# alxn3/nbody-llm

Hardware: AMD Instinct MI355X
Metric: pairwise_interactions_per_sec (higher is better)
Workload: dtype f32

## Files before the change

include/nbody_hip.h:

```cpp
#ifndef NBODY_HIP_H
#define NBODY_HIP_H

#include <stddef.h>
#include <stdint.h>

#ifdef __cplusplus
extern "C" {
#endif

#define NBODY_ABI_VERSION 4

typedef struct NbodyHandle NbodyHandle;

enum {
    NBODY_OK = 0,
    NBODY_ERR_INVALID = -1,
    NBODY_ERR_HIP = -2,
    NBODY_ERR_CAPACITY = -3,
    NBODY_ERR_TREE_DEPTH = -4,
    NBODY_ERR_COMM = -5,
    NBODY_ERR_NO_DEVICE = -6
};

#define NBODY_MAX_TREE_DEPTH 192

enum { NBODY_BRUTE_FORCE = 0,
       NBODY_BARNES_HUT = 1 };

enum { NBODY_MATH_STRICT = 0,
       NBODY_MATH_FAST = 1 };

enum { NBODY_TREE_HOST = 0,
       NBODY_TREE_DEVICE = 1,
       NBODY_TREE_AUTO = 2 };

enum {
    NBODY_LEAF_REFERENCE = 0,
    NBODY_LEAF_DIRECT = 1
};

enum { NBODY_F32 = 0,
       NBODY_F64 = 1 };

enum { NBODY_SHARD_INDEX = 0,
       NBODY_SHARD_SPATIAL = 1 };

typedef struct NbodyConfig {
    uint32_t struct_size;
    int32_t method;
    int32_t math_mode;
    int32_t leaf_mode;
    int32_t device;
    int32_t rank;
    int32_t world_size;
    int32_t host_threads;
    uint64_t capacity;
    int32_t tree_build;
    int32_t dtype;
    int32_t shard_mode;
    int32_t reserved;
} NbodyConfig;

typedef struct NbodyStats {
    uint64_t steps;
    uint64_t interactions;
    uint64_t node_visits;
    uint64_t tree_nodes;
    uint64_t force_launches;
    uint64_t force_kernel_interactions;
    double force_kernel_ms;
    double tree_build_ms;
    double tree_copy_ms;
    double exchange_ms;
} NbodyStats;

int nbody_create(const NbodyConfig* cfg, NbodyHandle** out);
void nbody_destroy(NbodyHandle* h);
int nbody_clone(const NbodyHandle* h, NbodyHandle** out);
int nbody_get_config(const NbodyHandle* h, NbodyConfig* out);

int nbody_upload(NbodyHandle* h, const void* aos, size_t n, size_t stride_bytes);
int nbody_download(NbodyHandle* h, void* aos, size_t cap, size_t stride_bytes, size_t* n_out);
int nbody_count(NbodyHandle* h, size_t* n_out);
int nbody_count_global(NbodyHandle* h, size_t* n_out);
int nbody_add_point(NbodyHandle* h, const void* particle);
int nbody_remove_point(NbodyHandle* h, size_t index);

int nbody_set_settings(NbodyHandle* h, float g, float g_soft, float dt, float theta2);
int nbody_get_settings(const NbodyHandle* h, float* g, float* g_soft, float* dt, float* theta2);
int nbody_set_bounds(NbodyHandle* h, const float center[3], float width);
int nbody_set_settings_f64(NbodyHandle* h, double g, double g_soft, double dt, double theta2);
int nbody_get_settings_f64(const NbodyHandle* h, double* g, double* g_soft, double* dt, double* theta2);
int nbody_set_bounds_f64(NbodyHandle* h, const double center[3], double width);

int nbody_init(NbodyHandle* h);
int nbody_step_by(NbodyHandle* h, float dt);
int nbody_step_by_f64(NbodyHandle* h, double dt);
int nbody_steps(NbodyHandle* h, int k);
int nbody_update_forces(NbodyHandle* h);
int nbody_elapsed(const NbodyHandle* h, float* out);
int nbody_elapsed_f64(const NbodyHandle* h, double* out);
int nbody_sync(NbodyHandle* h);

int nbody_set_profiling(NbodyHandle* h, int on);
int nbody_stats(NbodyHandle* h, NbodyStats* out);
int nbody_reset_stats(NbodyHandle* h);
int nbody_energy(NbodyHandle* h, double* kinetic, double* potential);
enum { NBODY_POTENTIAL_PAIRS = 0,
       NBODY_POTENTIAL_TREE  = 1 };
int nbody_potentials(NbodyHandle* h, int mode, double* phi, size_t cap, size_t* n_out, uint64_t counts[2]);
int nbody_energy_world(NbodyHandle* h, int mode, double* kinetic, double* potential);
int nbody_tree_export(NbodyHandle* h, float* com_mass, float* width, int32_t* skip, size_t cap, size_t* n_nodes);
int nbody_tree_export_f64(NbodyHandle* h, double* com_mass, double* width, int32_t* skip, size_t cap, size_t* n_nodes);
int nbody_tree_export_cells(NbodyHandle* h, float* min_max6, int32_t* depth, size_t cap, size_t* n_nodes);
const char* nbody_last_error(const NbodyHandle* h);

int nbody_set_tuning(NbodyHandle* h, const char* name, int value);
int nbody_get_tuning(const NbodyHandle* h, const char* name, int* value);
int nbody_is_tuning_build(void);

#define NBODY_COMM_ID_BYTES 128
int nbody_comm_unique_id(void* id_bytes);
int nbody_comm_local_id(void* id_bytes);
int nbody_comm_init(NbodyHandle* h, const void* id_bytes);
int nbody_comm_transport(const NbodyHandle* h, char* out, size_t cap);
int nbody_local_range(const NbodyHandle* h, size_t* first, size_t* count);
int nbody_download_ids(NbodyHandle* h, int32_t* ids, size_t cap, size_t* n_out);
typedef struct NbodyLetStats {
    uint64_t steps;
    uint64_t bodies_migrated;
    uint64_t nodes_local;
    uint64_t nodes_global;
    uint64_t nodes_sent;
    uint64_t nodes_received;
    uint64_t bytes_sent;
    uint64_t bytes_allgather_equivalent;
    double phase_ms[5];
    uint64_t host_syncs;
    uint64_t migrant_respills;
    uint64_t node_array_peak_bytes;
    uint64_t node_array_bytes;
} NbodyLetStats;
int nbody_let_stats(NbodyHandle* h, NbodyLetStats* out);

int nbody_ic_plummer(void* aos, size_t n, size_t stride_bytes, uint64_t seed);
int nbody_ic_disc(void* aos, size_t n_disc, size_t stride_bytes, uint64_t seed);
int nbody_ic_plummer_f64(void* aos, size_t n, size_t stride_bytes, uint64_t seed);
int nbody_ic_disc_f64(void* aos, size_t n_disc, size_t stride_bytes, uint64_t seed);

int nbody_debug_step_begin(NbodyHandle* h, float dt);
int nbody_debug_import_segment(NbodyHandle* h, NbodyHandle* peer);
int nbody_debug_step_forces(NbodyHandle* h, float dt);
int nbody_debug_import_partials(NbodyHandle* h, NbodyHandle* peer);
int nbody_debug_step_end(NbodyHandle* h, float dt);
int nbody_debug_let_phase(NbodyHandle* h, int phase, float dt);
int nbody_debug_let_exchange(NbodyHandle* h, NbodyHandle* peer, int which);
int nbody_debug_let_set_balance(NbodyHandle* h, int by_work);
int nbody_debug_let_bounds(NbodyHandle* h, unsigned long long* out);
int nbody_debug_let_set_prune(NbodyHandle* h, int prune);

int nbody_host_cross_plan(int rank, int world, int seg_cap, int n_own, int* ipt, int* n_sets, int* n_parts, int* parts,
                          int* n_recv, int* recv_from);

int nbody_host_exchange_layout(const int* matrix, int world, int rank, long long clamp, int packed_send, size_t send_stride,
                               size_t* out_at, size_t* n_out, size_t* in_at, size_t* n_in, size_t* total_in);

int nbody_host_launch_plan(size_t n_bodies, float theta2, int fast_math, int out[3]);

int nbody_host_build_tree(const float* pos4, size_t n, const float center[3], float width, int threads,
                          float* com_mass, float* node_width, int32_t* skip, int32_t* leaf_body, int32_t* order,
                          size_t cap, size_t* n_nodes);

int nbody_abi_version(void);
int nbody_device_count(void);

#ifdef __cplusplus
}
#endif
#endif
```

nbody-llm_amd/__init__.py:

```python
from __future__ import annotations

import ctypes as C
import os
from dataclasses import dataclass

import numpy as np

_HERE = os.path.dirname(os.path.abspath(__file__))
LIB_PATH = os.environ.get("NBODY_HIP_LIBRARY") or os.path.join(_HERE, "libnbody_hip.so")

if not os.path.exists(LIB_PATH):
    raise ImportError(
        f"{LIB_PATH} not found: build it with `make -C nbody-llm_amd/csrc` (or __graft_entry__.build()); "
        "there is no Python/CPU fallback for the HIP engine"
    )

lib = C.CDLL(LIB_PATH, mode=C.RTLD_LOCAL)

NBODY_OK = 0
NBODY_ERR_INVALID = -1
NBODY_ERR_HIP = -2
NBODY_ERR_CAPACITY = -3
NBODY_ERR_TREE_DEPTH = -4
NBODY_ERR_COMM = -5
NBODY_ERR_NO_DEVICE = -6
BRUTE_FORCE, BARNES_HUT = 0, 1
STRICT, FAST = 0, 1
LEAF_REFERENCE = 0
LEAF_DIRECT = 1
TREE_HOST, TREE_DEVICE, TREE_AUTO = 0, 1, 2
COMM_ID_BYTES = 128

PARTICLE_DTYPE = np.dtype(
    [("position", "<f4", 3), ("velocity", "<f4", 3), ("acceleration", "<f4", 3), ("mass", "<f4")]
)
assert PARTICLE_DTYPE.itemsize == 40
PARTICLE_DTYPE64 = np.dtype(
    [("position", "<f8", 3), ("velocity", "<f8", 3), ("acceleration", "<f8", 3), ("mass", "<f8")]
)
assert PARTICLE_DTYPE64.itemsize == 80
F32, F64 = 0, 1
POTENTIAL_PAIRS, POTENTIAL_TREE = 0, 1
SHARD_INDEX, SHARD_SPATIAL = 0, 1

DECLARED_SYMBOLS = [
    "nbody_create", "nbody_destroy", "nbody_clone", "nbody_upload", "nbody_download", "nbody_count",
    "nbody_count_global", "nbody_add_point", "nbody_remove_point", "nbody_set_settings", "nbody_get_settings",
    "nbody_set_bounds", "nbody_init", "nbody_step_by", "nbody_steps", "nbody_update_forces", "nbody_elapsed",
    "nbody_sync", "nbody_set_profiling", "nbody_stats", "nbody_reset_stats", "nbody_energy", "nbody_tree_export",
    "nbody_last_error", "nbody_comm_unique_id", "nbody_comm_init", "nbody_local_range", "nbody_ic_plummer",
    "nbody_ic_disc", "nbody_host_build_tree", "nbody_abi_version", "nbody_device_count",
    "nbody_debug_step_begin", "nbody_debug_import_segment", "nbody_debug_step_forces",
    "nbody_debug_import_partials", "nbody_debug_step_end", "nbody_host_cross_plan",
    "nbody_set_settings_f64", "nbody_get_settings_f64", "nbody_set_bounds_f64", "nbody_step_by_f64", "nbody_elapsed_f64",
    "nbody_tree_export_f64", "nbody_ic_plummer_f64", "nbody_ic_disc_f64",
    "nbody_download_ids", "nbody_let_stats", "nbody_debug_let_phase", "nbody_debug_let_exchange", "nbody_debug_let_set_prune",
    "nbody_debug_let_bounds", "nbody_debug_let_set_balance",
    "nbody_comm_local_id", "nbody_comm_transport", "nbody_host_exchange_layout",
    "nbody_set_tuning", "nbody_get_tuning", "nbody_is_tuning_build", "nbody_tree_export_cells", "nbody_host_launch_plan",
    "nbody_get_config", "nbody_potentials", "nbody_energy_world",
]


class NbodyConfig(C.Structure):
    _fields_ = [
        ("struct_size", C.c_uint32), ("method", C.c_int32), ("math_mode", C.c_int32), ("leaf_mode", C.c_int32),
        ("device", C.c_int32), ("rank", C.c_int32), ("world_size", C.c_int32), ("host_threads", C.c_int32),
        ("capacity", C.c_uint64), ("tree_build", C.c_int32), ("dtype", C.c_int32), ("shard_mode", C.c_int32), ("reserved", C.c_int32),
    ]


class NbodyLetStats(C.Structure):
    _fields_ = [(k, C.c_uint64) for k in ("steps", "bodies_migrated", "nodes_local", "nodes_global", "nodes_sent", "nodes_received",
                                          "bytes_sent", "bytes_allgather_equivalent")] + [("phase_ms", C.c_double * 5)] + \
               [(k, C.c_uint64) for k in ("host_syncs", "migrant_respills", "node_array_peak_bytes", "node_array_bytes")]


class NbodyStats(C.Structure):
    _fields_ = [
        ("steps", C.c_uint64), ("interactions", C.c_uint64), ("node_visits", C.c_uint64), ("tree_nodes", C.c_uint64),
        ("force_launches", C.c_uint64), ("force_kernel_interactions", C.c_uint64), ("force_kernel_ms", C.c_double), ("tree_build_ms", C.c_double),
        ("tree_copy_ms", C.c_double), ("exchange_ms", C.c_double),
    ]


_H = C.c_void_p
_f, _sz, _i = C.c_float, C.c_size_t, C.c_int
_pf = C.POINTER(C.c_float)


def _sig(name, restype, *argtypes):
    fn = getattr(lib, name)
    fn.restype = restype
    fn.argtypes = list(argtypes)
    return fn


_sig("nbody_create", _i, C.POINTER(NbodyConfig), C.POINTER(_H))
_sig("nbody_destroy", None, _H)
_sig("nbody_clone", _i, _H, C.POINTER(_H))
_sig("nbody_upload", _i, _H, C.c_void_p, _sz, _sz)
_sig("nbody_download", _i, _H, C.c_void_p, _sz, _sz, C.POINTER(_sz))
_sig("nbody_count", _i, _H, C.POINTER(_sz))
_sig("nbody_count_global", _i, _H, C.POINTER(_sz))
_sig("nbody_add_point", _i, _H, C.c_void_p)
_sig("nbody_remove_point", _i, _H, _sz)
_sig("nbody_set_settings", _i, _H, _f, _f, _f, _f)
_sig("nbody_get_settings", _i, _H, _pf, _pf, _pf, _pf)
_sig("nbody_set_bounds", _i, _H, _pf, _f)
_sig("nbody_init", _i, _H)
_sig("nbody_step_by", _i, _H, _f)
_sig("nbody_steps", _i, _H, _i)
_sig("nbody_update_forces", _i, _H)
_sig("nbody_elapsed", _i, _H, _pf)
_sig("nbody_sync", _i, _H)
_sig("nbody_set_profiling", _i, _H, _i)
_sig("nbody_stats", _i, _H, C.POINTER(NbodyStats))
_sig("nbody_reset_stats", _i, _H)
_sig("nbody_energy", _i, _H, C.POINTER(C.c_double), C.POINTER(C.c_double))
_sig("nbody_potentials", _i, _H, _i, C.c_void_p, _sz, C.POINTER(_sz), C.POINTER(C.c_uint64))
_sig("nbody_energy_world", _i, _H, _i, C.POINTER(C.c_double), C.POINTER(C.c_double))
_sig("nbody_tree_export", _i, _H, C.c_void_p, C.c_void_p, C.c_void_p, _sz, C.POINTER(_sz))
_sig("nbody_tree_export_cells", _i, _H, C.c_void_p, C.c_void_p, _sz, C.POINTER(_sz))
_sig("nbody_last_error", C.c_char_p, _H)
_sig("nbody_comm_unique_id", _i, C.c_void_p)
_sig("nbody_comm_init", _i, _H, C.c_void_p)
_sig("nbody_comm_local_id", _i, C.c_void_p)
_sig("nbody_comm_transport", _i, _H, C.c_char_p, _sz)
_sig("nbody_local_range", _i, _H, C.POINTER(_sz), C.POINTER(_sz))
_sig("nbody_ic_plummer", _i, C.c_void_p, _sz, _sz, C.c_uint64)
_sig("nbody_ic_disc", _i, C.c_void_p, _sz, _sz, C.c_uint64)
_sig("nbody_host_build_tree", _i, C.c_void_p, _sz, _pf, _f, _i, C.c_void_p, C.c_void_p, C.c_void_p, C.c_void_p,
     C.c_void_p, _sz, C.POINTER(_sz))
_sig("nbody_debug_step_begin", _i, _H, _f)
_sig("nbody_debug_import_segment", _i, _H, _H)
_sig("nbody_debug_step_forces", _i, _H, _f)
_sig("nbody_debug_import_partials", _i, _H, _H)
_sig("nbody_debug_step_end", _i, _H, _f)
_sig("nbody_host_cross_plan", _i, _i, _i, _i, _i, C.POINTER(_i), C.POINTER(_i), C.POINTER(_i), C.c_void_p, C.POINTER(_i),
     C.c_void_p)
_d = C.c_double
_pd = C.POINTER(C.c_double)
_sig("nbody_set_settings_f64", _i, _H, _d, _d, _d, _d)
_sig("nbody_get_settings_f64", _i, _H, _pd, _pd, _pd, _pd)
_sig("nbody_set_bounds_f64", _i, _H, _pd, _d)
_sig("nbody_step_by_f64", _i, _H, _d)
_sig("nbody_elapsed_f64", _i, _H, _pd)
_sig("nbody_tree_export_f64", _i, _H, C.c_void_p, C.c_void_p, C.c_void_p, _sz, C.POINTER(_sz))
_sig("nbody_ic_plummer_f64", _i, C.c_void_p, _sz, _sz, C.c_uint64)
_sig("nbody_ic_disc_f64", _i, C.c_void_p, _sz, _sz, C.c_uint64)
_sig("nbody_download_ids", _i, _H, C.c_void_p, _sz, C.POINTER(_sz))
_sig("nbody_let_stats", _i, _H, C.POINTER(NbodyLetStats))
_sig("nbody_debug_let_phase", _i, _H, _i, _f)
_sig("nbody_debug_let_exchange", _i, _H, _H, _i)
_sig("nbody_debug_let_set_prune", _i, _H, _i)
_sig("nbody_debug_let_bounds", _i, _H, C.c_void_p)
_sig("nbody_debug_let_set_balance", _i, _H, _i)
_sig("nbody_host_exchange_layout", _i, C.c_void_p, _i, _i, C.c_longlong, _i, _sz, C.c_void_p, C.c_void_p, C.c_void_p, C.c_void_p, C.POINTER(_sz))
_sig("nbody_host_launch_plan", _i, _sz, _f, _i, C.POINTER(_i))
_sig("nbody_set_tuning", _i, _H, C.c_char_p, _i)
_sig("nbody_get_tuning", _i, _H, C.c_char_p, C.POINTER(_i))
_sig("nbody_is_tuning_build", _i)
_sig("nbody_get_config", _i, _H, C.POINTER(NbodyConfig))
_sig("nbody_abi_version", _i)
_sig("nbody_device_count", _i)


_default_tuning: dict = {}


class tuning_defaults:
    def __init__(self, **knobs):
        self.knobs = knobs

    def __enter__(self):
        self.saved = dict(_default_tuning)
        _default_tuning.update(self.knobs)
        return self

    def __exit__(self, *a):
        _default_tuning.clear()
        _default_tuning.update(self.saved)


def launch_plan(n_bodies: int, theta2: float = 0.25, fast_math: bool = True) -> dict:
    out = (C.c_int * 3)()
    rc = lib.nbody_host_launch_plan(int(n_bodies), float(theta2), int(bool(fast_math)), out)
    if rc != 0:
        raise NbodyError(rc, "nbody_host_launch_plan")
    return {"walk_bodies_per_lane": out[0], "walk_segments": out[1], "sym_bodies_per_lane": out[2]}


def is_tuning_build() -> bool:
    return bool(lib.nbody_is_tuning_build())


class NbodyError(RuntimeError):
    def __init__(self, code: int, msg: str):
        super().__init__(f"nbody error {code}: {msg}")
        self.code = code


def device_count() -> int:
    return int(lib.nbody_device_count())


def plummer(n: int, seed: int = 20250523, f64: bool = False) -> np.ndarray:
    if f64:
        out = np.zeros(n, dtype=PARTICLE_DTYPE64)
        rc = lib.nbody_ic_plummer_f64(out.ctypes.data, n, 80, seed)
        if rc:
            raise NbodyError(rc, "nbody_ic_plummer_f64")
        return out
    out = np.zeros(n, dtype=PARTICLE_DTYPE)
    rc = lib.nbody_ic_plummer(out.ctypes.data, n, 40, seed)
    if rc:
        raise NbodyError(rc, "nbody_ic_plummer")
    return out


def disc(n_disc: int, seed: int = 20250523, f64: bool = False) -> np.ndarray:
# ... 367 lines not shown
```

nbody-llm_amd/csrc/bf_pair.h:

```cpp
#pragma once
#include <hip/hip_runtime.h>

namespace nbody {
namespace {

__device__ __forceinline__ float rotl(float v, int src_lane_x4) {
    return __int_as_float(__builtin_amdgcn_ds_bpermute(src_lane_x4, __float_as_int(v)));
}

#define PAD_POS 1.0e15f

template <int IPT, int DBG = 0, bool SYM = true>
__device__ __forceinline__ void pair_evals(const float (&xi)[IPT], const float (&yi)[IPT], const float (&zi)[IPT],
                                           const float (&mi)[IPT], float (&axi)[IPT], float (&ayi)[IPT],
                                           float (&azi)[IPT], float xj, float yj, float zj, float mj, float& axj,
                                           float& ayj, float& azj, float eps2) {
    float dx[IPT], dy[IPT], dz[IPT], r[IPT], sj[IPT];
#pragma unroll
    for (int q = 0; q < IPT; ++q) dx[q] = xj - xi[q];
#pragma unroll
    for (int q = 0; q < IPT; ++q) dy[q] = yj - yi[q];
#pragma unroll
    for (int q = 0; q < IPT; ++q) dz[q] = zj - zi[q];
    __builtin_amdgcn_sched_barrier(0);
#pragma unroll
    for (int q = 0; q < IPT; ++q) r[q] = __builtin_fmaf(dx[q], dx[q], eps2);
    __builtin_amdgcn_sched_barrier(0);
#pragma unroll
    for (int q = 0; q < IPT; ++q) r[q] = __builtin_fmaf(dy[q], dy[q], r[q]);
    __builtin_amdgcn_sched_barrier(0);
#pragma unroll
    for (int q = 0; q < IPT; ++q) r[q] = __builtin_fmaf(dz[q], dz[q], r[q]);
    __builtin_amdgcn_sched_barrier(0);
#pragma unroll
    for (int q = 0; q < IPT; ++q) {
        if (DBG & 2) asm volatile("v_mul_f32 %0, %0, %0" : "+v"(r[q]));
        else r[q] = __builtin_amdgcn_rsqf(r[q]);
    }
    __builtin_amdgcn_sched_barrier(0);
#pragma unroll
    for (int q = 0; q < IPT; ++q) sj[q] = r[q] * r[q];
    __builtin_amdgcn_sched_barrier(0);
#pragma unroll
    for (int q = 0; q < IPT; ++q) r[q] = sj[q] * r[q];
    __builtin_amdgcn_sched_barrier(0);
#pragma unroll
    for (int q = 0; q < IPT; ++q) sj[q] = mj * r[q];
    __builtin_amdgcn_sched_barrier(0);
    if (SYM) {
#pragma unroll
        for (int q = 0; q < IPT; ++q) r[q] = mi[q] * r[q];
        __builtin_amdgcn_sched_barrier(0);
#pragma unroll
        for (int q = 0; q < IPT; ++q) {
            axi[q] = __builtin_fmaf(dx[q], sj[q], axi[q]);
            axj = __builtin_fmaf(-dx[q], r[q], axj);
            ayi[q] = __builtin_fmaf(dy[q], sj[q], ayi[q]);
            ayj = __builtin_fmaf(-dy[q], r[q], ayj);
            azi[q] = __builtin_fmaf(dz[q], sj[q], azi[q]);
            azj = __builtin_fmaf(-dz[q], r[q], azj);
            __builtin_amdgcn_sched_barrier(0);
        }
    } else {
#pragma unroll
        for (int q = 0; q < IPT; ++q) axi[q] = __builtin_fmaf(dx[q], sj[q], axi[q]);
        __builtin_amdgcn_sched_barrier(0);
#pragma unroll
        for (int q = 0; q < IPT; ++q) ayi[q] = __builtin_fmaf(dy[q], sj[q], ayi[q]);
        __builtin_amdgcn_sched_barrier(0);
#pragma unroll
        for (int q = 0; q < IPT; ++q) azi[q] = __builtin_fmaf(dz[q], sj[q], azi[q]);
        __builtin_amdgcn_sched_barrier(0);
    }
}


typedef float v2f __attribute__((ext_vector_type(2)));

__device__ __forceinline__ v2f splat2(float v) { v2f r = {v, v}; return r; }
__device__ __forceinline__ v2f pk_fma(v2f a, v2f b, v2f c) { return __builtin_elementwise_fma(a, b, c); }

template <int IPT2, int DBG = 0, bool SYM = true>
__device__ __forceinline__ void pair_evals_pk(const v2f (&xi)[IPT2], const v2f (&yi)[IPT2], const v2f (&zi)[IPT2],
                                              const v2f (&mi)[IPT2], v2f (&axi)[IPT2], v2f (&ayi)[IPT2],
                                              v2f (&azi)[IPT2], float xj, float yj, float zj, float mj, v2f& axj,
                                              v2f& ayj, v2f& azj, float eps2) {
    v2f dx[IPT2], dy[IPT2], dz[IPT2], r[IPT2], sj[IPT2];
    const v2f xj2 = splat2(xj), yj2 = splat2(yj), zj2 = splat2(zj), mj2 = splat2(mj), e2 = splat2(eps2);
#pragma unroll
    for (int q = 0; q < IPT2; ++q) dx[q] = xj2 - xi[q];
#pragma unroll
    for (int q = 0; q < IPT2; ++q) dy[q] = yj2 - yi[q];
#pragma unroll
    for (int q = 0; q < IPT2; ++q) dz[q] = zj2 - zi[q];
    __builtin_amdgcn_sched_barrier(0);
#pragma unroll
    for (int q = 0; q < IPT2; ++q) r[q] = pk_fma(dx[q], dx[q], e2);
    __builtin_amdgcn_sched_barrier(0);
#pragma unroll
    for (int q = 0; q < IPT2; ++q) r[q] = pk_fma(dy[q], dy[q], r[q]);
    __builtin_amdgcn_sched_barrier(0);
#pragma unroll
    for (int q = 0; q < IPT2; ++q) r[q] = pk_fma(dz[q], dz[q], r[q]);
    __builtin_amdgcn_sched_barrier(0);
#pragma unroll
    for (int q = 0; q < IPT2; ++q) {
        if (DBG & 2) { asm volatile("v_mul_f32 %0, %0, %0" : "+v"(r[q].x)); asm volatile("v_mul_f32 %0, %0, %0" : "+v"(r[q].y)); }
        else { r[q].x = __builtin_amdgcn_rsqf(r[q].x); r[q].y = __builtin_amdgcn_rsqf(r[q].y); }
    }
    __builtin_amdgcn_sched_barrier(0);
#pragma unroll
    for (int q = 0; q < IPT2; ++q) sj[q] = r[q] * r[q];
    __builtin_amdgcn_sched_barrier(0);
#pragma unroll
    for (int q = 0; q < IPT2; ++q) r[q] = sj[q] * r[q];
    __builtin_amdgcn_sched_barrier(0);
#pragma unroll
    for (int q = 0; q < IPT2; ++q) sj[q] = mj2 * r[q];
    __builtin_amdgcn_sched_barrier(0);
    if (SYM) {
#pragma unroll
        for (int q = 0; q < IPT2; ++q) r[q] = mi[q] * r[q];
        __builtin_amdgcn_sched_barrier(0);
#pragma unroll
        for (int q = 0; q < IPT2; ++q) {
            axi[q] = pk_fma(dx[q], sj[q], axi[q]);
            axj = pk_fma(-dx[q], r[q], axj);
            ayi[q] = pk_fma(dy[q], sj[q], ayi[q]);
            ayj = pk_fma(-dy[q], r[q], ayj);
            azi[q] = pk_fma(dz[q], sj[q], azi[q]);
            azj = pk_fma(-dz[q], r[q], azj);
            __builtin_amdgcn_sched_barrier(0);
        }
    } else {
#pragma unroll
        for (int q = 0; q < IPT2; ++q) axi[q] = pk_fma(dx[q], sj[q], axi[q]);
        __builtin_amdgcn_sched_barrier(0);
#pragma unroll
        for (int q = 0; q < IPT2; ++q) ayi[q] = pk_fma(dy[q], sj[q], ayi[q]);
        __builtin_amdgcn_sched_barrier(0);
#pragma unroll
        for (int q = 0; q < IPT2; ++q) azi[q] = pk_fma(dz[q], sj[q], azi[q]);
        __builtin_amdgcn_sched_barrier(0);
    }
}

template <int IPT>
__device__ __forceinline__ void pack_pairs(const float (&a)[IPT], v2f (&b)[IPT / 2]) {
#pragma unroll
    for (int q = 0; q < IPT / 2; ++q) b[q] = v2f{a[2 * q], a[2 * q + 1]};
}
template <int IPT>
__device__ __forceinline__ void unpack_pairs(const v2f (&b)[IPT / 2], float (&a)[IPT]) {
#pragma unroll
    for (int q = 0; q < IPT / 2; ++q) { a[2 * q] = b[q].x; a[2 * q + 1] = b[q].y; }
}

}
}
```

nbody-llm_amd/csrc/kernels.h:

```cpp
#pragma once
#include <hip/hip_runtime.h>
#include <cstdint>
#include <vector>

namespace nbody {

struct Tuning {
    int cross_sym = 1;
    int sym_packed = 1;
    int bf_fast_variant = 0;
    int bh_walk_duo = -1;
    int bh_walk_xcd = 1;
    int let_list_div = 4;
    int sym_ipt = 0;
    int sym_wpb = 4;
    int sym_rounds = 1;
    int sym_k = 0;
    int sym_min_bodies = 1024;
    int sym_reduce_split = 1;
    int cross_slots = 3072;
    int cross_ipt = 0;
    int cross_wpb = 4;
    int bh_walk_split = 0;
    int bh_walk_order = 1;
    int bh_reduce_split = 1;
    int tree_max_tie = 64;
    int bf64_min_bodies = 10240;
    int bf64_ipt = 0;
    int bf64_rot = 0;
    int bf64_waves = 0;
    int bh_walk_variant = 0;
    int bh_walk_lds_block = 1024;
    int bh_hot_cap = 2048;
    int bh_walk_debug = 0;
    int sym_debug = 0;
};
const Tuning& tuning();
struct WalkPlan { int bodies_per_lane; int segments; };
WalkPlan walk_plan(size_t n_order, bool fast_math, int max_segments, float theta2);
void bind_tuning(const Tuning* t);

struct Shard {
    float4* pos_all = nullptr;
    float4* vel = nullptr;
    float4* acc = nullptr;
    int* seg_count = nullptr;
    int* escaped = nullptr;
    unsigned char* keep = nullptr;
    unsigned long long* tile_state = nullptr;
    int* epoch = nullptr;
    int* poison = nullptr;
    int* ids = nullptr;
    unsigned long long* inter = nullptr;
    int n_seg = 1;
    int seg_cap = 0;
    int my_seg = 0;
    float4* own_pos() const { return pos_all + size_t(my_seg) * seg_cap; }
    int* own_count() const { return seg_count + my_seg; }
};

struct BoundsF {
    float lo[3];
    float hi[3];
};

void launch_aos_to_soa(hipStream_t s, const float* aos, int stride_f, int n, float4* pos, float4* vel, float4* acc);
void launch_soa_to_aos(hipStream_t s, float* aos, int stride_f, int n, const float4* pos, const float4* vel, const float4* acc);

void launch_drift_half(hipStream_t s, const Shard& sh, int n_upper, float dt, BoundsF b);
void launch_compact(hipStream_t s, const Shard& sh, int n_upper);
void launch_kick_drift(hipStream_t s, const Shard& sh, int n_upper, float dt);

void launch_bf_forces_strict(hipStream_t s, const Shard& sh, int n_upper, float g, float g_soft2);
void launch_bf_forces_fast(hipStream_t s, const Shard& sh, int n_upper, float g, float g_soft2);

struct SymPlan {
    int ipt = 8;
    int A = 0;
    int K = 0;
    int wpb = 16;
    int res_combine = 0;
    int k_res = 0;
    int sym_sets = 0;
    int n_planes = 0;
    int k_os = 0;
    size_t n_pad = 0;
    size_t plane_stride = 0;
    std::vector<int> bounds;
};
SymPlan make_sym_plan(int n_upper);
int sym_bodies_per_lane(size_t n);
uint64_t sym_main_pairs(const SymPlan& p, size_t n);
void launch_bf_sym_main(hipStream_t s, const Shard& sh, const SymPlan& p, const int* d_bounds, float4* planes,
                        int n_upper, float g_soft2);
void launch_bf_os(hipStream_t s, const Shard& sh, int A, int K, float4* planes, size_t plane_stride, float g_soft2);
void launch_bf_sym_tail(hipStream_t s, const Shard& sh, const SymPlan& p, float4* planes, int n_upper, float g,
                        float g_soft2, const float* kick_dt);

struct CrossPartners {
    static constexpr int kMax = 8;
    int n = 0;
    int seg[kMax];
    int c0[kMax], c1[kMax];
    int a0[kMax], a1[kMax];
};
struct CrossPlan {
    static constexpr int kMaxPlanes = 256;
    int ipt = 8;
    int A = 0;
    CrossPartners parts;
    int n_recv = 0;
    int recv_from[CrossPartners::kMax];
    int k_res = 0;
    std::vector<int4> slices;
};
CrossPlan make_cross_plan(int rank, int world, int seg_cap, int n_own_upper);
void launch_bf_cross(hipStream_t s, const Shard& sh, const CrossPlan& p, const int4* d_slices, float4* res_planes,
                     float4* xplanes, float4* send, size_t plane_stride, float g_soft2);

constexpr int kMaxSplit = 64, kMaxAnc = 192;
constexpr size_t kSplitInts = size_t(kMaxSplit) + 1 + kMaxSplit + size_t(kMaxSplit) * kMaxAnc;
struct TreeDev {
    const float4* nodes = nullptr;
    int n_nodes = 0;
    const int* order = nullptr;
    int n_order = 0;
    int n_split = 1;
    const int* split_first = nullptr;
    const int* split_anc = nullptr;
    const int* split_n_anc = nullptr;
    float4* split_planes = nullptr;
    size_t split_stride = 0;
    float4* nested_stack = nullptr;
    size_t nested_stride = 0;
    float4* walk = nullptr;
    float4* hot = nullptr;
    int* unified = nullptr;
    int* hot_info = nullptr;
    int hot_cap = 0;
    int hot_threshold = 0;
    const int* poison = nullptr;
    const int* n_order_dev = nullptr;
    int store_work = 0;
    float4* bfs = nullptr;
    void* bfs_ws = nullptr;
    size_t bfs_cap = 0;
};
struct TreeDevWork {
    const unsigned long long* keys = nullptr;
    const signed char* delta = nullptr;
    const int* base = nullptr;
    const int* ids = nullptr;
    const unsigned long long* keys2 = nullptr;
    const int* wpre = nullptr;
    const void* incl = nullptr;
};
struct TreeCat {
    float4* pos = nullptr;
    int* flags = nullptr;
    int* base = nullptr;
    int* own_order = nullptr;
    int* info = nullptr;
};
size_t tree_build_workspace_bytes(size_t n_cap);
size_t tree_build_tmp_bytes(size_t n_cap);
size_t tree_cat_bytes(size_t n_cap);
TreeCat tree_cat_layout(void* buf, size_t n_cap);
void launch_tree_cat(hipStream_t s, const Shard& sh, const TreeCat& c);
size_t tree_cat_bytes64(size_t n_cap);
TreeCat tree_cat_layout64(void* buf, size_t n_cap, double4** pos_cat);
void launch_tree_cat64(hipStream_t s, const double4* pos_all, const int* seg_count, int n_seg, int seg_cap, int my_seg, double4* pos_cat, int* info);
int launch_tree_own_order(hipStream_t s, const int* order, const TreeCat& c, int n_total_upper, void* tmp, size_t tmp_bytes);
struct TreeSplitReq { int n_split = 0; int* first = nullptr; int* n_anc = nullptr; int* anc = nullptr; int max_anc = 0; const int* info = nullptr; int* poison = nullptr; };
int build_octree_device(hipStream_t s, const float4* pos, const int* d_count, int n_upper, const float center[3],
                        float width, void* workspace, size_t n_cap, float4* nodes, int node_cap, int* order,
                        int* out_info, TreeDevWork* work, int want_hot = 0 , const TreeSplitReq* split = nullptr);
size_t bfs_workspace_bytes(size_t n_cap);
int build_bfs_layout(hipStream_t s, const float4* nodes, int n_nodes, void* workspace, size_t n_cap, float4* out);
}
namespace nbody64 { struct Node64; }
namespace nbody {
int build_octree_device_f64(hipStream_t s, const double4* pos, const int* d_count, int n_upper, const double center[3], double width,
                            void* workspace, size_t n_cap, nbody64::Node64* nodes, int node_cap, int* order, int* out_info,
                            TreeDevWork* work, const TreeSplitReq* split = nullptr);
int tree_sort_keys(hipStream_t s, const float4* pos, const int* d_count, int n_upper, const float center[3], float width,
                   void* workspace, size_t n_cap, int* out_info, TreeDevWork* work);
int tree_emit_sorted(hipStream_t s, const float4* pos, const int* d_count, int n_upper, float width, void* workspace, size_t n_cap,
                     float4* nodes, int node_cap, int* order, int* out_info, int want_hot, const int* edge, const TreeSplitReq* split = nullptr);
int tree_scan_sorted(hipStream_t s, const float4* pos, const int* d_count, int n_upper, void* workspace, size_t n_cap, int* out_info,
                     const int* edge, const float4* weight_src = nullptr );
__host__ __device__ inline int body_weight(float visits) { const int v = int(visits) >> 4; return v < 1 ? 1 : v; }
int tree_emit_nodes(hipStream_t s, const float4* pos, const int* d_count, int n_upper, float width, void* workspace, size_t n_cap,
                    float4* nodes, int node_cap, int slice_cap, int* order, int* out_info, int want_hot, const int* edge,
                    const int* node_offset, int* parent, unsigned char* depth);
void launch_tree_split_anc(hipStream_t s, const TreeDevWork& work, int n, int n_nodes, int n_split, int* first,
                           int* n_anc, int* anc, int max_anc, const int* info = nullptr ,
                           int* poison = nullptr );

#define NBODY_WALK_COUNTER_SLOTS 1024u
void launch_walk_split_scan(hipStream_t s, const float4* nodes, const int* range, int n_split, int* first, int* n_anc, int* anc, int first_given = 0);
void launch_bh_walk(hipStream_t s, const Shard& sh, const TreeDev& t, float g, float g_soft2, float theta2,
                    int fast_math, unsigned long long* counters , int leaf_direct = 0,
                    const float* kick_dt = nullptr ,
                    int* kicked = nullptr );

void launch_energy(hipStream_t s, const Shard& sh, int n_upper, double g_soft2, double* out2);

}
```

nbody-llm_amd/csrc/kernels_bf_sym.hip:

```cpp
#include "kernels.h"
#include "bf_pair.h"

#include <algorithm>

namespace nbody {

namespace {

#ifdef NBODY_TUNING
__device__ unsigned long long nbody_sym_stamps[3 * 8192];
#endif

}

template <int IPT>
__device__ __forceinline__ void sym_rest_wave(const float4* __restrict__ pos, int n, int A, int group, int slice,
                                              int n_slices, float& ax, float& ay, float& az, float eps2);

template <int IPT, int NW>
__device__ __forceinline__ void sym_rest_block(const float4* __restrict__ pos, int n, int A, int group,
                                               float4* __restrict__ plane, float eps2, float (*red)[3][64]);

template <int IPT, int WPB, int DBG = 0, bool PK = false>
__global__ __launch_bounds__(WPB * 64) void k_bf_sym(const float4* __restrict__ pos, const int* __restrict__ count,
                                                     int A, int K, const int* __restrict__ bounds, int sym_sets,
                                                     float4* __restrict__ planes, size_t plane_stride, float eps2,
                                                     int res_combine) {
    const int lane = threadIdx.x & 63;
    const int wslot = __builtin_amdgcn_readfirstlane(threadIdx.x >> 6);
    const int n_main_blocks = (A * K + WPB - 1) / WPB;
    if (int(blockIdx.x) >= n_main_blocks) {
        __shared__ float red[WPB - 1][3][64];
        sym_rest_block<IPT, WPB>(pos, *count, A, blockIdx.x - n_main_blocks,
                                 planes + size_t(sym_sets + (res_combine ? K / WPB : K)) * plane_stride, eps2, red);
        return;
    }
    const int gw = blockIdx.x * WPB + (wslot & 3) * (WPB / 4) + (wslot >> 2);
    if (gw >= A * K) return;
    const int a = gw / K;
    const int part = gw - a * K;
    const int n = *count;
    const int Cn = A * IPT;
    const int k0 = bounds[part], k1 = bounds[part + 1];
    const int src_lane = ((lane + 63) & 63) * 4;
    const int src_lane2 = ((lane + 62) & 63) * 4;
    float eps2v = eps2;
    asm volatile("" : "+v"(eps2v));

    float xi[IPT], yi[IPT], zi[IPT], mi[IPT], axi[IPT], ayi[IPT], azi[IPT];
#pragma unroll
    for (int q = 0; q < IPT; ++q) {
        const int i = (a * IPT + q) * 64 + lane;
        const float4 p = (i < n) ? pos[i] : make_float4(PAD_POS, PAD_POS, PAD_POS, 0.f);
        xi[q] = p.x; yi[q] = p.y; zi[q] = p.z; mi[q] = p.w;
        axi[q] = ayi[q] = azi[q] = 0.f;
    }

    auto chunk_of = [&](int k) {
        int c = (a + 1) * IPT + k;
        if (c >= Cn) c -= Cn;
        return c;
    };
    auto load_chunk = [&](int k) {
        const int j = chunk_of(k) * 64 + lane;
        return (j < n) ? pos[j] : make_float4(PAD_POS, PAD_POS, PAD_POS, 0.f);
    };

    [[maybe_unused]] unsigned long long t_beg = 0, r_beg = 0;
    if (DBG & 4) { t_beg = __builtin_amdgcn_s_memtime(); r_beg = __builtin_amdgcn_s_memrealtime(); }
    float4 nxt = (k0 < k1) ? load_chunk(k0) : make_float4(0.f, 0.f, 0.f, 0.f);
    v2f xi2[IPT / 2], yi2[IPT / 2], zi2[IPT / 2], mi2[IPT / 2], axi2[IPT / 2], ayi2[IPT / 2], azi2[IPT / 2];
    if (PK) {
        pack_pairs<IPT>(xi, xi2); pack_pairs<IPT>(yi, yi2); pack_pairs<IPT>(zi, zi2); pack_pairs<IPT>(mi, mi2);
        pack_pairs<IPT>(axi, axi2); pack_pairs<IPT>(ayi, ayi2); pack_pairs<IPT>(azi, azi2);
    }
    for (int k = k0; k < k1; ++k) {
        float xj = nxt.x, yj = nxt.y, zj = nxt.z, mj = nxt.w;
        float axj = 0.f, ayj = 0.f, azj = 0.f;
        v2f axj2 = {0.f, 0.f}, ayj2 = {0.f, 0.f}, azj2 = {0.f, 0.f};
        if (k + 1 < k1) nxt = load_chunk(k + 1);
        switch ((4 * (k1 - k) - 1) / (k1 - k0)) {
            case 3: __builtin_amdgcn_s_setprio(3); break;
            case 2: __builtin_amdgcn_s_setprio(2); break;
            case 1: __builtin_amdgcn_s_setprio(1); break;
            default: __builtin_amdgcn_s_setprio(0); break;
        }
        if (PK) {
            for (int s = 0; s < 64; s += 2) {
                const float x1 = rotl(xj, src_lane), y1 = rotl(yj, src_lane), z1 = rotl(zj, src_lane), m1 = rotl(mj, src_lane);
                pair_evals_pk<IPT / 2, DBG>(xi2, yi2, zi2, mi2, axi2, ayi2, azi2, xj, yj, zj, mj, axj2, ayj2, azj2, eps2v);
                axj2.x = rotl(axj2.x, src_lane); ayj2.x = rotl(ayj2.x, src_lane); azj2.x = rotl(azj2.x, src_lane);
                axj2.y = rotl(axj2.y, src_lane); ayj2.y = rotl(ayj2.y, src_lane); azj2.y = rotl(azj2.y, src_lane);
                xj = rotl(x1, src_lane); yj = rotl(y1, src_lane); zj = rotl(z1, src_lane); mj = rotl(m1, src_lane);
                pair_evals_pk<IPT / 2, DBG>(xi2, yi2, zi2, mi2, axi2, ayi2, azi2, x1, y1, z1, m1, axj2, ayj2, azj2, eps2v);
                axj2.x = rotl(axj2.x, src_lane); ayj2.x = rotl(ayj2.x, src_lane); azj2.x = rotl(azj2.x, src_lane);
                axj2.y = rotl(axj2.y, src_lane); ayj2.y = rotl(ayj2.y, src_lane); azj2.y = rotl(azj2.y, src_lane);
            }
        } else {
            float x1 = rotl(xj, src_lane), y1 = rotl(yj, src_lane), z1 = rotl(zj, src_lane), m1 = rotl(mj, src_lane);
#pragma unroll 2
            for (int s = 0; s < 64; ++s) {
                const float x2 = rotl(xj, src_lane2), y2 = rotl(yj, src_lane2), z2 = rotl(zj, src_lane2), m2 = rotl(mj, src_lane2);
                pair_evals<IPT, DBG>(xi, yi, zi, mi, axi, ayi, azi, xj, yj, zj, mj, axj, ayj, azj, eps2v);
                axj = rotl(axj, src_lane); ayj = rotl(ayj, src_lane); azj = rotl(azj, src_lane);
                xj = x1; yj = y1; zj = z1; mj = m1;
                x1 = x2; y1 = y2; z1 = z2; m1 = m2;
            }
        }
        if (PK) { axj = axj2.x + axj2.y; ayj = ayj2.x + ayj2.y; azj = azj2.x + azj2.y; }
        const int d = k / IPT + 1;
        planes[size_t(d - 1) * plane_stride + size_t(chunk_of(k)) * 64 + lane] = make_float4(axj, ayj, azj, 0.f);
    }
    if (PK) { unpack_pairs<IPT>(axi2, axi); unpack_pairs<IPT>(ayi2, ayi); unpack_pairs<IPT>(azi2, azi); }

#ifdef NBODY_TUNING
    if (DBG & 4) {
        const unsigned long long t_end = __builtin_amdgcn_s_memtime(), r_end = __builtin_amdgcn_s_memrealtime();
        if (lane == 0 && gw < 8192) {
            nbody_sym_stamps[gw * 3 + 0] = t_end - t_beg;
            nbody_sym_stamps[gw * 3 + 1] = r_end - r_beg;
            const unsigned hw = __builtin_amdgcn_s_getreg((4 ) | (0 << 6) | (31 << 11));
            const unsigned xcc = __builtin_amdgcn_s_getreg((20 ) | (0 << 6) | (31 << 11));
            nbody_sym_stamps[gw * 3 + 2] = (unsigned long long)(k1 - k0) | ((unsigned long long)hw << 16) | ((unsigned long long)(xcc & 0xF) << 48);
        }
    }
#endif
    if (res_combine) {
        __shared__ float comb[WPB - 1][3 * IPT][64];
        const int first_part = (part / WPB) * WPB;
        const int rel = part - first_part;
        if (rel > 0) {
#pragma unroll
            for (int q = 0; q < IPT; ++q) {
                comb[rel - 1][3 * q + 0][lane] = axi[q];
                comb[rel - 1][3 * q + 1][lane] = ayi[q];
                comb[rel - 1][3 * q + 2][lane] = azi[q];
            }
        }
        __syncthreads();
        if (rel == 0) {
            float4* __restrict__ out = planes + size_t(sym_sets + part / WPB) * plane_stride;
#pragma unroll
            for (int q = 0; q < IPT; ++q) {
                float sx = axi[q], sy = ayi[q], sz = azi[q];
                for (int w = 0; w < WPB - 1; ++w) { sx += comb[w][3 * q + 0][lane]; sy += comb[w][3 * q + 1][lane]; sz += comb[w][3 * q + 2][lane]; }
                out[size_t(a * IPT + q) * 64 + lane] = make_float4(sx, sy, sz, 0.f);
            }
        }
        return;
    }
    float4* __restrict__ out = planes + size_t(sym_sets + part) * plane_stride;
#pragma unroll
    for (int q = 0; q < IPT; ++q) out[size_t(a * IPT + q) * 64 + lane] = make_float4(axi[q], ayi[q], azi[q], 0.f);
}

template <int IPT, int WPB, bool PK>
__global__ __launch_bounds__(WPB * 64) void k_bf_os(const float4* __restrict__ pos_all,
                                                    const int* __restrict__ seg_count, int n_seg, int seg_cap,
                                                    int my_seg, int A, int K, float4* __restrict__ planes,
                                                    size_t plane_stride, float eps2) {
    __shared__ float4 stage[WPB][2][64];
    const int lane = threadIdx.x & 63;
    const int wslot = __builtin_amdgcn_readfirstlane(threadIdx.x >> 6);
    const int gw = blockIdx.x * WPB + (wslot & 3) * (WPB / 4) + (wslot >> 2);
    if (gw >= A * K) return;
    const int a = gw / K, part = gw - a * K;
    const int n_own = seg_count[my_seg];
    const float4* __restrict__ own = pos_all + size_t(my_seg) * seg_cap;
    float eps2v = eps2;
    asm volatile("" : "+v"(eps2v));

    float xi[IPT], yi[IPT], zi[IPT], mi[IPT], axi[IPT], ayi[IPT], azi[IPT];
#pragma unroll
    for (int q = 0; q < IPT; ++q) {
        const int i = (a * IPT + q) * 64 + lane;
        const float4 p = (i < n_own) ? own[i] : make_float4(PAD_POS, PAD_POS, PAD_POS, 0.f);
        xi[q] = p.x; yi[q] = p.y; zi[q] = p.z; mi[q] = p.w;
        axi[q] = ayi[q] = azi[q] = 0.f;
    }
    long long R = 0;
    for (int s = 0; s < n_seg; ++s) if (s != my_seg) R += seg_count[s];
    const long long r0 = R * part / K, r1 = R * (part + 1) / K;
    long long seg_first = 0;
    float dummy_x = 0.f, dummy_y = 0.f, dummy_z = 0.f;
    v2f dummy2 = {0.f, 0.f};
    v2f xi2[IPT / 2], yi2[IPT / 2], zi2[IPT / 2], mi2[IPT / 2], axi2[IPT / 2], ayi2[IPT / 2], azi2[IPT / 2];
    if (PK) {
        pack_pairs<IPT>(xi, xi2); pack_pairs<IPT>(yi, yi2); pack_pairs<IPT>(zi, zi2); pack_pairs<IPT>(mi, mi2);
        pack_pairs<IPT>(axi, axi2); pack_pairs<IPT>(ayi, ayi2); pack_pairs<IPT>(azi, azi2);
    }
    for (int s = 0; s < n_seg; ++s) {
        if (s == my_seg) continue;
        const int ns = seg_count[s];
        const long long lo = r0 > seg_first ? r0 : seg_first;
        const long long hi = r1 < seg_first + ns ? r1 : seg_first + ns;
        const float4* __restrict__ ps = pos_all + size_t(s) * seg_cap - seg_first;
        int buf = 0;
        if (lo < hi) {
            const long long j = lo + lane;
            stage[wslot][0][lane] = (j < hi) ? ps[j] : make_float4(PAD_POS, PAD_POS, PAD_POS, 0.f);
        }
        for (long long c0 = lo; c0 < hi; c0 += 64) {
            const long long jn = c0 + 64 + lane;
            float4 nxt = make_float4(PAD_POS, PAD_POS, PAD_POS, 0.f);
            if (c0 + 64 < hi && jn < hi) nxt = ps[jn];
            const int cnt = int(hi - c0 < 64 ? hi - c0 : 64);
            switch (int((4 * (r1 - c0) - 1) / (r1 - r0))) {
                case 3: __builtin_amdgcn_s_setprio(3); break;
                case 2: __builtin_amdgcn_s_setprio(2); break;
                case 1: __builtin_amdgcn_s_setprio(1); break;
                default: __builtin_amdgcn_s_setprio(0); break;
            }
            float4 pj = stage[wslot][buf][0];
            for (int t = 0; t < cnt; ++t) {
                const float4 pn = stage[wslot][buf][(t + 1) & 63];
                if (PK)
                    pair_evals_pk<IPT / 2, 0, false>(xi2, yi2, zi2, mi2, axi2, ayi2, azi2, pj.x, pj.y, pj.z, pj.w, dummy2,
                                                     dummy2, dummy2, eps2v);
                else
                    pair_evals<IPT, 0, false>(xi, yi, zi, mi, axi, ayi, azi, pj.x, pj.y, pj.z, pj.w, dummy_x, dummy_y,
                                              dummy_z, eps2v);
                pj = pn;
            }
            buf ^= 1;
            stage[wslot][buf][lane] = nxt;
        }
        seg_first += ns;
    }
    if (PK) { unpack_pairs<IPT>(axi2, axi); unpack_pairs<IPT>(ayi2, ayi); unpack_pairs<IPT>(azi2, azi); }
    float4* __restrict__ out = planes + size_t(part) * plane_stride;
#pragma unroll
    for (int q = 0; q < IPT; ++q) out[size_t(a * IPT + q) * 64 + lane] = make_float4(axi[q], ayi[q], azi[q], 0.f);
}

template <int IPT>
__device__ __forceinline__ void sym_rest_wave(const float4* __restrict__ pos, int n, int A, int group, int slice,
                                              int n_slices, float& ax, float& ay, float& az, float eps2) {
    constexpr int SET = 64 * IPT;
    const int lane = threadIdx.x & 63;
    const int i = group * 64 + lane;
    const int a = (group * 64) / SET;
    const float4 pi = (i < n) ? pos[i] : make_float4(PAD_POS, PAD_POS, PAD_POS, 0.f);
    ax = ay = az = 0.f;
    const int n_win = (A % 2 == 0 && A > 1) ? 2 : 1;
    for (int w = 0; w < n_win; ++w) {
        int set = (w == 0) ? a : a + A / 2;
        if (set >= A) set -= A;
        const int j0 = set * SET + SET * slice / n_slices;
        const int j1 = min(n, set * SET + SET * (slice + 1) / n_slices);
#pragma unroll 8
        for (int j = j0; j < j1; ++j) {
            const float4 pj = pos[j];
            const float dx = pj.x - pi.x, dy = pj.y - pi.y, dz = pj.z - pi.z;
            const float r2 = __builtin_fmaf(dz, dz, __builtin_fmaf(dy, dy, __builtin_fmaf(dx, dx, eps2)));
            const float rinv = __builtin_amdgcn_rsqf(r2);
            float sj = pj.w * ((rinv * rinv) * rinv);
            sj = (j == i) ? 0.f : sj;
            ax = __builtin_fmaf(dx, sj, ax);
            ay = __builtin_fmaf(dy, sj, ay);
            az = __builtin_fmaf(dz, sj, az);
        }
    }
}

template <int IPT, int NW>
__device__ __forceinline__ void sym_rest_block(const float4* __restrict__ pos, int n, int A, int group,
                                               float4* __restrict__ plane, float eps2, float (*red)[3][64]) {
    const int lane = threadIdx.x & 63;
    const int wv = __builtin_amdgcn_readfirstlane(threadIdx.x >> 6);
    float ax, ay, az;
    sym_rest_wave<IPT>(pos, n, A, group, wv, NW, ax, ay, az, eps2);
    if (wv > 0) { red[wv - 1][0][lane] = ax; red[wv - 1][1][lane] = ay; red[wv - 1][2][lane] = az; }
    __syncthreads();
    if (wv == 0) {
#pragma unroll
        for (int w = 0; w < NW - 1; ++w) { ax += red[w][0][lane]; ay += red[w][1][lane]; az += red[w][2][lane]; }
        plane[group * 64 + lane] = make_float4(ax, ay, az, 0.f);
    }
}

template <int IPT>
__global__ __launch_bounds__(512) void k_bf_sym_rest(const float4* __restrict__ pos, const int* __restrict__ count,
                                                     int A, float4* __restrict__ plane, float eps2) {
    __shared__ float red[7][3][64];
    sym_rest_block<IPT, 8>(pos, *count, A, blockIdx.x, plane, eps2, red);
}

template <bool KICK>
__global__ __launch_bounds__(256) void k_bf_sym_reduce(const float4* __restrict__ planes, int n_planes,
                                                       size_t plane_stride, const int* __restrict__ count, float g,
                                                       float4* __restrict__ acc, float4* __restrict__ pos,
                                                       float4* __restrict__ vel, float dt, const int* __restrict__ seg_count,
                                                       int n_seg, unsigned long long* __restrict__ inter) {
    const int i = blockIdx.x * 256 + threadIdx.x;
    if (inter && i == 0) {
        long long tot = 0;
        for (int s = 0; s < n_seg; ++s) tot += seg_count[s];
        if (tot > 0) atomicAdd(inter, (unsigned long long)(*count) * (unsigned long long)(tot - 1));
    }
    if (i >= *count) return;
    float sx = 0.f, sy = 0.f, sz = 0.f, cx = 0.f, cy = 0.f, cz = 0.f;
    for (int p = 0; p < n_planes; ++p) {
        const float4 v = planes[size_t(p) * plane_stride + i];
        const float yx = v.x - cx, yy = v.y - cy, yz = v.z - cz;
        const float tx = sx + yx, ty = sy + yy, tz = sz + yz;
        cx = (tx - sx) - yx; cy = (ty - sy) - yy; cz = (tz - sz) - yz;
        sx = tx; sy = ty; sz = tz;
    }
    const float4 a = make_float4(g * sx, g * sy, g * sz, 0.f);
    acc[i] = a;
    if (KICK) {
        float4 p = pos[i], v = vel[i];
        v.x += a.x * dt; v.y += a.y * dt; v.z += a.z * dt;
        p.x += (v.x * 0.5f) * dt; p.y += (v.y * 0.5f) * dt; p.z += (v.z * 0.5f) * dt;
        vel[i] = v;
        pos[i] = p;
    }
}

template <bool KICK, int Q>
__global__ __launch_bounds__(64 * Q) void k_bf_sym_reduce_split(const float4* __restrict__ planes, int n_planes, size_t plane_stride,
                                                                const int* __restrict__ count, float g, float4* __restrict__ acc,
                                                                float4* __restrict__ pos, float4* __restrict__ vel, float dt,
                                                                const int* __restrict__ seg_count, int n_seg,
                                                                unsigned long long* __restrict__ inter) {
    __shared__ float part[Q][3][64];
    const int lane = threadIdx.x & 63, q = threadIdx.x >> 6;
    const int i = blockIdx.x * 64 + lane;
    if (inter && blockIdx.x == 0 && threadIdx.x == 0) {
        long long tot = 0;
        for (int s = 0; s < n_seg; ++s) tot += seg_count[s];
        if (tot > 0) atomicAdd(inter, (unsigned long long)(*count) * (unsigned long long)(tot - 1));
    }
    const int n = *count;
    float sx = 0.f, sy = 0.f, sz = 0.f, cx = 0.f, cy = 0.f, cz = 0.f;
    if (i < n) {
        const int p0 = int((long long)n_planes * q / Q), p1 = int((long long)n_planes * (q + 1) / Q);
        for (int p = p0; p < p1; ++p) {
            const float4 v = planes[size_t(p) * plane_stride + i];
            const float yx = v.x - cx, yy = v.y - cy, yz = v.z - cz;
            const float tx = sx + yx, ty = sy + yy, tz = sz + yz;
            cx = (tx - sx) - yx; cy = (ty - sy) - yy; cz = (tz - sz) - yz;
            sx = tx; sy = ty; sz = tz;
        }
    }
    part[q][0][lane] = sx; part[q][1][lane] = sy; part[q][2][lane] = sz;
    __syncthreads();
    if (q != 0 || i >= n) return;
    sx = sy = sz = cx = cy = cz = 0.f;
    for (int w = 0; w < Q; ++w) {
        const float yx = part[w][0][lane] - cx, yy = part[w][1][lane] - cy, yz = part[w][2][lane] - cz;
        const float tx = sx + yx, ty = sy + yy, tz = sz + yz;
        cx = (tx - sx) - yx; cy = (ty - sy) - yy; cz = (tz - sz) - yz;
        sx = tx; sy = ty; sz = tz;
    }
    const float4 a = make_float4(g * sx, g * sy, g * sz, 0.f);
    acc[i] = a;
    if (KICK) {
        float4 p = pos[i], v = vel[i];
        v.x += a.x * dt; v.y += a.y * dt; v.z += a.z * dt;
        p.x += (v.x * 0.5f) * dt; p.y += (v.y * 0.5f) * dt; p.z += (v.z * 0.5f) * dt;
        vel[i] = v;
        pos[i] = p;
    }
}

}
#ifdef NBODY_TUNING
namespace nbody { int read_sym_stamps(unsigned long long* out, int n_waves); }
extern "C" int nbody_sym_read_stamps(unsigned long long* out, int n_waves) { return nbody::read_sym_stamps(out, n_waves); }
#endif
namespace nbody {

int sym_bodies_per_lane(size_t n) {
    const Tuning& t = tuning();
    if (!t.sym_packed || t.sym_wpb != 4 || t.sym_ipt == 8) return 8;
    if (t.sym_ipt == 4) return 4;
    return n <= 10240 ? 4 : 8;
}

SymPlan make_sym_plan(int n_upper) {
    SymPlan p;
    const int IPT = sym_bodies_per_lane(size_t(n_upper));
    p.ipt = IPT;
    p.A = (n_upper + 64 * IPT - 1) / (64 * IPT);
    p.sym_sets = (p.A + 1) / 2 - 1;
    const int L = IPT * p.sym_sets;
    const int want = tuning().sym_wpb;
    p.wpb = want == 8 ? 8 : want == 12 ? 12 : want == 16 ? 16 : 4;
    int K = 1;
    if (p.wpb == 4) {
        K = L <= 100 ? L : L <= 160 ? (L + 1) / 2 : 64;
    } else {
        const int resident_wgs_per_cu = (p.wpb == 8) ? 2 : 1;
        const int slots = 256 * resident_wgs_per_cu * p.wpb;
        double best = 0.0;
        const int k_hi = std::min(126, std::min(L, std::max(1, slots * std::max(1, tuning().sym_rounds) * 4 / p.A)));
        for (int k = 1; k <= k_hi; ++k) {
            const long long waves = (long long)p.A * k;
            const long long rounds = (waves + slots - 1) / slots;
            if (rounds > 4 * std::max(1, tuning().sym_rounds) && k > 1) break;
            const double fill = double(waves) / double(rounds * slots);
            const double even = (L % k == 0) ? 1.0 : double(L / k) / double(L / k + 1);
            const double per_wave = double(L) / k / (double(L) / k + 0.3);
            if (fill * even * per_wave > best + 1e-9) { best = fill * even * per_wave; K = k; }
        }
    }
    if (tuning().sym_k > 0) K = std::min(126, tuning().sym_k);
    if (K > L) K = L;
    if (K < 1) K = 1;
    p.K = K;
    p.res_combine = (K % p.wpb == 0) ? 1 : 0;
    p.k_res = p.res_combine ? K / p.wpb : K;
    p.n_planes = p.sym_sets + p.k_res + 1;
    p.n_pad = size_t(p.A) * 64 * IPT;
    p.plane_stride = p.n_pad;
    p.bounds.resize(K + 1);
    for (int part = 0; part <= K; ++part) p.bounds[part] = int((long long)L * part / K);
    return p;
}

#ifdef NBODY_TUNING
int read_sym_stamps(unsigned long long* out, int n_waves) {
    return hipMemcpyFromSymbol(out, HIP_SYMBOL(nbody_sym_stamps), sizeof(unsigned long long) * 3 * n_waves) == hipSuccess ? 0 : -1;
}
#endif

uint64_t sym_main_pairs(const SymPlan& p, size_t n) {
    const size_t set = size_t(64) * p.ipt;
    auto size_of = [&](int a) { size_t lo = size_t(a) * set; return lo >= n ? size_t(0) : std::min(set, n - lo); };
    uint64_t pairs = 0;
    for (int a = 0; a < p.A; ++a)
        for (int d = 1; d <= p.sym_sets; ++d) pairs += uint64_t(size_of(a)) * uint64_t(size_of((a + d) % p.A));
    return pairs;
}

void launch_bf_sym_main(hipStream_t s, const Shard& sh, const SymPlan& p, const int* d_bounds, float4* planes,
                        int n_upper, float g_soft2) {
    if (n_upper <= 0 || p.sym_sets <= 0) return;
    const int main_blocks = (p.A * p.K + p.wpb - 1) / p.wpb;
    const int rest_blocks = int(p.n_pad / 64);
    const dim3 grid(main_blocks + rest_blocks), block(p.wpb * 64);
#define SYM_LAUNCH(WPB, DBG) hipLaunchKernelGGL((k_bf_sym<8, WPB, DBG, PKV>), grid, block, 0, s, sh.own_pos(), sh.own_count(), p.A, p.K, d_bounds, p.sym_sets, planes, p.plane_stride, g_soft2, p.res_combine)
#ifdef NBODY_TUNING
    const int dbg = tuning().sym_debug;
#else
    constexpr int dbg = 0;
#endif
    if (p.ipt == 4) {
        hipLaunchKernelGGL((k_bf_sym<4, 4, 0, true>), grid, block, 0, s, sh.own_pos(), sh.own_count(), p.A, p.K, d_bounds, p.sym_sets, planes, p.plane_stride, g_soft2, p.res_combine);
        return;
    }
    if (tuning().sym_packed) {
        constexpr bool PKV = true;
        if (dbg == 4) {
#ifdef NBODY_TUNING
            if (p.wpb == 12) SYM_LAUNCH(12, 4); else if (p.wpb == 8) SYM_LAUNCH(8, 4); else if (p.wpb == 4) SYM_LAUNCH(4, 4); else SYM_LAUNCH(16, 4);
#endif
        } else {
            if (p.wpb == 12) SYM_LAUNCH(12, 0); else if (p.wpb == 8) SYM_LAUNCH(8, 0); else if (p.wpb == 4) SYM_LAUNCH(4, 0); else SYM_LAUNCH(16, 0);
        }
    } else {
        constexpr bool PKV = false;
        if (dbg >= 4 && dbg <= 7) {
#ifdef NBODY_TUNING
            if (dbg == 4) { if (p.wpb == 12) SYM_LAUNCH(12, 4); else if (p.wpb == 8) SYM_LAUNCH(8, 4); else if (p.wpb == 4) SYM_LAUNCH(4, 4); else SYM_LAUNCH(16, 4); }
            else if (dbg == 5) SYM_LAUNCH(16, 5);
            else if (dbg == 6) SYM_LAUNCH(16, 6);
            else SYM_LAUNCH(16, 7);
#endif
        } else {
            if (p.wpb == 12) SYM_LAUNCH(12, 0); else if (p.wpb == 8) SYM_LAUNCH(8, 0); else if (p.wpb == 4) SYM_LAUNCH(4, 0); else SYM_LAUNCH(16, 0);
        }
    }
#undef SYM_LAUNCH
}

void launch_bf_os(hipStream_t s, const Shard& sh, int A, int K, float4* planes, size_t plane_stride, float g_soft2) {
    if (A <= 0 || K <= 0) return;
    const int wpb = 12;
    if (tuning().sym_packed)
        hipLaunchKernelGGL((k_bf_os<8, 12, true>), dim3((A * K + wpb - 1) / wpb), dim3(wpb * 64), 0, s, sh.pos_all,
                           sh.seg_count, sh.n_seg, sh.seg_cap, sh.my_seg, A, K, planes, plane_stride, g_soft2);
    else
        hipLaunchKernelGGL((k_bf_os<8, 12, false>), dim3((A * K + wpb - 1) / wpb), dim3(wpb * 64), 0, s, sh.pos_all,
                           sh.seg_count, sh.n_seg, sh.seg_cap, sh.my_seg, A, K, planes, plane_stride, g_soft2);
}

void launch_bf_sym_tail(hipStream_t s, const Shard& sh, const SymPlan& p, float4* planes, int n_upper, float g,
                        float g_soft2, const float* kick_dt) {
    if (n_upper <= 0) return;
    if (p.sym_sets == 0) {
        float4* resident0 = planes + size_t(p.sym_sets) * p.plane_stride;
        (void)hipMemsetAsync(resident0, 0, size_t(p.k_res) * p.plane_stride * sizeof(float4), s);
        if (p.ipt == 4)
            hipLaunchKernelGGL(k_bf_sym_rest<4>, dim3(int(p.n_pad / 64)), dim3(512), 0, s, sh.own_pos(),
                               sh.own_count(), p.A, planes + size_t(p.sym_sets + p.k_res) * p.plane_stride, g_soft2);
        else
        hipLaunchKernelGGL(k_bf_sym_rest<8>, dim3(int(p.n_pad / 64)), dim3(512), 0, s, sh.own_pos(),
                           sh.own_count(), p.A, planes + size_t(p.sym_sets + p.k_res) * p.plane_stride, g_soft2);
    }
    const float dt = kick_dt ? *kick_dt : 0.f;
#define REDUCE_ARGS planes, p.n_planes, p.plane_stride, sh.own_count(), g, sh.acc, sh.own_pos(), sh.vel, dt, sh.seg_count, sh.n_seg, sh.inter
    if (tuning().sym_reduce_split && p.n_planes >= 16) {
        const dim3 grid((n_upper + 63) / 64);
        if (n_upper <= 16384) {
            if (kick_dt) hipLaunchKernelGGL((k_bf_sym_reduce_split<true, 16>), grid, dim3(1024), 0, s, REDUCE_ARGS);
            else hipLaunchKernelGGL((k_bf_sym_reduce_split<false, 16>), grid, dim3(1024), 0, s, REDUCE_ARGS);
        } else {
            if (kick_dt) hipLaunchKernelGGL((k_bf_sym_reduce_split<true, 4>), grid, dim3(256), 0, s, REDUCE_ARGS);
            else hipLaunchKernelGGL((k_bf_sym_reduce_split<false, 4>), grid, dim3(256), 0, s, REDUCE_ARGS);
        }
    } else {
        const dim3 grid((n_upper + 255) / 256);
        if (kick_dt) hipLaunchKernelGGL(k_bf_sym_reduce<true>, grid, dim3(256), 0, s, REDUCE_ARGS);
        else hipLaunchKernelGGL(k_bf_sym_reduce<false>, grid, dim3(256), 0, s, REDUCE_ARGS);
    }
#undef REDUCE_ARGS
}

}
```

nbody-llm_amd/csrc/nbody_api.cpp:

```cpp
#include "nbody_handle.h"
#include "nbody_f64.h"
#include "nbody_let.h"
#include "nbody_pot.h"

#include <algorithm>
#include <chrono>
#include <cmath>
#include <cstdio>
#include <cstdlib>
#include <cstring>
#include <memory>
#include <string>
#include <thread>
#include <vector>


static thread_local std::string g_create_err;

int fail(NbodyHandle* h, int code, const std::string& msg) {
    if (h) h->err = msg; else g_create_err = msg;
    return code;
}

namespace {
// ... 16 lines not shown
    if (records <= h->aos_cap) return NBODY_OK;
    if (h->d_aos) (void)hipFree(h->d_aos);
    if (h->h_aos) (void)hipHostFree(h->h_aos);
    h->d_aos = nullptr; h->h_aos = nullptr; h->aos_cap = 0;
    HIP_TRY(h, hipMalloc(&h->d_aos, records * 10 * sizeof(float)));
    HIP_TRY(h, hipHostMalloc(&h->h_aos, records * 10 * sizeof(float), hipHostMallocDefault));
    h->aos_cap = records;
    return NBODY_OK;
}

int sync_count(NbodyHandle* h) {
    if (!h->count_dirty) return NBODY_OK;
    HIP_TRY(h, hipMemcpyAsync(h->h_counts, h->sh.seg_count, sizeof(int) * h->sh.n_seg, hipMemcpyDeviceToHost, h->stream));
    HIP_TRY(h, hipStreamSynchronize(h->stream));
    for (int s = 0; s < h->sh.n_seg; ++s) h->seg_count_host[s] = h->h_counts[s];
    h->n_local = size_t(h->h_counts[h->sh.my_seg]);
    h->count_dirty = false;
    return NBODY_OK;
}

int push_counts(NbodyHandle* h) {
    for (int s = 0; s < h->sh.n_seg; ++s) h->h_counts[s] = h->seg_count_host[s];
    HIP_TRY(h, hipMemcpyAsync(h->sh.seg_count, h->h_counts, sizeof(int) * h->sh.n_seg, hipMemcpyHostToDevice, h->stream));
    HIP_TRY(h, hipStreamSynchronize(h->stream));
    return NBODY_OK;
}

size_t total_upper(const NbodyHandle* h) {
    size_t t = 0;
    for (int c : h->seg_count_host) t += size_t(c);
    return t;
}

int exchange_begin(NbodyHandle* h) {
    if (h->sh.n_seg == 1 && !h->comm_ready) return NBODY_OK;
    if (!h->comm_ready) return fail(h, NBODY_ERR_COMM, "world_size > 1 but nbody_comm_init has not been called");
    HIP_TRY(h, hipEventRecord(h->ev_drifted, h->stream));
    HIP_TRY(h, hipStreamWaitEvent(h->comm_stream, h->ev_drifted, 0));
    TP_TRY(h, h->tp->group_begin());
    TP_TRY(h, h->tp->all_gather(h->sh.pos_all, size_t(h->sh.seg_cap) * sizeof(float4), h->comm_stream));
    TP_TRY(h, h->tp->all_gather(h->sh.seg_count, sizeof(int), h->comm_stream));
    TP_TRY(h, h->tp->group_end());
    HIP_TRY(h, hipEventRecord(h->ev_gathered, h->comm_stream));
    h->exchange_in_flight = true;
    return NBODY_OK;
}

int exchange_wait(NbodyHandle* h) {
    if (!h->exchange_in_flight) return NBODY_OK;
    HIP_TRY(h, hipStreamWaitEvent(h->stream, h->ev_gathered, 0));
    h->exchange_in_flight = false;
    return NBODY_OK;
}

int comm_check(NbodyHandle* h) {
    if (!h->tp) return NBODY_OK;
    int rc = h->tp->check();
    return rc ? fail(h, rc, h->tp->error()) : NBODY_OK;
}

int sharded_counts_exact(NbodyHandle* h) {
    if (!h->comm_ready) return fail(h, NBODY_ERR_COMM, "world_size > 1 but nbody_comm_init has not been called");
    int rc = exchange_wait(h);
    if (rc) return rc;
    HIP_TRY(h, hipStreamSynchronize(h->stream));
    TP_TRY(h, h->tp->all_gather(h->sh.seg_count, sizeof(int), h->stream));
    h->count_dirty = true;
    return sync_count(h);
}

int push_own_count(NbodyHandle* h) {
    h->h_counts[h->sh.my_seg] = int(h->n_local);
    HIP_TRY(h, hipMemcpyAsync(h->sh.own_count(), h->h_counts + h->sh.my_seg, sizeof(int), hipMemcpyHostToDevice, h->stream));
    HIP_TRY(h, hipStreamSynchronize(h->stream));
    return NBODY_OK;
}

int sharded_add_point(NbodyHandle* h, const void* particle) {
    int rc = sharded_counts_exact(h);
    if (rc) return rc;
    const int G = h->sh.n_seg, last = G - 1;
    if (total_upper(h) >= h->cfg.capacity || h->seg_count_host[last] >= h->sh.seg_cap)
        return fail(h, NBODY_ERR_CAPACITY, "capacity exhausted (a push goes to the end of the vector: the last rank's block is full)");
    if (h->sh.my_seg == last) {
        const float* p = static_cast<const float*>(particle);
        float4 rec[3] = {make_float4(p[0], p[1], p[2], p[9]), make_float4(p[3], p[4], p[5], 0.f), make_float4(p[6], p[7], p[8], 0.f)};
        const size_t k = h->n_local;
        HIP_TRY(h, hipMemcpyAsync(h->sh.own_pos() + k, &rec[0], sizeof(float4), hipMemcpyHostToDevice, h->stream));
        HIP_TRY(h, hipMemcpyAsync(h->sh.vel + k, &rec[1], sizeof(float4), hipMemcpyHostToDevice, h->stream));
        HIP_TRY(h, hipMemcpyAsync(h->sh.acc + k, &rec[2], sizeof(float4), hipMemcpyHostToDevice, h->stream));
        HIP_TRY(h, hipStreamSynchronize(h->stream));
        h->n_local = k + 1;
        rc = push_own_count(h);
        if (rc) return rc;
    }
    h->seg_count_host[last] += 1;
    return NBODY_OK;
}

int sharded_remove_point(NbodyHandle* h, size_t index) {
    int rc = sharded_counts_exact(h);
    if (rc) return rc;
    const int G = h->sh.n_seg, me = h->sh.my_seg;
    if (index >= total_upper(h)) return fail(h, NBODY_ERR_INVALID, "swap_remove index out of range");
    int r = 0, last = G - 1;
    size_t j = index;
    while (j >= size_t(h->seg_count_host[r])) { j -= size_t(h->seg_count_host[r]); ++r; }
    while (h->seg_count_host[last] == 0) --last;
    const size_t tail = size_t(h->seg_count_host[last]) - 1;
    if (r == last) {
        if (me == r && j != tail) {
            HIP_TRY(h, hipMemcpyAsync(h->sh.own_pos() + j, h->sh.own_pos() + tail, sizeof(float4), hipMemcpyDeviceToDevice, h->stream));
            HIP_TRY(h, hipMemcpyAsync(h->sh.vel + j, h->sh.vel + tail, sizeof(float4), hipMemcpyDeviceToDevice, h->stream));
            HIP_TRY(h, hipMemcpyAsync(h->sh.acc + j, h->sh.acc + tail, sizeof(float4), hipMemcpyDeviceToDevice, h->stream));
        }
    } else if (me == last || me == r) {
        rc = ensure_aos(h, 2);
        if (rc) return rc;
        if (me == last) {
            nbody::launch_soa_to_aos(h->stream, h->d_aos, 10, 1, h->sh.own_pos() + tail, h->sh.vel + tail, h->sh.acc + tail);
            TP_TRY(h, h->tp->send(h->d_aos, 40, r, h->stream));
        } else {
            TP_TRY(h, h->tp->recv(h->d_aos, 40, last, h->stream));
            nbody::launch_aos_to_soa(h->stream, h->d_aos, 10, 1, h->sh.own_pos() + j, h->sh.vel + j, h->sh.acc + j);
        }
        HIP_TRY(h, hipGetLastError());
    }
    if (me == last) {
        h->n_local = tail;
        rc = push_own_count(h);
        if (rc) return rc;
    } else {
        HIP_TRY(h, hipStreamSynchronize(h->stream));
    }
    h->seg_count_host[last] -= 1;
    return comm_check(h);
}

int drain_events(NbodyHandle* h) {
    if (h->ev_pending.empty()) return NBODY_OK;
    HIP_TRY(h, hipStreamSynchronize(h->stream));
    for (auto& ev : h->ev_pending) {
        float ms = 0.f;
        if (hipEventElapsedTime(&ms, ev.first, ev.second) == hipSuccess) {
            h->stats.force_kernel_ms += ms;
            h->stats.force_launches += 1;
        }
        h->ev_free.push_back(ev);
    }
    h->ev_pending.clear();
    return NBODY_OK;
}

constexpr size_t kShardedSymMinBodies = 2048;

int ensure_sym_plan(NbodyHandle* h) {
    const size_t set = size_t(64) * size_t(nbody::sym_bodies_per_lane(std::max<size_t>(1, h->n_local)));
    const int A = int((std::max<size_t>(1, h->n_local) + set - 1) / set);
    const int knobs = nbody::tuning().sym_wpb * 100 + nbody::tuning().sym_rounds + nbody::tuning().sym_k * 10000 + nbody::tuning().sym_ipt * 1000000;
    if (h->sym_plan.A == A && h->sym_plan.ipt * 64 == int(set) && h->d_sym_bounds && h->sym_waves == knobs) return NBODY_OK;
    h->sym_waves = knobs;
    h->sym_plan = nbody::make_sym_plan(int(std::max<size_t>(1, h->n_local)));
    nbody::SymPlan& p = h->sym_plan;
    h->cross_on = false;
    if (h->sh.n_seg > 1) {
        const size_t cap_pad = (size_t(h->sh.seg_cap) + 63) / 64 * 64;
        p.plane_stride = std::max(p.n_pad, cap_pad);
        if (nbody::tuning().cross_sym && h->sh.n_seg <= 2 * (nbody::CrossPartners::kMax - 1)) {
            h->cross = nbody::make_cross_plan(h->sh.my_seg, h->sh.n_seg, h->sh.seg_cap, int(std::max<size_t>(1, h->n_local)));
            h->cross_on = true;
            h->recv_plane0 = p.n_planes + h->cross.k_res;
            p.n_planes += h->cross.k_res + h->cross.n_recv;
        } else {
            const int a_os = int((p.n_pad + 511) / 512);
            p.k_os = std::max(1, std::min(256, 3072 / std::max(1, a_os)));
            p.plane_stride = std::max(p.plane_stride, size_t(a_os) * 512);
            p.n_planes += p.k_os;
        }
    }
    if (!h->d_sym_bounds) HIP_TRY(h, hipMalloc(&h->d_sym_bounds, 128 * sizeof(int)));
    HIP_TRY(h, hipMemcpyAsync(h->d_sym_bounds, p.bounds.data(), p.bounds.size() * sizeof(int), hipMemcpyHostToDevice, h->stream));
    HIP_TRY(h, hipStreamSynchronize(h->stream));
    const size_t need = size_t(p.n_planes) * p.plane_stride;
    if (need > h->planes_cap) {
        if (h->d_planes) (void)hipFree(h->d_planes);
        h->d_planes = nullptr; h->planes_cap = 0;
        HIP_TRY(h, hipMalloc(&h->d_planes, need * sizeof(float4)));
        h->planes_cap = need;
    }
    if (h->cross_on) {
        const nbody::CrossPlan& c = h->cross;
        if (c.slices.size() > h->cross_slices_cap) {
            if (h->d_cross_slices) (void)hipFree(h->d_cross_slices);
            h->d_cross_slices = nullptr; h->cross_slices_cap = 0;
            HIP_TRY(h, hipMalloc(&h->d_cross_slices, (c.slices.size() + 64) * sizeof(int4)));
            h->cross_slices_cap = c.slices.size() + 64;
        }
        if (!c.slices.empty()) {
            HIP_TRY(h, hipMemcpyAsync(h->d_cross_slices, c.slices.data(), c.slices.size() * sizeof(int4), hipMemcpyHostToDevice, h->stream));
            HIP_TRY(h, hipStreamSynchronize(h->stream));
        }
        const size_t xneed = size_t(std::max(1, c.parts.n)) * size_t(c.A) * p.plane_stride;
        if (xneed > h->xplanes_cap) {
            if (h->d_xplanes) (void)hipFree(h->d_xplanes);
            h->d_xplanes = nullptr; h->xplanes_cap = 0;
            HIP_TRY(h, hipMalloc(&h->d_xplanes, xneed * sizeof(float4)));
            h->xplanes_cap = xneed;
        }
        const size_t sneed = size_t(std::max(1, c.parts.n)) * p.plane_stride;
        if (sneed > h->send_cap) {
            if (h->d_send) (void)hipFree(h->d_send);
            h->d_send = nullptr; h->send_cap = 0;
            HIP_TRY(h, hipMalloc(&h->d_send, sneed * sizeof(float4)));
            h->send_cap = sneed;
        }
    }
    return NBODY_OK;
}

int bf_forces(NbodyHandle* h) {
    const float eps2 = h->g_soft * h->g_soft;
    const bool fast = h->cfg.math_mode == NBODY_MATH_FAST && nbody::tuning().bf_fast_variant == 0;
    const bool sharded = h->sh.n_seg > 1;
    const bool sym = fast && (sharded ? size_t(h->sh.seg_cap) >= kShardedSymMinBodies : h->n_local >= size_t(std::max(1024, nbody::tuning().sym_min_bodies)));
    const size_t tot = total_upper(h);
    if (sym) {
        int rc = ensure_sym_plan(h);
        if (rc) return rc;
        if (h->sym_pairs_n != h->n_local) {
            h->sym_pairs = nbody::sym_main_pairs(h->sym_plan, h->n_local);
            h->sym_pairs_n = h->n_local;
        }
    }
    const nbody::SymPlan& p = h->sym_plan;
    uint64_t timed = 0;
    if (!(sym && sharded)) {
        int rc = exchange_wait(h);
        if (rc) return rc;
    }
    if (!sym) {
        ForceTimer t(h);
        if (h->cfg.math_mode == NBODY_MATH_STRICT) nbody::launch_bf_forces_strict(h->stream, h->sh, int(h->n_local), h->g, eps2);
        else nbody::launch_bf_forces_fast(h->stream, h->sh, int(h->n_local), h->g, eps2);
        timed = tot > 0 ? uint64_t(h->n_local) * uint64_t(tot - 1) : 0;
    } else if (!sharded) {
        {
            ForceTimer t(h);
            nbody::launch_bf_sym_main(h->stream, h->sh, p, h->d_sym_bounds, h->d_planes, int(h->n_local), eps2);
        }
        timed = 2 * h->sym_pairs;
        h->tail_pending = true;
    } else {
        nbody::launch_bf_sym_main(h->stream, h->sh, p, h->d_sym_bounds, h->d_planes, int(h->n_local), eps2);
        {
            int rc = exchange_wait(h);
            if (rc) return rc;
        }
        if (h->cross_on) {
            const nbody::CrossPlan& c = h->cross;
            {
                ForceTimer t(h);
                nbody::launch_bf_cross(h->stream, h->sh, c, h->d_cross_slices,
                                       h->d_planes + size_t(h->recv_plane0 - c.k_res) * p.plane_stride, h->d_xplanes,
                                       h->d_send, p.plane_stride, eps2);
            }
            for (int i = 0; i < c.parts.n; ++i) {
                const long long set = 64LL * c.ipt;
                const long long own = std::max(0LL, std::min<long long>(h->n_local, set * c.parts.a1[i]) - set * c.parts.a0[i]);
                const long long theirs = std::max(0LL, std::min<long long>(h->seg_count_host[c.parts.seg[i]], 64LL * c.parts.c1[i]) - 64LL * c.parts.c0[i]);
                timed += 2ull * uint64_t(own) * uint64_t(theirs);
            }
        } else {
            ForceTimer t(h);
            nbody::launch_bf_os(h->stream, h->sh, int((p.n_pad + 511) / 512), p.k_os, h->d_planes + size_t(p.n_planes - p.k_os) * p.plane_stride, p.plane_stride, eps2);
            timed = uint64_t(h->n_local) * uint64_t(tot - h->n_local);
        }
        h->tail_pending = true;
    }
    HIP_TRY(h, hipGetLastError());
    if (tot > 0 && h->timed_this) h->stats.force_kernel_interactions += timed;
    return NBODY_OK;
}

int ensure_tree_dev(NbodyHandle* h, size_t nodes, size_t order) {
    int rc = grow_dev(h, h->d_nodes, h->d_node_cap, nodes, sizeof(nbody::NodeRec));
    return rc ? rc : grow_dev(h, h->d_order, h->d_order_cap, order, sizeof(int));
}

int bh_walk_device_tree(NbodyHandle* h, bool* fell_back);
int bh_walk_device_tree_async(NbodyHandle* h);
int bh_walk_host_tree(NbodyHandle* h);
void free_all(NbodyHandle* h);
int resolve_async(NbodyHandle* h);
int step_end(NbodyHandle* h, float dt);
int step_impl(NbodyHandle* h, float dt);

int ensure_nested_stack(NbodyHandle* h, nbody::TreeDev* td) {
    if (h->cfg.math_mode != NBODY_MATH_STRICT || h->cfg.leaf_mode != NBODY_LEAF_REFERENCE) return NBODY_OK;
    const size_t lanes = (size_t(h->sh.seg_cap) + 255) / 256 * 256;
    const int levels = (h->tree_on_device ? 43 : h->tree.max_depth) + 2;
    if (lanes > h->nested_cap || levels > h->nested_levels) {
        if (h->d_nested_stack) (void)hipFree(h->d_nested_stack);
        h->d_nested_stack = nullptr; h->nested_cap = 0; h->nested_levels = 0;
        const int lv = std::max(levels + 8, 32);
        HIP_TRY(h, hipMalloc(&h->d_nested_stack, lanes * size_t(lv) * sizeof(float4)));
        h->nested_cap = lanes;
        h->nested_levels = lv;
    }
    td->nested_stack = h->d_nested_stack;
    td->nested_stride = h->nested_cap;
    return NBODY_OK;
}

int setup_lds_walk(NbodyHandle* h, nbody::TreeDev* td, size_t n_tree) {
#ifndef NBODY_TUNING
    (void)h; (void)td; (void)n_tree;
    return NBODY_OK;
#else
    if (h->cfg.math_mode == NBODY_MATH_FAST && nbody::tuning().bh_walk_variant == 5 && (h->tree_on_device || h->tree.max_depth <= 42)) {
        if (h->bfs_cap < h->d_node_cap) {
            if (h->d_bfs) (void)hipFree(h->d_bfs);
            if (h->d_bfs_ws) (void)hipFree(h->d_bfs_ws);
            h->d_bfs = nullptr; h->d_bfs_ws = nullptr; h->bfs_cap = 0;
            HIP_TRY(h, hipMalloc(&h->d_bfs, h->d_node_cap * 2 * sizeof(float4)));
            HIP_TRY(h, hipMalloc(&h->d_bfs_ws, nbody::bfs_workspace_bytes(h->d_node_cap)));
            h->bfs_cap = h->d_node_cap;
        }
        td->bfs = h->d_bfs; td->bfs_ws = h->d_bfs_ws; td->bfs_cap = h->bfs_cap;
        return NBODY_OK;
    }
    if (h->cfg.math_mode != NBODY_MATH_FAST || nbody::tuning().bh_walk_variant != 3 || nbody::tuning().bh_hot_cap <= 0) return NBODY_OK;
    const int M = std::min(nbody::tuning().bh_hot_cap, 5000);
    if (h->walk_cap < h->d_node_cap) {
        if (h->d_walk) (void)hipFree(h->d_walk);
        if (h->d_unified) (void)hipFree(h->d_unified);
        h->d_walk = nullptr; h->d_unified = nullptr; h->walk_cap = 0;
        HIP_TRY(h, hipMalloc(&h->d_walk, (h->d_node_cap + 1) * 2 * sizeof(float4)));
        HIP_TRY(h, hipMalloc(&h->d_unified, (h->d_node_cap + 1) * sizeof(int)));
        h->walk_cap = h->d_node_cap;
    }
    if (h->hot_cap != M) {
        if (h->d_hot) (void)hipFree(h->d_hot);
        h->d_hot = nullptr; h->hot_cap = 0;
        HIP_TRY(h, hipMalloc(&h->d_hot, size_t(M) * 2 * sizeof(float4)));
        HIP_TRY(h, hipMemsetAsync(h->d_hot, 0, size_t(M) * 2 * sizeof(float4), h->stream));
        h->hot_cap = M;
        h->hot_threshold_n = 0;
    }
    if (!h->d_hot_info) {
        HIP_TRY(h, hipMalloc(&h->d_hot_info, 2 * sizeof(int)));
        HIP_TRY(h, hipMemsetAsync(h->d_hot_info, 0, 2 * sizeof(int), h->stream));
        HIP_TRY(h, hipHostMalloc(&h->h_hot_info, 2 * sizeof(int), hipHostMallocDefault));
        h->h_hot_info[0] = h->h_hot_info[1] = 0;
    }
    if (h->hot_threshold_n == 0 || n_tree > 2 * h->hot_threshold_n || 2 * n_tree < h->hot_threshold_n) {
        h->hot_threshold = int(std::max<size_t>(8, n_tree / 64));
        h->hot_threshold_n = std::max<size_t>(1, n_tree);
    } else {
        const int flagged = h->h_hot_info[1];
        if (flagged > M) h->hot_threshold = h->hot_threshold + h->hot_threshold / 8 + 1;
        else if (flagged < M - M / 3 && h->hot_threshold > 2) h->hot_threshold = h->hot_threshold - h->hot_threshold / 8 - 1;
    }
    td->walk = h->d_walk; td->unified = h->d_unified; td->hot = h->d_hot; td->hot_info = h->d_hot_info;
    td->hot_cap = M; td->hot_threshold = h->hot_threshold;
    return NBODY_OK;
#endif
}

int walk_tree(NbodyHandle* h, nbody::TreeDev& td, size_t n_tree) {
    if (h->pot.walking) {
        const size_t stride = (size_t(std::max(td.n_order, 1)) + 63) / 64 * 64;
        int rc = nbody::pot::ensure_planes(h, size_t(td.n_split) * stride);
        if (rc) return rc;
        nbody::launch_bh_pot_walk(h->stream, h->sh.own_pos(), td, h->g_soft * h->g_soft, h->theta2, h->pot.d_planes, stride, h->pot.d_sum,
                                  h->pot.d_counts);
        HIP_TRY(h, hipGetLastError());
        return NBODY_OK;
    }
    int rc = ensure_nested_stack(h, &td);
    if (!rc) rc = setup_lds_walk(h, &td, n_tree);
    if (rc) return rc;
    {
        ForceTimer t(h);
        int kicked = 0;
        nbody::launch_bh_walk(h->stream, h->sh, td, h->g, h->g_soft * h->g_soft, h->theta2,
                              h->cfg.math_mode == NBODY_MATH_FAST, h->d_counters, h->cfg.leaf_mode == NBODY_LEAF_DIRECT,
                              h->kick_pending ? &h->kick_dt : nullptr, &kicked);
        if (kicked) h->kick_pending = false;
    }
    if (td.hot_cap > 0) HIP_TRY(h, hipMemcpyAsync(h->h_hot_info, h->d_hot_info, 2 * sizeof(int), hipMemcpyDeviceToHost, h->stream));
    HIP_TRY(h, hipGetLastError());
    return NBODY_OK;
}

int bh_forces(NbodyHandle* h) {
    {
        int rc = exchange_wait(h);
        if (rc) return rc;
    }
    h->last_step_async = false;
    if (h->cfg.tree_build == NBODY_TREE_DEVICE && !h->host_tree_once) {
        const bool plain_walk = h->cfg.math_mode == NBODY_MATH_STRICT || nbody::tuning().bh_walk_variant == 0;
        if (h->async_bh && plain_walk && !nbody::tuning().bh_walk_debug) return bh_walk_device_tree_async(h);
        int rc = resolve_async(h);
        if (rc) return rc;
// ... 51 lines not shown
                                       &work, nbody::tuning().bh_walk_variant == 3) != 0)
            return fail(h, NBODY_ERR_HIP, "device octree build: rocPRIM call failed");
        HIP_TRY(h, hipGetLastError());
        HIP_TRY(h, hipMemcpyAsync(tb.h_info, tb.d_info, 3 * sizeof(int), hipMemcpyDeviceToHost, h->stream));
        if (sharded)
            HIP_TRY(h, hipMemcpyAsync(h->h_counts, sh.seg_count, sizeof(int) * sh.n_seg, hipMemcpyDeviceToHost, h->stream));
        HIP_TRY(h, hipStreamSynchronize(h->stream));
        if (!sharded) h->h_counts[0] = tb.h_info[2];
        if (!(tb.h_info[1] & 2)) break;
        rc = ensure_tree_dev(h, size_t(tb.h_info[0]) + 64, tot_upper);
        if (rc) return rc;
    }
    for (int s = 0; s < sh.n_seg; ++s) h->seg_count_host[s] = h->h_counts[s];
    h->n_local = size_t(h->h_counts[sh.my_seg]);
    h->count_dirty = false;
    if (tb.h_info[1] & 5) { *fell_back = true; return NBODY_OK; }
    const int n_nodes = tb.h_info[0];
    const size_t n_order = h->n_local;
    const size_t n_tree = total_upper(h);
    const int* d_walk_order = h->d_order;
    if (sharded) {
        if (nbody::launch_tree_own_order(h->stream, h->d_order, cat, int(n_tree), tb.ws, nbody::tree_build_tmp_bytes(n_cap)) != 0)
            return fail(h, NBODY_ERR_HIP, "device octree build: rocPRIM call failed");
        d_walk_order = cat.own_order;
    }
    h->stats.tree_build_ms += ms_since(t1);
    h->stats.tree_nodes = uint64_t(n_nodes);
    h->tree_on_device = true;
    h->tree.n_nodes = size_t(n_nodes);

    const int K = walk_split_plan(n_order, h->cfg.math_mode != NBODY_MATH_STRICT || h->pot.walking, h->theta2, size_t(n_nodes)).segments;
    rc = h->split.ensure(h, K, size_t(sh.seg_cap));
    if (rc) return rc;
    if (n_tree > 0) h->split.list_on_device(h->stream, work, int(n_tree), n_nodes, K);
    nbody::TreeDev td;
    td.nodes = h->d_nodes; td.n_nodes = n_nodes;
    td.order = d_walk_order; td.n_order = int(n_order);
    walk_split_view(h->split, K, size_t(sh.seg_cap), &td);
    return walk_tree(h, td, n_tree);
}

int bh_walk_device_tree_async(NbodyHandle* h) {
    Shard& sh = h->sh;
    auto t1 = clk::now();
    TreeBuildBufs& tb = h->tree_bufs;
    int rc = tb.ensure(h, size_t(sh.seg_cap), 0);
    if (rc) return rc;
    const size_t n_upper = h->n_local;
    rc = ensure_tree_dev(h, std::max<size_t>(h->d_node_cap, 4 * n_upper + 64), n_upper);
    if (rc) return rc;
    if (h->pending.empty()) HIP_TRY(h, hipMemsetAsync(h->d_poison + 1, 0, sizeof(int), h->stream));
    const int K = walk_split_plan(n_upper, h->cfg.math_mode != NBODY_MATH_STRICT, h->theta2, n_upper).segments;
    rc = h->split.ensure(h, K, size_t(sh.seg_cap));
    if (rc) return rc;
    const nbody::TreeSplitReq req = h->split.request(K, tb.d_info, h->d_poison);
    nbody::TreeDevWork work;
    if (nbody::build_octree_device(h->stream, sh.own_pos(), sh.own_count(), int(n_upper), h->center, h->width, tb.ws, size_t(sh.seg_cap),
                                   h->d_nodes, int(h->d_node_cap), h->d_order, tb.d_info, &work, 0, n_upper > 0 ? &req : nullptr) != 0)
        return fail(h, NBODY_ERR_HIP, "device octree build: rocPRIM call failed");
    HIP_TRY(h, hipGetLastError());
    h->stats.tree_build_ms += ms_since(t1);
    h->tree_on_device = true;
    if (n_upper == 0)
        h->split.list_on_device(h->stream, work, 0, int(h->d_node_cap), K, tb.d_info, h->d_poison);
    nbody::TreeDev td;
    td.nodes = h->d_nodes; td.n_nodes = int(h->d_node_cap);
    td.order = h->d_order; td.n_order = int(n_upper);
    td.n_order_dev = tb.d_info + 2;
    td.poison = h->d_poison;
    walk_split_view(h->split, K, size_t(sh.seg_cap), &td);
    rc = walk_tree(h, td, n_upper);
    if (rc) return rc;
    h->last_step_async = true;
    h->count_dirty = true;
    return NBODY_OK;
}

int resolve_async(NbodyHandle* h) {
    if (!h->async_bh) return NBODY_OK;
    for (int round = 0; round < 1000000; ++round) {
        HIP_TRY(h, hipMemcpyAsync(h->h_poison, h->d_poison, 2 * sizeof(int), hipMemcpyDeviceToHost, h->stream));
        if (h->tree_bufs.d_info) HIP_TRY(h, hipMemcpyAsync(h->h_poison + 2, h->tree_bufs.d_info, 3 * sizeof(int), hipMemcpyDeviceToHost, h->stream));
        HIP_TRY(h, hipStreamSynchronize(h->stream));
        const int flags = h->h_poison[0], done = h->h_poison[1];
        if (!flags) {
            if (h->tree_on_device && h->tree_bufs.d_info) {
                h->tree.n_nodes = size_t(h->h_poison[2]);
                h->stats.tree_nodes = uint64_t(h->h_poison[2]);
            }
            h->pending.clear();
            return NBODY_OK;
        }
        std::vector<NbodyHandle::PendingStep> rest;
        if (size_t(done) < h->pending.size()) rest.assign(h->pending.begin() + done, h->pending.end());
        h->pending.clear();
        HIP_TRY(h, hipMemsetAsync(h->d_poison, 0, 2 * sizeof(int), h->stream));
        if (flags & 2) {
            int rc = ensure_tree_dev(h, 2 * h->d_node_cap + 64, h->n_local);
            if (rc) return rc;
        }
        if (rest.empty()) {
            h->host_tree_once = true;
            return NBODY_OK;
        }
        h->elapsed = rest[0].elapsed_before;
        h->stats.steps -= rest.size();
        h->host_tree_once = true;
        int rc = sync_count(h);
        if (rc) return rc;
        rc = step_end(h, rest[0].dt);
        if (rc) return rc;
        for (size_t k = 1; k < rest.size(); ++k) {
            rc = step_impl(h, rest[k].dt);
            if (rc) return rc;
        }
    }
    return fail(h, NBODY_ERR_INVALID, "resolve_async did not converge");
}

int partials_begin(NbodyHandle* h) {
    if (!(h->cross_on && h->tail_pending) || h->cross.parts.n + h->cross.n_recv == 0) return NBODY_OK;
    if (!h->comm_ready) return fail(h, NBODY_ERR_COMM, "world_size > 1 but nbody_comm_init has not been called");
    const nbody::CrossPlan& c = h->cross;
    const size_t S = h->sym_plan.plane_stride;
    const size_t bytes = size_t(h->sh.seg_cap) * sizeof(float4);
    HIP_TRY(h, hipEventRecord(h->ev_partials_ready, h->stream));
    HIP_TRY(h, hipStreamWaitEvent(h->comm_stream, h->ev_partials_ready, 0));
    TP_TRY(h, h->tp->group_begin());
    for (int i = 0; i < c.parts.n; ++i)
        TP_TRY(h, h->tp->send(h->d_send + size_t(i) * S, bytes, c.parts.seg[i], h->comm_stream));
    for (int i = 0; i < c.n_recv; ++i)
        TP_TRY(h, h->tp->recv(h->d_planes + size_t(h->recv_plane0 + i) * S, bytes, c.recv_from[i], h->comm_stream));
    TP_TRY(h, h->tp->group_end());
    HIP_TRY(h, hipEventRecord(h->ev_partials_done, h->comm_stream));
    h->partials_in_flight = true;
    return NBODY_OK;
}

int partials_wait(NbodyHandle* h) {
    if (!h->partials_in_flight) return NBODY_OK;
    HIP_TRY(h, hipStreamWaitEvent(h->stream, h->ev_partials_done, 0));
    h->partials_in_flight = false;
    return NBODY_OK;
}

int forces_begin(NbodyHandle* h) {
    return h->cfg.method == NBODY_BARNES_HUT ? bh_forces(h) : bf_forces(h);
}

int forces_finish(NbodyHandle* h) {
    if (!h->tail_pending) return NBODY_OK;
    h->tail_pending = false;
    const float eps2 = h->g_soft * h->g_soft;
    nbody::launch_bf_sym_tail(h->stream, h->sh, h->sym_plan, h->d_planes, int(h->n_local), h->g, eps2,
                              h->kick_pending ? &h->kick_dt : nullptr);
    h->kick_pending = false;
    HIP_TRY(h, hipGetLastError());
    return NBODY_OK;
}

int forces(NbodyHandle* h) {
    int rc = forces_begin(h);
    if (rc) return rc;
    rc = partials_begin(h);
    if (rc) return rc;
    rc = partials_wait(h);
    if (rc) return rc;
    return forces_finish(h);
}

int step_begin(NbodyHandle* h, float dt) {
    if (!h->bounds_set) return fail(h, NBODY_ERR_INVALID, "nbody_set_bounds has not been called");
    nbody::launch_drift_half(h->stream, h->sh, int(h->n_local), dt, h->bnd);
    nbody::launch_compact(h->stream, h->sh, int(h->n_local));
    h->count_dirty = true;
    HIP_TRY(h, hipGetLastError());
    return NBODY_OK;
}

int step_forces(NbodyHandle* h, float dt) {
    h->kick_pending = true;
    h->kick_dt = dt;
    int rc = forces_begin(h);
    if (rc) { h->kick_pending = false; h->tail_pending = false; }
    return rc;
}

int step_finish(NbodyHandle* h, float dt) {
    int rc = forces_finish(h);
    if (rc) { h->kick_pending = false; return rc; }
    if (h->kick_pending) nbody::launch_kick_drift(h->stream, h->sh, int(h->n_local), dt);
    h->kick_pending = false;
    HIP_TRY(h, hipGetLastError());
    if (h->ev_pending.size() >= 4096) {
        rc = drain_events(h);
        if (rc) return rc;
    }
    h->elapsed += dt;
    h->stats.steps += 1;
    return NBODY_OK;
}

int step_end(NbodyHandle* h, float dt) {
    int rc = step_forces(h, dt);
    if (rc) return rc;
    rc = partials_begin(h);
    if (rc) return rc;
    rc = partials_wait(h);
    if (rc) return rc;
    return step_finish(h, dt);
}

int step_impl(NbodyHandle* h, float dt) {
    const float elapsed_before = h->elapsed;
    int rc = step_begin(h, dt);
    if (rc) return rc;
    rc = exchange_begin(h);
    if (rc) return rc;
    rc = step_end(h, dt);
    if (rc) return rc;
    if (h->last_step_async) {
        h->pending.push_back(NbodyHandle::PendingStep{dt, elapsed_before});
        if (h->pending.size() >= 4096) rc = resolve_async(h);
    }
    return rc;
}

int spatial_walk(NbodyHandle* h, NbodyHandle* twin, int n_orig) {
    const int G = h->cfg.world_size, cap = h->sh.seg_cap;
    PotBufs& p = h->pot;
    int rc = nbody::let::potential_pass(twin);
    if (rc) return fail(h, rc, twin->err);
    rc = nbody::pot::begin(h, size_t(cap));
    if (!rc) rc = grow_dev(h, p.d_rec, p.rec_cap, size_t(G) * size_t(cap), sizeof(nbody::PotRec));
    const size_t n_ids = size_t(h->cfg.capacity) + 1;
    if (!rc) rc = grow_dev(h, p.d_slot_of, p.slot_cap, n_ids, sizeof(int));
    if (rc) return rc;
    if (!p.d_rec_count) HIP_TRY(h, hipMalloc(&p.d_rec_count, sizeof(int) * size_t(G)));
    HIP_TRY(h, hipStreamSynchronize(h->stream));
    hipStream_t ts = twin->stream;
    nbody::PotRec* rec = static_cast<nbody::PotRec*>(p.d_rec);
    nbody::launch_pot_pack(ts, twin->sh.ids, twin->pot.d_sum, twin->sh.own_count(), cap, rec + size_t(h->cfg.rank) * size_t(cap));
    HIP_TRY(h, hipMemcpyAsync(p.d_rec_count + h->cfg.rank, twin->sh.own_count(), sizeof(int), hipMemcpyDeviceToDevice, ts));
    if (twin->comm_ready) {
        TP_TRY(twin, twin->tp->group_begin());
        TP_TRY(twin, twin->tp->all_gather(rec, size_t(cap) * sizeof(nbody::PotRec), ts));
        TP_TRY(twin, twin->tp->all_gather(p.d_rec_count, sizeof(int), ts));
        TP_TRY(twin, twin->tp->group_end());
    }
    HIP_TRY(h, hipMemsetAsync(p.d_slot_of, 0xFF, n_ids * sizeof(int), ts));
    nbody::launch_pot_scatter(ts, h->sh.ids, h->sh.own_count(), n_orig, p.d_slot_of, int(std::min<size_t>(n_ids, 0x7fffffff)), rec, p.d_rec_count, G, cap, p.d_sum);
    HIP_TRY(h, hipMemcpyAsync(p.d_counts, twin->pot.d_counts, 2 * NBODY_WALK_COUNTER_SLOTS * sizeof(unsigned long long), hipMemcpyDeviceToDevice, ts));
    HIP_TRY(h, hipGetLastError());
    HIP_TRY(h, hipStreamSynchronize(ts));
    if (twin->tp) { rc = twin->tp->check(); if (rc) return fail(h, rc, twin->tp->error()); }
    return NBODY_OK;
}

int spatial_potentials(NbodyHandle* h, size_t* n_own, nbody::PotBodies* bodies, double* g) {
    if (!h->bounds_set) return fail(h, NBODY_ERR_INVALID, "nbody_set_bounds has not been called");
    if (h->cfg.world_size > 1 && !h->comm_ready) return fail(h, NBODY_ERR_COMM, "world_size > 1 but nbody_comm_init has not been called");
    const size_t saved_n = h->n_local;
    const bool saved_dirty = h->count_dirty;
    const std::vector<int> saved_counts = h->seg_count_host;
    NbodyHandle* twin = nullptr;
    int rc = nbody_clone(h, &twin);
    const int n_orig = int(h->n_local);
    h->n_local = saved_n; h->count_dirty = saved_dirty; h->seg_count_host = saved_counts;
    if (rc) return fail(h, rc, std::string("nbody_potentials: scratch clone: ") + nbody_last_error(nullptr));
    twin->tp = std::move(h->tp);
    twin->comm_ready = h->comm_ready;
    nbody::bind_tuning(&twin->tune);
    rc = spatial_walk(h, twin, n_orig);
    if (rc && !twin->err.empty()) h->err = twin->err;
    h->tp = std::move(twin->tp);
    twin->comm_ready = false;
    nbody::bind_tuning(&h->tune);
    free_all(twin);
    (void)hipSetDevice(h->device);
    if (rc) return rc;
    bodies->pos_all = h->sh.pos_all; bodies->vel = h->sh.vel; bodies->seg_count = h->sh.seg_count;
    bodies->f64 = 0; bodies->n_seg = 1; bodies->seg_cap = h->sh.seg_cap; bodies->my_seg = 0;
    bodies->world = h->comm_ready ? h->cfg.world_size : 1;
    *g = double(h->g);
    *n_own = size_t(n_orig);
    return NBODY_OK;
}

int potentials_device(NbodyHandle* h, int mode, size_t* n_own, nbody::PotBodies* bodies, double* g) {
    if (mode != NBODY_POTENTIAL_PAIRS && mode != NBODY_POTENTIAL_TREE) return fail(h, NBODY_ERR_INVALID, "mode must be NBODY_POTENTIAL_PAIRS or NBODY_POTENTIAL_TREE");
    if (h->let && mode == NBODY_POTENTIAL_PAIRS)
        return fail(h, NBODY_ERR_INVALID, "NBODY_POTENTIAL_PAIRS is not possible on NBODY_SHARD_SPATIAL handles (a rank does not hold the world's bodies): NBODY_POTENTIAL_TREE is the mode for them");
    if (h->let) return spatial_potentials(h, n_own, bodies, g);
    if (mode == NBODY_POTENTIAL_TREE && h->cfg.method != NBODY_BARNES_HUT) return fail(h, NBODY_ERR_INVALID, "NBODY_POTENTIAL_TREE needs a Barnes-Hut handle");
    if (h->f64) return nbody64::potentials_device(h, mode, n_own, bodies, g);
    if (mode == NBODY_POTENTIAL_TREE && !h->bounds_set) return fail(h, NBODY_ERR_INVALID, "nbody_set_bounds has not been called");
    Shard& sh = h->sh;
    int rc = resolve_async(h);
    if (!rc) rc = exchange_wait(h);
    if (rc) return rc;
    if (sh.n_seg > 1) {
        if (!h->comm_ready) return fail(h, NBODY_ERR_COMM, "world_size > 1 but nbody_comm_init has not been called");
        TP_TRY(h, h->tp->group_begin());
        TP_TRY(h, h->tp->all_gather(sh.pos_all, size_t(sh.seg_cap) * sizeof(float4), h->stream));
        TP_TRY(h, h->tp->all_gather(sh.seg_count, sizeof(int), h->stream));
        TP_TRY(h, h->tp->group_end());
    }
    const size_t saved_n = h->n_local;
// ... 30 lines not shown
    h->tp.reset();
    if (h->ev_drifted) (void)hipEventDestroy(h->ev_drifted);
    if (h->ev_gathered) (void)hipEventDestroy(h->ev_gathered);
    if (h->ev_partials_ready) (void)hipEventDestroy(h->ev_partials_ready);
    if (h->ev_partials_done) (void)hipEventDestroy(h->ev_partials_done);
    if (h->comm_stream) (void)hipStreamDestroy(h->comm_stream);
    for (auto& ev : h->ev_pending) { (void)hipEventDestroy(ev.first); (void)hipEventDestroy(ev.second); }
    for (auto& ev : h->ev_free) { (void)hipEventDestroy(ev.first); (void)hipEventDestroy(ev.second); }
    h->tree.clear();
    nbody64::destroy(h);
    nbody::let::destroy(h);
    void* dev[] = {h->sh.pos_all, h->sh.vel, h->sh.acc, h->sh.seg_count, h->sh.escaped, h->sh.keep, h->sh.tile_state, h->sh.epoch, h->sh.inter, h->d_poison, h->d_aos,
                   h->d_nodes, h->d_order, h->d_walk, h->d_unified, h->d_hot, h->d_hot_info, h->d_bfs, h->d_bfs_ws, h->d_nested_stack, h->d_counters, h->d_energy, h->d_sym_bounds, h->d_planes, h->d_cross_slices, h->d_xplanes, h->d_send};
    for (void* p : dev) if (p) (void)hipFree(p);
    void* host[] = {h->h_aos, h->h_pos, h->h_counts, h->h_counters, h->h_hot_info, h->h_poison};
    for (void* p : host) if (p) (void)hipHostFree(p);
    h->split.release();
    h->tree_bufs.release();
    h->pot.release();
    if (h->stream) (void)hipStreamDestroy(h->stream);
    delete h;
}

int create_impl(const NbodyConfig* cfg, NbodyHandle** out) {
    if (!cfg || !out) return fail(nullptr, NBODY_ERR_INVALID, "null argument");
    constexpr uint32_t kOldConfigSize = 48;
    NbodyConfig full{};
    if (cfg->struct_size == kOldConfigSize) { std::memcpy(&full, cfg, kOldConfigSize); full.struct_size = sizeof(NbodyConfig); cfg = &full; }
    if (cfg->struct_size != sizeof(NbodyConfig)) return fail(nullptr, NBODY_ERR_INVALID, "NbodyConfig.struct_size mismatch");
    if (cfg->shard_mode != NBODY_SHARD_INDEX && cfg->shard_mode != NBODY_SHARD_SPATIAL) return fail(nullptr, NBODY_ERR_INVALID, "unknown shard_mode");
    if (cfg->shard_mode == NBODY_SHARD_SPATIAL && (cfg->method != NBODY_BARNES_HUT || cfg->math_mode != NBODY_MATH_FAST || cfg->dtype != NBODY_F32))
        return fail(nullptr, NBODY_ERR_INVALID, "NBODY_SHARD_SPATIAL is the fast-math f32 Barnes-Hut path (halo exchange over the device-built tree)");
    if (cfg->method != NBODY_BRUTE_FORCE && cfg->method != NBODY_BARNES_HUT) return fail(nullptr, NBODY_ERR_INVALID, "unknown method");
    if (cfg->math_mode != NBODY_MATH_STRICT && cfg->math_mode != NBODY_MATH_FAST) return fail(nullptr, NBODY_ERR_INVALID, "unknown math_mode");
    if (cfg->leaf_mode != NBODY_LEAF_REFERENCE && cfg->leaf_mode != NBODY_LEAF_DIRECT) return fail(nullptr, NBODY_ERR_INVALID, "unknown leaf_mode");
    if (cfg->tree_build != NBODY_TREE_HOST && cfg->tree_build != NBODY_TREE_DEVICE && cfg->tree_build != NBODY_TREE_AUTO)
        return fail(nullptr, NBODY_ERR_INVALID, "unknown tree_build");
    if (cfg->world_size < 1 || cfg->rank < 0 || cfg->rank >= cfg->world_size) return fail(nullptr, NBODY_ERR_INVALID, "bad rank/world_size");
    if (cfg->capacity == 0 || cfg->capacity > (1ull << 30)) return fail(nullptr, NBODY_ERR_INVALID, "capacity must be in [1, 2^30]");
    if (cfg->dtype != NBODY_F32 && cfg->dtype != NBODY_F64) return fail(nullptr, NBODY_ERR_INVALID, "unknown dtype");
    if (cfg->dtype == NBODY_F64 && cfg->world_size != 1 && cfg->shard_mode != NBODY_SHARD_INDEX)
        return fail(nullptr, NBODY_ERR_INVALID, "f64 worlds are sharded by index blocks (NBODY_SHARD_INDEX)");

    int ndev = 0;
    if (hipGetDeviceCount(&ndev) != hipSuccess || ndev <= 0)
        return fail(nullptr, NBODY_ERR_NO_DEVICE, "no HIP device (this library has no CPU fallback)");
    int dev = cfg->device;
    if (dev < 0) {
        const char* lr = std::getenv("LOCAL_RANK");
        dev = lr ? std::atoi(lr) % ndev : 0;
    }
    if (dev >= ndev) return fail(nullptr, NBODY_ERR_INVALID, "device ordinal out of range");

    NbodyHandle* h = new NbodyHandle();
    h->cfg = *cfg;
    if (h->cfg.tree_build == NBODY_TREE_AUTO)
        h->cfg.tree_build = cfg->math_mode == NBODY_MATH_FAST ? NBODY_TREE_DEVICE : NBODY_TREE_HOST;
    if (h->cfg.dtype == NBODY_F64) {
        if (cfg->tree_build == NBODY_TREE_AUTO) h->cfg.tree_build = h->cfg.math_mode == NBODY_MATH_FAST ? NBODY_TREE_DEVICE : NBODY_TREE_HOST;
        if (cfg->world_size > 1 && h->cfg.math_mode != NBODY_MATH_FAST) h->cfg.tree_build = NBODY_TREE_HOST;
    }
    if (h->cfg.shard_mode == NBODY_SHARD_SPATIAL) h->cfg.tree_build = NBODY_TREE_DEVICE;
    cfg = &h->cfg;
    h->device = dev;
    *out = nullptr;
    auto bail = [&](int rc) { g_create_err = h->err; free_all(h); return rc; };
#define CREATE_TRY(expr)                                                                                  \
    do {                                                                                                  \
        hipError_t e_ = (expr);                                                                           \
        if (e_ != hipSuccess) { h->err = std::string(#expr) + ": " + hipGetErrorString(e_); return bail(NBODY_ERR_HIP); } \
    } while (0)
    CREATE_TRY(hipSetDevice(dev));
    CREATE_TRY(hipStreamCreateWithFlags(&h->stream, hipStreamNonBlocking));
    if (cfg->dtype == NBODY_F64) {
        CREATE_TRY(hipHostMalloc(&h->h_poison, 8 * sizeof(int), hipHostMallocDefault));
        if (cfg->method == NBODY_BARNES_HUT) {
            int threads = cfg->host_threads > 0 ? cfg->host_threads : std::min(16, std::max(1, int(std::thread::hardware_concurrency()) - 2));
            h->pool.reset(new nbody::WorkerPool(std::max(1, threads)));
            CREATE_TRY(hipMalloc(&h->d_counters, 2 * NBODY_WALK_COUNTER_SLOTS * sizeof(unsigned long long)));
            CREATE_TRY(hipMemsetAsync(h->d_counters, 0, 2 * NBODY_WALK_COUNTER_SLOTS * sizeof(unsigned long long), h->stream));
            CREATE_TRY(hipHostMalloc(&h->h_counters, 2 * NBODY_WALK_COUNTER_SLOTS * sizeof(unsigned long long), hipHostMallocDefault));
        }
        h->sh.n_seg = cfg->world_size; h->sh.my_seg = cfg->rank; h->sh.seg_cap = int((cfg->capacity + cfg->world_size - 1) / cfg->world_size);
        h->seg_count_host.assign(size_t(cfg->world_size), 0);
        int rc64 = nbody64::create(h);
        if (rc64) return bail(rc64);
        *out = h;
        return NBODY_OK;
    }
    Shard& sh = h->sh;
    sh.n_seg = cfg->world_size;
    sh.my_seg = cfg->rank;
    sh.seg_cap = int((cfg->capacity + cfg->world_size - 1) / cfg->world_size);
    const bool spatial = cfg->shard_mode == NBODY_SHARD_SPATIAL;
    if (spatial) {
        sh.n_seg = 1;
        sh.my_seg = 0;
        if (cfg->world_size > 1) sh.seg_cap = int(std::min<uint64_t>(cfg->capacity, 4 * uint64_t(sh.seg_cap) + 64));
    }
    const size_t cap = size_t(sh.seg_cap);
    CREATE_TRY(hipMalloc(&sh.pos_all, size_t(sh.n_seg) * cap * sizeof(float4)));
    CREATE_TRY(hipMalloc(&sh.vel, cap * sizeof(float4)));
    CREATE_TRY(hipMalloc(&sh.acc, cap * sizeof(float4)));
    CREATE_TRY(hipMalloc(&sh.seg_count, sizeof(int) * sh.n_seg));
    CREATE_TRY(hipMalloc(&sh.escaped, sizeof(int)));
    CREATE_TRY(hipMalloc(&sh.keep, cap));
    CREATE_TRY(hipMemsetAsync(sh.pos_all, 0, size_t(sh.n_seg) * cap * sizeof(float4), h->stream));
    CREATE_TRY(hipMemsetAsync(sh.vel, 0, cap * sizeof(float4), h->stream));
    CREATE_TRY(hipMemsetAsync(sh.acc, 0, cap * sizeof(float4), h->stream));
    CREATE_TRY(hipMemsetAsync(sh.seg_count, 0, sizeof(int) * sh.n_seg, h->stream));
    CREATE_TRY(hipMemsetAsync(sh.escaped, 0, sizeof(int), h->stream));
    CREATE_TRY(hipMemsetAsync(sh.keep, 1, cap, h->stream));
    {
        const size_t tiles = (cap + 1023) / 1024 + 1;
        CREATE_TRY(hipMalloc(&sh.tile_state, tiles * sizeof(unsigned long long)));
        CREATE_TRY(hipMemsetAsync(sh.tile_state, 0, tiles * sizeof(unsigned long long), h->stream));
        CREATE_TRY(hipMalloc(&sh.epoch, sizeof(int)));
        CREATE_TRY(hipMemsetAsync(sh.epoch, 0, sizeof(int), h->stream));
        CREATE_TRY(hipMemsetAsync(sh.epoch, 1, 1, h->stream));
        CREATE_TRY(hipMalloc(&sh.inter, sizeof(unsigned long long)));
        CREATE_TRY(hipMemsetAsync(sh.inter, 0, sizeof(unsigned long long), h->stream));
        CREATE_TRY(hipMalloc(&h->d_poison, 2 * sizeof(int)));
        CREATE_TRY(hipMemsetAsync(h->d_poison, 0, 2 * sizeof(int), h->stream));
        CREATE_TRY(hipHostMalloc(&h->h_poison, 8 * sizeof(int), hipHostMallocDefault));
    }
    CREATE_TRY(hipHostMalloc(&h->h_counts, sizeof(int) * sh.n_seg, hipHostMallocDefault));
    h->seg_count_host.assign(sh.n_seg, 0);
    if (cfg->method == NBODY_BARNES_HUT) {
        int threads = cfg->host_threads > 0 ? cfg->host_threads : std::min(16, std::max(1, int(std::thread::hardware_concurrency()) - 2));
        if (threads < 1) threads = 1;
        h->pool.reset(new nbody::WorkerPool(threads));
        h->tree.alloc = pinned_alloc;
        h->tree.release = pinned_free;
        CREATE_TRY(hipHostMalloc(&h->h_pos, size_t(sh.n_seg) * cap * sizeof(float4), hipHostMallocDefault));
        CREATE_TRY(hipMalloc(&h->d_counters, 2 * NBODY_WALK_COUNTER_SLOTS * sizeof(unsigned long long)));
        CREATE_TRY(hipMemsetAsync(h->d_counters, 0, 2 * NBODY_WALK_COUNTER_SLOTS * sizeof(unsigned long long), h->stream));
        CREATE_TRY(hipHostMalloc(&h->h_counters, 2 * NBODY_WALK_COUNTER_SLOTS * sizeof(unsigned long long), hipHostMallocDefault));
    }
    CREATE_TRY(hipStreamSynchronize(h->stream));
#undef CREATE_TRY
    {
        const char* v = std::getenv("NBODY_BH_ASYNC");
        h->async_bh = cfg->method == NBODY_BARNES_HUT && cfg->tree_build == NBODY_TREE_DEVICE && cfg->world_size == 1 &&
                      !spatial && !(v && v[0] == '0');
        if (h->async_bh) sh.poison = h->d_poison;
    }
    if (spatial) {
        int rc_let = nbody::let::create(h);
        if (rc_let) return bail(rc_let);
    }
    {
        nbody::Tuning& t = h->tune;
        const struct { const char* env; int* knob; } table[] = {
            {"NBODY_BF_VARIANT", &t.bf_fast_variant}, {"NBODY_CROSS_SYM", &t.cross_sym}, {"NBODY_SYM_PACKED", &t.sym_packed},
            {"NBODY_BH_SPLIT", &t.bh_walk_split}, {"NBODY_SYM_WPB", &t.sym_wpb}, {"NBODY_SYM_IPT", &t.sym_ipt}, {"NBODY_BH_DUO", &t.bh_walk_duo}, {"NBODY_BH_XCD", &t.bh_walk_xcd},
#ifdef NBODY_TUNING
            {"NBODY_BH_VARIANT", &t.bh_walk_variant}, {"NBODY_BH_HOT", &t.bh_hot_cap}, {"NBODY_BH_LDS_BLOCK", &t.bh_walk_lds_block},
#endif
        };
        for (const auto& e : table)
            if (const char* v = std::getenv(e.env)) *e.knob = std::atoi(v);
    }
    *out = h;
    return NBODY_OK;
}

}

extern "C" {

int nbody_abi_version(void) { return NBODY_ABI_VERSION; }

int nbody_device_count(void) {
    int n = 0;
    if (hipGetDeviceCount(&n) != hipSuccess) return 0;
    return n;
}

const char* nbody_last_error(const NbodyHandle* h) { return h ? h->err.c_str() : g_create_err.c_str(); }

int nbody_create(const NbodyConfig* cfg, NbodyHandle** out) { return create_impl(cfg, out); }

void nbody_destroy(NbodyHandle* h) { free_all(h); }

int nbody_clone(const NbodyHandle* src, NbodyHandle** out) {
    if (!src || !out) return fail(nullptr, NBODY_ERR_INVALID, "null argument");
    NbodyHandle* s = const_cast<NbodyHandle*>(src);
    int rc = use_device(s);
    if (rc) return rc;
    rc = resolve_async(s);
    if (rc) return rc;
    if (!s->f64) rc = sync_count(s);
    if (rc) return rc;
    NbodyHandle* h = nullptr;
    rc = create_impl(&src->cfg, &h);
    if (rc) return rc;
    if (src->f64) {
        rc = nbody64::clone_state(s, h);
        if (rc) { g_create_err = h->err; free_all(h); return rc; }
        *out = h;
        return NBODY_OK;
    }
    const Shard& a = src->sh;
    const size_t cap = size_t(a.seg_cap);
    hipError_t e = hipStreamSynchronize(s->stream);
    if (e == hipSuccess) e = hipMemcpyAsync(h->sh.pos_all, a.pos_all, size_t(a.n_seg) * cap * sizeof(float4), hipMemcpyDeviceToDevice, h->stream);
    if (e == hipSuccess) e = hipMemcpyAsync(h->sh.vel, a.vel, cap * sizeof(float4), hipMemcpyDeviceToDevice, h->stream);
    if (e == hipSuccess) e = hipMemcpyAsync(h->sh.acc, a.acc, cap * sizeof(float4), hipMemcpyDeviceToDevice, h->stream);
    if (e == hipSuccess) e = hipMemcpyAsync(h->sh.seg_count, a.seg_count, sizeof(int) * a.n_seg, hipMemcpyDeviceToDevice, h->stream);
    if (e == hipSuccess) e = hipStreamSynchronize(h->stream);
    if (e != hipSuccess) {
        g_create_err = std::string("clone copy: ") + hipGetErrorString(e);
        free_all(h);
        return NBODY_ERR_HIP;
    }
    h->g = src->g; h->g_soft = src->g_soft; h->dt = src->dt; h->theta2 = src->theta2;
    h->tune = src->tune;
    std::memcpy(h->center, src->center, sizeof(h->center));
    h->width = src->width; h->bnd = src->bnd; h->bounds_set = src->bounds_set;
    h->elapsed = src->elapsed;
    h->n_local = src->n_local;
    h->seg_count_host = src->seg_count_host;
    h->first_global = src->first_global; h->n_at_upload = src->n_at_upload;
    if (src->let) {
        rc = nbody::let::clone_state(s, h);
        if (rc) { g_create_err = h->err; free_all(h); return rc; }
    }
    *out = h;
    return NBODY_OK;
}

int nbody_upload(NbodyHandle* h, const void* aos, size_t n, size_t stride) {
    if (!h || (!aos && n)) return fail(h, NBODY_ERR_INVALID, "null argument");
    if (stride < 40 || stride % 4) return fail(h, NBODY_ERR_INVALID, "stride must be a multiple of 4 and >= 40 bytes");
    if (n > h->cfg.capacity) return fail(h, NBODY_ERR_CAPACITY, "more bodies than NbodyConfig.capacity");
    int rc = use_device(h);
    if (rc) return rc;
    if (h->f64) return (n && !aos) ? NBODY_ERR_INVALID : nbody64::upload(h, aos, n, stride);
    if (h->let) return nbody::let::upload(h, aos, n, stride);
    rc = resolve_async(h);
    if (rc) return rc;
    Shard& sh = h->sh;
    const size_t G = size_t(sh.n_seg);
    const size_t blk = (n + G - 1) / G;
    rc = ensure_aos(h, n);
    if (rc) return rc;
    const char* src = static_cast<const char*>(aos);
    for (size_t k = 0; k < n; ++k) std::memcpy(h->h_aos + 10 * k, src + k * stride, 40);
    if (n) HIP_TRY(h, hipMemcpyAsync(h->d_aos, h->h_aos, n * 40, hipMemcpyHostToDevice, h->stream));
    for (size_t s = 0; s < G; ++s) {
        size_t lo = std::min(n, s * blk), hi = std::min(n, lo + blk);
        h->seg_count_host[s] = int(hi - lo);
        bool own = int(s) == sh.my_seg;
        nbody::launch_aos_to_soa(h->stream, h->d_aos + 10 * lo, 10, int(hi - lo), sh.pos_all + s * size_t(sh.seg_cap),
                                 own ? sh.vel : nullptr, own ? sh.acc : nullptr);
        if (own) { h->first_global = lo; h->n_at_upload = hi - lo; h->n_local = hi - lo; }
    }
    HIP_TRY(h, hipGetLastError());
    HIP_TRY(h, hipMemsetAsync(sh.escaped, 0, sizeof(int), h->stream));
    h->count_dirty = false;
    return push_counts(h);
}

int nbody_download(NbodyHandle* h, void* aos, size_t cap, size_t stride, size_t* n_out) {
    if (!h) return NBODY_ERR_INVALID;
    if (stride < 40 || stride % 4) return fail(h, NBODY_ERR_INVALID, "stride must be a multiple of 4 and >= 40 bytes");
    int rc = use_device(h);
    if (rc) return rc;
    if (h->f64) return nbody64::download(h, aos, cap, stride, n_out);
    rc = resolve_async(h);
    if (rc) return rc;
    rc = sync_count(h);
    if (rc) return rc;
    const size_t n = h->n_local;
    if (n_out) *n_out = n;
    if (n > cap) return fail(h, NBODY_ERR_CAPACITY, "download buffer too small");
    if (n == 0) return NBODY_OK;
    if (!aos) return fail(h, NBODY_ERR_INVALID, "null buffer");
    rc = ensure_aos(h, n);
    if (rc) return rc;
    nbody::launch_soa_to_aos(h->stream, h->d_aos, 10, int(n), h->sh.own_pos(), h->sh.vel, h->sh.acc);
    HIP_TRY(h, hipGetLastError());
    HIP_TRY(h, hipMemcpyAsync(h->h_aos, h->d_aos, n * 40, hipMemcpyDeviceToHost, h->stream));
    HIP_TRY(h, hipStreamSynchronize(h->stream));
    rc = comm_check(h);
    if (rc) return rc;
    char* dst = static_cast<char*>(aos);
    for (size_t k = 0; k < n; ++k) std::memcpy(dst + k * stride, h->h_aos + 10 * k, 40);
    return NBODY_OK;
}

int nbody_count(NbodyHandle* h, size_t* n_out) {
    if (!h || !n_out) return NBODY_ERR_INVALID;
    int rc = use_device(h);
    if (rc) return rc;
    if (h->f64) return nbody64::count(h, n_out);
    rc = resolve_async(h);
    if (rc) return rc;
    rc = sync_count(h);
    if (rc) return rc;
    *n_out = h->n_local;
    return NBODY_OK;
}

int nbody_count_global(NbodyHandle* h, size_t* n_out) {
    if (!h || !n_out) return NBODY_ERR_INVALID;
    int rc = use_device(h);
    if (rc) return rc;
    if (h->f64) return nbody64::count_global(h, n_out);
    if (h->let) return nbody::let::count_global(h, n_out);
    rc = resolve_async(h);
    if (rc) return rc;
    rc = sync_count(h);
    if (rc) return rc;
    *n_out = total_upper(h);
    return NBODY_OK;
}

int nbody_add_point(NbodyHandle* h, const void* particle) {
    if (!h || !particle) return NBODY_ERR_INVALID;
    int rc = use_device(h);
    if (rc) return rc;
    if (h->f64) return nbody64::add_point(h, particle);
    if (h->let) return nbody::let::add_point(h, particle);
    if (h->sh.n_seg != 1) return sharded_add_point(h, particle);
    rc = resolve_async(h);
    if (rc) return rc;
    rc = sync_count(h);
    if (rc) return rc;
    if (h->n_local >= size_t(h->sh.seg_cap)) return fail(h, NBODY_ERR_CAPACITY, "capacity exhausted");
    const float* p = static_cast<const float*>(particle);
    float4 rec[3] = {make_float4(p[0], p[1], p[2], p[9]), make_float4(p[3], p[4], p[5], 0.f), make_float4(p[6], p[7], p[8], 0.f)};
    const size_t k = h->n_local;
    HIP_TRY(h, hipMemcpyAsync(h->sh.pos_all + k, &rec[0], sizeof(float4), hipMemcpyHostToDevice, h->stream));
    HIP_TRY(h, hipMemcpyAsync(h->sh.vel + k, &rec[1], sizeof(float4), hipMemcpyHostToDevice, h->stream));
    HIP_TRY(h, hipMemcpyAsync(h->sh.acc + k, &rec[2], sizeof(float4), hipMemcpyHostToDevice, h->stream));
    HIP_TRY(h, hipStreamSynchronize(h->stream));
    h->n_local = k + 1;
    h->seg_count_host[0] = int(h->n_local);
    return push_counts(h);
}

int nbody_remove_point(NbodyHandle* h, size_t index) {
    if (!h) return NBODY_ERR_INVALID;
    int rc = use_device(h);
    if (rc) return rc;
    if (h->f64) return nbody64::remove_point(h, index);
    if (h->let) return nbody::let::remove_point(h, index);
    if (h->sh.n_seg != 1) return sharded_remove_point(h, index);
    rc = resolve_async(h);
    if (rc) return rc;
    rc = sync_count(h);
    if (rc) return rc;
    if (index >= h->n_local) return fail(h, NBODY_ERR_INVALID, "swap_remove index out of range");
    const size_t last = h->n_local - 1;
    if (index != last) {
        HIP_TRY(h, hipMemcpyAsync(h->sh.pos_all + index, h->sh.pos_all + last, sizeof(float4), hipMemcpyDeviceToDevice, h->stream));
        HIP_TRY(h, hipMemcpyAsync(h->sh.vel + index, h->sh.vel + last, sizeof(float4), hipMemcpyDeviceToDevice, h->stream));
        HIP_TRY(h, hipMemcpyAsync(h->sh.acc + index, h->sh.acc + last, sizeof(float4), hipMemcpyDeviceToDevice, h->stream));
    }
    h->n_local = last;
    h->seg_count_host[0] = int(last);
    return push_counts(h);
}

int nbody_set_settings(NbodyHandle* h, float g, float g_soft, float dt, float theta2) {
    if (!h) return NBODY_ERR_INVALID;
    if (h->f64) return nbody64::set_settings(h, double(g), double(g_soft), double(dt), double(theta2));
    h->g = g; h->g_soft = g_soft; h->dt = dt; h->theta2 = theta2;
    return NBODY_OK;
}

int nbody_get_settings(const NbodyHandle* h, float* g, float* g_soft, float* dt, float* theta2) {
    if (!h) return NBODY_ERR_INVALID;
    if (h->f64) {
        double a, b, c, d;
        nbody64::get_settings(h, &a, &b, &c, &d);
        if (g) *g = float(a);
        if (g_soft) *g_soft = float(b);
        if (dt) *dt = float(c);
        if (theta2) *theta2 = float(d);
        return NBODY_OK;
    }
    if (g) *g = h->g;
    if (g_soft) *g_soft = h->g_soft;
    if (dt) *dt = h->dt;
    if (theta2) *theta2 = h->theta2;
    return NBODY_OK;
}

int nbody_set_settings_f64(NbodyHandle* h, double g, double g_soft, double dt, double theta2) {
    if (!h) return NBODY_ERR_INVALID;
    if (h->f64) return nbody64::set_settings(h, g, g_soft, dt, theta2);
    return nbody_set_settings(h, float(g), float(g_soft), float(dt), float(theta2));
}

int nbody_get_settings_f64(const NbodyHandle* h, double* g, double* g_soft, double* dt, double* theta2) {
    if (!h) return NBODY_ERR_INVALID;
    if (h->f64) return nbody64::get_settings(h, g, g_soft, dt, theta2);
    if (g) *g = double(h->g);
    if (g_soft) *g_soft = double(h->g_soft);
    if (dt) *dt = double(h->dt);
    if (theta2) *theta2 = double(h->theta2);
    return NBODY_OK;
}

int nbody_set_bounds_f64(NbodyHandle* h, const double center[3], double width) {
    if (!h || !center) return NBODY_ERR_INVALID;
    if (h->f64) return nbody64::set_bounds(h, center, width);
    const float c[3] = {float(center[0]), float(center[1]), float(center[2])};
    return nbody_set_bounds(h, c, float(width));
}

int nbody_set_bounds(NbodyHandle* h, const float center[3], float width) {
    if (!h || !center) return NBODY_ERR_INVALID;
    if (h->f64) {
        const double c[3] = {double(center[0]), double(center[1]), double(center[2])};
        return nbody64::set_bounds(h, c, double(width));
    }
    std::memcpy(h->center, center, sizeof(h->center));
    h->width = width;
    compute_bounds(h);
    h->bounds_set = true;
    return NBODY_OK;
}

int nbody_init(NbodyHandle* h) {
    if (!h) return NBODY_ERR_INVALID;
    if (h->f64) return nbody64::init(h);
    h->elapsed = 0.f;
    return NBODY_OK;
}

int nbody_step_by(NbodyHandle* h, float dt) {
    if (!h) return NBODY_ERR_INVALID;
    int rc = use_device(h);
    if (rc) return rc;
    if (h->f64) return nbody64::step_by(h, double(dt));
    if (h->let) return nbody::let::step(h, dt);
    return step_impl(h, dt);
}

int nbody_step_by_f64(NbodyHandle* h, double dt) {
    if (!h) return NBODY_ERR_INVALID;
    int rc = use_device(h);
    if (rc) return rc;
    if (h->f64) return nbody64::step_by(h, dt);
    if (h->let) return nbody::let::step(h, float(dt));
    return step_impl(h, float(dt));
}

int nbody_steps(NbodyHandle* h, int k) {
    if (!h || k < 0) return NBODY_ERR_INVALID;
    int rc = use_device(h);
    if (rc) return rc;
    if (h->f64) return nbody64::steps(h, k);
    if (h->let) {
        for (int i = 0; i < k; ++i) { rc = nbody::let::step(h, h->dt); if (rc) return rc; }
        return NBODY_OK;
    }
    for (int i = 0; i < k; ++i) {
        rc = step_impl(h, h->dt);
        if (rc) return rc;
    }
    return NBODY_OK;
}

int nbody_update_forces(NbodyHandle* h) {
    if (!h) return NBODY_ERR_INVALID;
    int rc = use_device(h);
    if (rc) return rc;
    if (h->f64) return nbody64::update_forces(h);
    if (h->let) return h->bounds_set ? nbody::let::update_forces(h) : fail(h, NBODY_ERR_INVALID, "nbody_set_bounds has not been called");
    if (h->cfg.method == NBODY_BARNES_HUT && !h->bounds_set) return fail(h, NBODY_ERR_INVALID, "nbody_set_bounds has not been called");
    rc = resolve_async(h);
    if (rc) return rc;
    rc = exchange_begin(h);
    if (rc) return rc;
    rc = forces(h);
    if (rc || !h->last_step_async) return rc;
    h->last_step_async = false;
    rc = resolve_async(h);
    if (rc || !h->host_tree_once) return rc;
    return forces(h);
}

int nbody_elapsed(const NbodyHandle* h, float* out) {
    if (!h || !out) return NBODY_ERR_INVALID;
    *out = h->f64 ? float(nbody64::elapsed(h)) : h->elapsed;
    return NBODY_OK;
}

// ... 151 lines not shown
        h->tree.reserve(n, 0);
        HIP_TRY(h, hipMemcpyAsync(h->tree.nodes, h->d_nodes, n * sizeof(nbody::NodeRec), hipMemcpyDeviceToHost, h->stream));
        HIP_TRY(h, hipStreamSynchronize(h->stream));
    }
    if (n > cap) return fail(h, NBODY_ERR_CAPACITY, "tree export buffer too small");
    for (size_t i = 0; i < n; ++i) {
        const nbody::NodeRec& r = h->tree.nodes[i];
        if (com_mass) { com_mass[4 * i] = r.a.x; com_mass[4 * i + 1] = r.a.y; com_mass[4 * i + 2] = r.a.z; com_mass[4 * i + 3] = r.a.m; }
        if (width) width[i] = std::sqrt(r.b.w2);
        if (skip) skip[i] = r.b.skip;
    }
    return NBODY_OK;
}

int nbody_tree_export_f64(NbodyHandle* h, double* com_mass, double* width, int32_t* skip, size_t cap, size_t* n_nodes) {
    if (!h) return NBODY_ERR_INVALID;
    if (h->cfg.method != NBODY_BARNES_HUT) return fail(h, NBODY_ERR_INVALID, "not a Barnes-Hut handle");
    if (!h->f64) return fail(h, NBODY_ERR_INVALID, "f32 handle: use nbody_tree_export");
    return nbody64::tree_export(h, com_mass, width, skip, cap, n_nodes);
}

extern "C++" {
namespace {
template <class F>
void cells_from_preorder(const F* com_mass, const int32_t* skip, size_t n, const F root_center[3], F root_width, float* min_max6, int32_t* depth) {
    struct Open { size_t end; F c[3]; F half; int depth; };
    std::vector<Open> stack;
    for (size_t i = 0; i < n; ++i) {
        while (!stack.empty() && stack.back().end <= i) stack.pop_back();
        Open me;
        me.end = size_t(skip[i]);
        if (stack.empty()) {
            for (int k = 0; k < 3; ++k) me.c[k] = root_center[k];
            me.half = root_width * F(0.5);
            me.depth = 0;
        } else {
            const Open& p = stack.back();
            me.half = p.half * F(0.5);
            for (int k = 0; k < 3; ++k) me.c[k] = com_mass[4 * i + k] > p.c[k] ? p.c[k] + me.half : p.c[k] - me.half;
            me.depth = p.depth + 1;
        }
        if (min_max6)
            for (int k = 0; k < 3; ++k) {
                min_max6[6 * i + k] = float(me.c[k] + (-me.half));
                min_max6[6 * i + 3 + k] = float(me.c[k] + me.half);
            }
        if (depth) depth[i] = me.depth;
        if (me.end > i + 1) stack.push_back(me);
    }
}
}
}

int nbody_tree_export_cells(NbodyHandle* h, float* min_max6, int32_t* depth, size_t cap, size_t* n_nodes) {
    if (!h) return NBODY_ERR_INVALID;
    size_t n = 0;
    if (h->f64) {
        int rc = nbody_tree_export_f64(h, nullptr, nullptr, nullptr, 0, &n);
        if (rc) return rc;
        if (n_nodes) *n_nodes = n;
        if (!min_max6 && !depth) return NBODY_OK;
        if (n > cap) return fail(h, NBODY_ERR_CAPACITY, "tree export buffer too small");
        std::vector<double> cm(4 * n), w(n);
        std::vector<int32_t> sk(n);
        rc = nbody_tree_export_f64(h, cm.data(), w.data(), sk.data(), n, &n);
        if (rc) return rc;
        double c[3], width;
        nbody64::get_bounds(h, c, &width);
        cells_from_preorder<double>(cm.data(), sk.data(), n, c, width, min_max6, depth);
        return NBODY_OK;
    }
    int rc = nbody_tree_export(h, nullptr, nullptr, nullptr, 0, &n);
    if (rc) return rc;
    if (n_nodes) *n_nodes = n;
    if (!min_max6 && !depth) return NBODY_OK;
    if (n > cap) return fail(h, NBODY_ERR_CAPACITY, "tree export buffer too small");
    std::vector<float> cm(4 * n), w(n);
    std::vector<int32_t> sk(n);
    rc = nbody_tree_export(h, cm.data(), w.data(), sk.data(), n, &n);
    if (rc) return rc;
    cells_from_preorder<float>(cm.data(), sk.data(), n, h->center, h->width, min_max6, depth);
    return NBODY_OK;
}

int nbody_comm_unique_id(void* id_bytes) {
    if (!id_bytes) return NBODY_ERR_INVALID;
    const char* v = std::getenv("NBODY_TRANSPORT");
    std::string err;
    int rc = nbody::transport_make_id((v && std::strcmp(v, "ipc") == 0) ? nbody::kTransportIpc : nbody::kTransportRccl, id_bytes, &err);
    return rc ? fail(nullptr, rc, err) : NBODY_OK;
}

int nbody_comm_local_id(void* id_bytes) {
    if (!id_bytes) return NBODY_ERR_INVALID;
    std::string err;
    int rc = nbody::transport_make_id(nbody::kTransportIpc, id_bytes, &err);
    return rc ? fail(nullptr, rc, err) : NBODY_OK;
}

struct Agreement {
    int32_t abi, method, math_mode, leaf_mode, tree_build, dtype, shard_mode, world, seg_cap;
    int32_t cross_sym, sym_packed, bf_variant, walk_variant, walk_split;
    uint64_t capacity;
};
static const char* const kAgreementFields[] = {"ABI version", "method", "math_mode", "leaf_mode", "tree_build", "dtype", "shard_mode", "world_size",
                                               "shard capacity", "NBODY_CROSS_SYM", "NBODY_SYM_PACKED", "NBODY_BF_VARIANT", "NBODY_BH_VARIANT",
                                               "NBODY_BH_SPLIT"};

int nbody_comm_init(NbodyHandle* h, const void* id_bytes) {
    if (!h || !id_bytes) return NBODY_ERR_INVALID;
    int rc = use_device(h);
    if (rc) return rc;
    h->comm_ready = false;
    h->tp.reset();
    {
        std::string err;
        int code = NBODY_ERR_COMM;
        h->tp.reset(nbody::transport_create(id_bytes, h->cfg.rank, h->cfg.world_size, h->device, &err, &code));
        if (!h->tp) return fail(h, code, err);
    }
    if (!h->comm_stream) {
        HIP_TRY(h, hipStreamCreateWithFlags(&h->comm_stream, hipStreamNonBlocking));
        HIP_TRY(h, hipEventCreateWithFlags(&h->ev_drifted, hipEventDisableTiming));
        HIP_TRY(h, hipEventCreateWithFlags(&h->ev_gathered, hipEventDisableTiming));
        HIP_TRY(h, hipEventCreateWithFlags(&h->ev_partials_ready, hipEventDisableTiming));
        HIP_TRY(h, hipEventCreateWithFlags(&h->ev_partials_done, hipEventDisableTiming));
    }
    Agreement mine{NBODY_ABI_VERSION, h->cfg.method, h->cfg.math_mode, h->cfg.leaf_mode, h->cfg.tree_build, h->cfg.dtype, h->cfg.shard_mode,
                   h->cfg.world_size, h->sh.seg_cap, nbody::tuning().cross_sym, nbody::tuning().sym_packed, nbody::tuning().bf_fast_variant, nbody::tuning().bh_walk_variant,
                   nbody::tuning().bh_walk_split, h->cfg.capacity};
    std::vector<Agreement> all(size_t(h->cfg.world_size));
    TP_TRY(h, h->tp->host_all_gather(&mine, all.data(), sizeof(Agreement)));
    for (int r = 0; r < h->cfg.world_size; ++r) {
        const int32_t* a = reinterpret_cast<const int32_t*>(&all[size_t(r)]);
        const int32_t* m = reinterpret_cast<const int32_t*>(&mine);
        for (size_t f = 0; f < sizeof(kAgreementFields) / sizeof(kAgreementFields[0]); ++f)
            if (a[f] != m[f]) {
                h->tp.reset();
                return fail(h, NBODY_ERR_COMM, std::string("nbody_comm_init: rank ") + std::to_string(r) + " and rank " + std::to_string(h->cfg.rank) + " disagree on " +
                                                   kAgreementFields[f] + " (" + std::to_string(a[f]) + " vs " + std::to_string(m[f]) + "): every rank of a world must be created alike");
            }
        if (all[size_t(r)].capacity != mine.capacity) {
            h->tp.reset();
            return fail(h, NBODY_ERR_COMM, "nbody_comm_init: ranks disagree on NbodyConfig.capacity");
        }
    }
    h->comm_ready = true;
    return NBODY_OK;
}

namespace {
struct Knob { const char* name; int nbody::Tuning::*field; bool tuning_build_only; };
const Knob kKnobs[] = {
    {"cross_sym", &nbody::Tuning::cross_sym, false}, {"sym_packed", &nbody::Tuning::sym_packed, false},
    {"bf_fast_variant", &nbody::Tuning::bf_fast_variant, false}, {"sym_wpb", &nbody::Tuning::sym_wpb, false}, {"sym_ipt", &nbody::Tuning::sym_ipt, false}, {"let_list_div", &nbody::Tuning::let_list_div, false}, {"bh_walk_duo", &nbody::Tuning::bh_walk_duo, false}, {"bh_walk_xcd", &nbody::Tuning::bh_walk_xcd, false},
    {"sym_rounds", &nbody::Tuning::sym_rounds, false}, {"sym_k", &nbody::Tuning::sym_k, false},
    {"sym_min_bodies", &nbody::Tuning::sym_min_bodies, false}, {"sym_reduce_split", &nbody::Tuning::sym_reduce_split, false},
    {"cross_slots", &nbody::Tuning::cross_slots, false}, {"cross_ipt", &nbody::Tuning::cross_ipt, false},
    {"cross_wpb", &nbody::Tuning::cross_wpb, false}, {"bh_walk_split", &nbody::Tuning::bh_walk_split, false},
    {"bh_walk_order", &nbody::Tuning::bh_walk_order, false}, {"bh_reduce_split", &nbody::Tuning::bh_reduce_split, false},
    {"tree_max_tie", &nbody::Tuning::tree_max_tie, false},
    {"bf64_min_bodies", &nbody::Tuning::bf64_min_bodies, false}, {"bf64_ipt", &nbody::Tuning::bf64_ipt, false},
    {"bf64_rot", &nbody::Tuning::bf64_rot, false}, {"bf64_waves", &nbody::Tuning::bf64_waves, false},
    {"bh_walk_variant", &nbody::Tuning::bh_walk_variant, true}, {"bh_walk_lds_block", &nbody::Tuning::bh_walk_lds_block, true},
    {"bh_hot_cap", &nbody::Tuning::bh_hot_cap, true}, {"bh_walk_debug", &nbody::Tuning::bh_walk_debug, true},
    {"sym_debug", &nbody::Tuning::sym_debug, true},
};
}

int nbody_set_tuning(NbodyHandle* h, const char* name, int value) {
    if (!h || !name) return NBODY_ERR_INVALID;
    for (const Knob& k : kKnobs)
        if (std::strcmp(k.name, name) == 0) {
#ifndef NBODY_TUNING
            if (k.tuning_build_only && value != nbody::Tuning{}.*(k.field))
                return fail(h, NBODY_ERR_INVALID, std::string("nbody_set_tuning: '") + name + "' selects code only the tuning build carries (make -C nbody-llm_amd/csrc tuning)");
#endif
            if (h->comm_ready && (std::strcmp(name, "cross_sym") == 0 || std::strcmp(name, "sym_packed") == 0 || std::strcmp(name, "bf_fast_variant") == 0))
                return fail(h, NBODY_ERR_INVALID, std::string("nbody_set_tuning: '") + name + "' is part of what the ranks agreed on at nbody_comm_init: set it before");
            h->tune.*(k.field) = value;
            return NBODY_OK;
        }
    return fail(h, NBODY_ERR_INVALID, std::string("nbody_set_tuning: unknown knob '") + name + "'");
}

int nbody_get_tuning(const NbodyHandle* h, const char* name, int* value) {
    if (!h || !name || !value) return NBODY_ERR_INVALID;
    for (const Knob& k : kKnobs)
        if (std::strcmp(k.name, name) == 0) { *value = h->tune.*(k.field); return NBODY_OK; }
    return NBODY_ERR_INVALID;
}

int nbody_get_config(const NbodyHandle* h, NbodyConfig* out) {
    if (!h || !out) return NBODY_ERR_INVALID;
    *out = h->cfg;
    return NBODY_OK;
}

int nbody_is_tuning_build(void) {
#ifdef NBODY_TUNING
    return 1;
#else
    return 0;
#endif
}

int nbody_comm_transport(const NbodyHandle* h, char* out, size_t cap) {
    if (!h || !out || cap == 0) return NBODY_ERR_INVALID;
    std::snprintf(out, cap, "%s", h->tp ? h->tp->name() : "none");
    return NBODY_OK;
}

int nbody_download_ids(NbodyHandle* h, int32_t* ids, size_t cap, size_t* n_out) {
    if (!h) return NBODY_ERR_INVALID;
    int rc = use_device(h);
    if (rc) return rc;
    if (!h->let) return fail(h, NBODY_ERR_INVALID, "nbody_download_ids is for NBODY_SHARD_SPATIAL handles (index-block shards: nbody_local_range)");
    return nbody::let::download_ids(h, ids, cap, n_out);
}

int nbody_let_stats(NbodyHandle* h, NbodyLetStats* out) {
    if (!h || !out) return NBODY_ERR_INVALID;
    if (!h->let) return fail(h, NBODY_ERR_INVALID, "not an NBODY_SHARD_SPATIAL handle");
    return nbody::let::stats(h, out);
}

int nbody_debug_let_phase(NbodyHandle* h, int phase, float dt) {
    if (!h) return NBODY_ERR_INVALID;
    int rc = use_device(h);
    if (rc) return rc;
    if (!h->let) return fail(h, NBODY_ERR_INVALID, "not an NBODY_SHARD_SPATIAL handle");
    return nbody::let::debug_phase(h, phase, dt);
}

int nbody_debug_let_exchange(NbodyHandle* h, NbodyHandle* peer, int which) {
    if (!h || !peer) return NBODY_ERR_INVALID;
    int rc = use_device(h);
    if (rc) return rc;
    if (!h->let || !peer->let) return fail(h, NBODY_ERR_INVALID, "not an NBODY_SHARD_SPATIAL handle");
    return nbody::let::debug_exchange(h, peer, which);
}

int nbody_debug_let_set_prune(NbodyHandle* h, int prune);

int nbody_local_range(const NbodyHandle* h, size_t* first, size_t* count) {
    if (!h) return NBODY_ERR_INVALID;
    if (first) *first = h->first_global;
    if (count) *count = h->n_at_upload;
    return NBODY_OK;
}

int nbody_debug_step_begin(NbodyHandle* h, float dt) {
    if (!h) return NBODY_ERR_INVALID;
    if (h->f64) return fail(h, NBODY_ERR_INVALID, "f64 handles are single-shard");
    int rc = use_device(h);
    return rc ? rc : step_begin(h, dt);
}

int nbody_debug_import_segment(NbodyHandle* h, NbodyHandle* peer) {
    if (!h || !peer) return NBODY_ERR_INVALID;
    if (h->f64 || peer->f64) return fail(h, NBODY_ERR_INVALID, "f64 handles are single-shard");
    if (h->sh.n_seg != peer->sh.n_seg || h->sh.seg_cap != peer->sh.seg_cap) return fail(h, NBODY_ERR_INVALID, "peer has a different sharding");
    int rc = use_device(h);
    if (rc) return rc;
    const int s = peer->sh.my_seg;
    HIP_TRY(h, hipStreamSynchronize(peer->stream));
    HIP_TRY(h, hipMemcpyAsync(h->sh.pos_all + size_t(s) * h->sh.seg_cap, peer->sh.own_pos(), size_t(h->sh.seg_cap) * sizeof(float4), hipMemcpyDeviceToDevice, h->stream));
    HIP_TRY(h, hipMemcpyAsync(h->sh.seg_count + s, peer->sh.own_count(), sizeof(int), hipMemcpyDeviceToDevice, h->stream));
    HIP_TRY(h, hipStreamSynchronize(h->stream));
    h->count_dirty = true;
    return NBODY_OK;
}

int nbody_debug_step_forces(NbodyHandle* h, float dt) {
    if (!h) return NBODY_ERR_INVALID;
    if (h->f64) return fail(h, NBODY_ERR_INVALID, "f64 handles are single-shard");
    int rc = use_device(h);
    return rc ? rc : step_forces(h, dt);
}

int nbody_debug_import_partials(NbodyHandle* h, NbodyHandle* peer) {
    if (!h || !peer) return NBODY_ERR_INVALID;
    if (h->f64 || peer->f64) return fail(h, NBODY_ERR_INVALID, "f64 handles are single-shard");
    int rc = use_device(h);
    if (rc) return rc;
    if (!(h->cross_on && h->tail_pending)) return NBODY_OK;
    if (!(peer->cross_on && peer->tail_pending)) return fail(h, NBODY_ERR_INVALID, "peer is not in the same phase");
    int src = -1, dst = -1;
    for (int i = 0; i < peer->cross.parts.n; ++i) if (peer->cross.parts.seg[i] == h->sh.my_seg) src = i;
    for (int i = 0; i < h->cross.n_recv; ++i) if (h->cross.recv_from[i] == peer->sh.my_seg) dst = i;
    if ((src < 0) != (dst < 0)) return fail(h, NBODY_ERR_INVALID, "send/receive plans of the two shards do not match");
    if (src < 0) return NBODY_OK;
    HIP_TRY(h, hipStreamSynchronize(peer->stream));
    HIP_TRY(h, hipMemcpyAsync(h->d_planes + size_t(h->recv_plane0 + dst) * h->sym_plan.plane_stride,
                              peer->d_send + size_t(src) * peer->sym_plan.plane_stride,
                              size_t(h->sh.seg_cap) * sizeof(float4), hipMemcpyDeviceToDevice, h->stream));
    HIP_TRY(h, hipStreamSynchronize(h->stream));
    return NBODY_OK;
}

int nbody_debug_step_end(NbodyHandle* h, float dt) {
    if (!h) return NBODY_ERR_INVALID;
    if (h->f64) return fail(h, NBODY_ERR_INVALID, "f64 handles are single-shard");
    int rc = use_device(h);
    return rc ? rc : step_finish(h, dt);
}

int nbody_host_cross_plan(int rank, int world, int seg_cap, int n_own, int* ipt, int* n_sets, int* n_parts, int* parts,
                          int* n_recv, int* recv_from) {
    if (world < 2 || rank < 0 || rank >= world || seg_cap <= 0 || n_own < 0 || n_own > seg_cap) return NBODY_ERR_INVALID;
    if (world > 2 * (nbody::CrossPartners::kMax - 1)) return NBODY_ERR_INVALID;
    const nbody::CrossPlan p = nbody::make_cross_plan(rank, world, seg_cap, n_own);
    if (ipt) *ipt = p.ipt;
    if (n_sets) *n_sets = p.A;
    if (n_parts) *n_parts = p.parts.n;
    if (parts)
        for (int i = 0; i < p.parts.n; ++i) {
            parts[5 * i + 0] = p.parts.seg[i]; parts[5 * i + 1] = p.parts.c0[i]; parts[5 * i + 2] = p.parts.c1[i];
            parts[5 * i + 3] = p.parts.a0[i]; parts[5 * i + 4] = p.parts.a1[i];
        }
    if (n_recv) *n_recv = p.n_recv;
    if (recv_from) for (int i = 0; i < p.n_recv; ++i) recv_from[i] = p.recv_from[i];
    return NBODY_OK;
}

int nbody_host_launch_plan(size_t n_bodies, float theta2, int fast_math, int out[3]) {
    if (!out) return NBODY_ERR_INVALID;
    nbody::bind_tuning(nullptr);
    const nbody::WalkPlan p = nbody::walk_plan(n_bodies, fast_math != 0, nbody::kMaxSplit, theta2);
    out[0] = p.bodies_per_lane; out[1] = p.segments; out[2] = nbody::sym_bodies_per_lane(n_bodies);
    return NBODY_OK;
}

int nbody_host_exchange_layout(const int* matrix, int world, int rank, long long clamp, int packed_send, size_t send_stride,
                               size_t* out_at, size_t* n_out, size_t* in_at, size_t* n_in, size_t* total_in) {
    if (!matrix || world < 1 || world > 16 || rank < 0 || rank >= world || !out_at || !n_out || !in_at || !n_in) return NBODY_ERR_INVALID;
    const size_t t = nbody::let::exchange_layout(matrix, world, rank, clamp, packed_send != 0, send_stride, out_at, n_out, in_at, n_in);
    if (total_in) *total_in = t;
    return NBODY_OK;
}

int nbody_host_build_tree(const float* pos4, size_t n, const float center[3], float width, int threads,
                          float* com_mass, float* node_width, int32_t* skip, int32_t* leaf_body, int32_t* order,
                          size_t cap, size_t* n_nodes) {
    if ((!pos4 && n) || !center || !n_nodes) return NBODY_ERR_INVALID;
    if (n > (1ull << 30)) return NBODY_ERR_INVALID;
    static thread_local std::unique_ptr<nbody::WorkerPool> tl_pool;
    static thread_local int tl_threads = 0;
// ... 24 lines not shown
```

nbody-llm_amd/csrc/nbody_handle.h:

```cpp
#pragma once
#include "../../include/nbody_hip.h"
#include "kernels.h"
#include "kernels_f64.h"
#include "octree_host.h"

#include "transport.h"

#include <hip/hip_runtime.h>

#include <chrono>
#include <memory>
#include <string>
#include <utility>
#include <vector>

using nbody::BoundsF;
using nbody::Shard;

namespace nbody64 { struct State; }
namespace nbody { namespace let { struct State; } }
struct NbodyHandle;


int fail(NbodyHandle* h, int code, const std::string& msg);
// ... 83 lines not shown
        nbody::TreeSplitReq r;
        r.n_split = K; r.first = first(); r.n_anc = n_anc(); r.anc = anc(); r.max_anc = nbody::kMaxAnc; r.info = info; r.poison = poison;
        return r;
    }
    void release() {
        if (d) (void)hipFree(d);
        if (h) (void)hipHostFree(h);
        if (planes) (void)hipFree(planes);
        d = h = nullptr; planes = nullptr; planes_cap = 0;
    }
};

inline void walk_split_view(const WalkSplitBuf<float4>& b, int K, size_t stride, nbody::TreeDev* td) {
    td->n_split = K;
    td->split_first = b.first(); td->split_n_anc = b.n_anc(); td->split_anc = b.anc();
    if (K > 1) { td->split_planes = b.planes; td->split_stride = stride; }
}
inline nbody64::WalkSplit64 walk_split_view(const WalkSplitBuf<double4>& b, int K, size_t stride) {
    return nbody64::WalkSplit64{K, b.first(), b.anc(), b.n_anc(), b.planes, stride};
}

struct TreeBuildBufs {
    void* ws = nullptr;
    void* cat = nullptr;
    size_t cap = 0;
    int* d_info = nullptr;
    int* h_info = nullptr;

    int ensure(NbodyHandle* hh, size_t n_cap, size_t cat_bytes) {
        if (cap < n_cap) {
            if (ws) (void)hipFree(ws);
            if (cat) (void)hipFree(cat);
            ws = nullptr; cat = nullptr; cap = 0;
            HIP_TRY(hh, hipMalloc(&ws, nbody::tree_build_workspace_bytes(n_cap)));
            if (cat_bytes) HIP_TRY(hh, hipMalloc(&cat, cat_bytes));
            cap = n_cap;
        }
        if (!d_info) {
            HIP_TRY(hh, hipMalloc(&d_info, 4 * sizeof(int)));
            HIP_TRY(hh, hipHostMalloc(&h_info, 4 * sizeof(int), hipHostMallocDefault));
        }
        return NBODY_OK;
    }
    void release() {
        for (void* p : {ws, cat, static_cast<void*>(d_info)}) if (p) (void)hipFree(p);
        if (h_info) (void)hipHostFree(h_info);
        *this = TreeBuildBufs{};
    }
};

struct PotBufs {
    bool walking = false;
    double* d_sum = nullptr;
    size_t sum_cap = 0;
    double* d_planes = nullptr;
    size_t planes_cap = 0;
    unsigned long long* d_counts = nullptr;
    unsigned long long* h_counts = nullptr;
    double* d_part = nullptr;
    size_t part_blocks = 0;
    void* d_rec = nullptr;
    size_t rec_cap = 0;
    int* d_rec_count = nullptr;
    int* d_slot_of = nullptr;
    size_t slot_cap = 0;
    void release() {
        for (void* p : {static_cast<void*>(d_sum), static_cast<void*>(d_planes), static_cast<void*>(d_counts), static_cast<void*>(d_part), d_rec,
                        static_cast<void*>(d_rec_count), static_cast<void*>(d_slot_of)})
            if (p) (void)hipFree(p);
        if (h_counts) (void)hipHostFree(h_counts);
        *this = PotBufs{};
    }
};

struct PotWalkScope {
    PotBufs& p;
    explicit PotWalkScope(PotBufs& pb) : p(pb) { p.walking = true; }
    ~PotWalkScope() { p.walking = false; }
    PotWalkScope(const PotWalkScope&) = delete;
    PotWalkScope& operator=(const PotWalkScope&) = delete;
};

struct NbodyHandle {
    NbodyConfig cfg{};
    nbody::Tuning tune;
    int device = 0;
    hipStream_t stream = nullptr;
    Shard sh;
    float g = 1.0f, g_soft = 0.0f, dt = 1e-3f, theta2 = 0.5f;
    float center[3] = {0.f, 0.f, 0.f};
    float width = 0.f;
    BoundsF bnd{};
    bool bounds_set = false;
    float elapsed = 0.f;

    size_t n_local = 0;
    bool count_dirty = false;
    std::vector<int> seg_count_host;
    size_t first_global = 0, n_at_upload = 0;

    float* d_aos = nullptr;
    float* h_aos = nullptr;
    size_t aos_cap = 0;

    std::unique_ptr<nbody::WorkerPool> pool;
    nbody::HostTree tree;
    nbody::BuildScratch tree_scratch;
    float4* d_nodes = nullptr;
    int* d_order = nullptr;
    size_t d_node_cap = 0, d_order_cap = 0;
    float* h_pos = nullptr;
    int* h_counts = nullptr;
    std::vector<int32_t> own_order;
    TreeBuildBufs tree_bufs;
    float4* d_nested_stack = nullptr;
    size_t nested_cap = 0;
    int nested_levels = 0;
    bool tree_on_device = false;
    WalkSplitBuf<float4> split;
    float4* d_walk = nullptr;
    int* d_unified = nullptr;
    size_t walk_cap = 0;
    float4* d_bfs = nullptr;
    void* d_bfs_ws = nullptr;
    size_t bfs_cap = 0;
    float4* d_hot = nullptr;
    int hot_cap = 0;
    int* d_hot_info = nullptr;
    int* h_hot_info = nullptr;
    int hot_threshold = 0;
    size_t hot_threshold_n = 0;
    unsigned long long* d_counters = nullptr;
    unsigned long long* h_counters = nullptr;

    nbody::SymPlan sym_plan;
    int* d_sym_bounds = nullptr;
    float4* d_planes = nullptr;
    size_t planes_cap = 0;
    int sym_waves = 0;
    nbody::CrossPlan cross;
    bool cross_on = false;
    int4* d_cross_slices = nullptr;
    size_t cross_slices_cap = 0;
    float4* d_xplanes = nullptr;
    float4* d_send = nullptr;
    size_t xplanes_cap = 0, send_cap = 0;
    int recv_plane0 = 0;
    bool tail_pending = false;
    bool partials_in_flight = false;
    hipEvent_t ev_partials_ready = nullptr, ev_partials_done = nullptr;
    bool kick_pending = false;
    float kick_dt = 0.f;
    uint64_t sym_pairs = 0;
    size_t sym_pairs_n = 0;

    bool async_bh = false;
    struct PendingStep { float dt; float elapsed_before; };
    std::vector<PendingStep> pending;
    bool last_step_async = false;
    bool host_tree_once = false;
    int* d_poison = nullptr;
    int* h_poison = nullptr;

    NbodyStats stats{};
    bool profiling = false;
    int profile_every = 1;
    unsigned profile_tick = 0;
    bool timed_this = false;
    std::vector<std::pair<hipEvent_t, hipEvent_t>> ev_pending, ev_free;
    double* d_energy = nullptr;
    size_t energy_blocks = 0;
    PotBufs pot;

    std::unique_ptr<nbody::Transport> tp;
    bool comm_ready = false;
    hipStream_t comm_stream = nullptr;
    hipEvent_t ev_drifted = nullptr, ev_gathered = nullptr;
    bool exchange_in_flight = false;

    nbody64::State* f64 = nullptr;
    nbody::let::State* let = nullptr;

    std::string err;
};



template <class T>
int grow_dev(NbodyHandle* h, T*& p, size_t& cap, size_t n, size_t elem_bytes) {
    if (n <= cap) return NBODY_OK;
    if (p) (void)hipFree(p);
    p = nullptr; cap = 0;
    const size_t want = n + n / 4 + 1024;
    HIP_TRY(h, hipMalloc(reinterpret_cast<void**>(&p), want * elem_bytes));
    cap = want;
    return NBODY_OK;
}

struct ForceTimer {
    NbodyHandle* h;
    std::pair<hipEvent_t, hipEvent_t> ev{nullptr, nullptr};
    explicit ForceTimer(NbodyHandle* hh) : h(hh) {
        h->timed_this = false;
        if (!h->profiling) return;
        if (h->profile_every > 1 && (h->profile_tick++ % unsigned(h->profile_every)) != 0) return;
        h->timed_this = true;
        if (!h->ev_free.empty()) { ev = h->ev_free.back(); h->ev_free.pop_back(); }
        else {
            if (hipEventCreate(&ev.first) != hipSuccess || hipEventCreate(&ev.second) != hipSuccess) { ev = {nullptr, nullptr}; return; }
        }
        (void)hipEventRecord(ev.first, h->stream);
    }
    ~ForceTimer() {
        if (!ev.first) return;
        (void)hipEventRecord(ev.second, h->stream);
        h->ev_pending.push_back(ev);
    }
};

template <class F, class NodeDev>
struct HostTreePass {
    const F* pos_all;
    const int* seg_count;
    int n_seg, seg_cap, my_seg;
    F* h_pos;
    int* h_counts;
    std::vector<int>& count_host;
    size_t& n_local;
    bool& count_dirty;
    const F* center;
    F width;
    nbody::HostTreeT<F>& tree;
    nbody::BuildScratchT<F>& scratch;
    std::vector<int32_t>& own_order;
    NodeDev*& d_nodes;
    size_t& node_cap;
    int*& d_order;
    size_t& order_cap;
    size_t n_order = 0;

    int run(NbodyHandle* h) {
        auto t0 = clk::now();
        for (int g = 0; g < n_seg; ++g) {
            const size_t cnt = size_t(count_host[size_t(g)]);
            if (cnt)
                HIP_TRY(h, hipMemcpyAsync(h_pos + 4 * size_t(g) * seg_cap, pos_all + 4 * size_t(g) * seg_cap, cnt * 4 * sizeof(F),
                                          hipMemcpyDeviceToHost, h->stream));
        }
        HIP_TRY(h, hipMemcpyAsync(h_counts, seg_count, sizeof(int) * n_seg, hipMemcpyDeviceToHost, h->stream));
        HIP_TRY(h, hipStreamSynchronize(h->stream));
        for (int g = 0; g < n_seg; ++g) count_host[size_t(g)] = h_counts[g];
        n_local = size_t(h_counts[my_seg]);
        count_dirty = false;
        const double copy_ms = ms_since(t0);

        auto t1 = clk::now();
        nbody::build_octree<F>(h_pos, n_seg, seg_cap, h_counts, center, width, *h->pool, scratch, tree);
        if (tree.too_deep) return fail(h, NBODY_ERR_TREE_DEPTH, "octree deeper than NBODY_MAX_TREE_DEPTH (coincident bodies?)");
        const int32_t* order = tree.order;
        n_order = tree.n_order;
        if (n_seg > 1) {
            own_order.clear();
            const int lo = my_seg * seg_cap, hi = lo + seg_cap;
            for (size_t k = 0; k < tree.n_order; ++k) {
                const int id = tree.order[k];
                if (id >= lo && id < hi) own_order.push_back(id - lo);
            }
            order = own_order.data();
            n_order = own_order.size();
        }
        h->stats.tree_build_ms += ms_since(t1);
        h->stats.tree_nodes = tree.n_nodes;

        auto t2 = clk::now();
        int rc = grow_dev(h, d_nodes, node_cap, tree.n_nodes, sizeof(nbody::NodeRecT<F>));
        if (!rc) rc = grow_dev(h, d_order, order_cap, n_order, sizeof(int));
        if (rc) return rc;
        HIP_TRY(h, hipMemcpyAsync(d_nodes, tree.nodes, tree.n_nodes * sizeof(nbody::NodeRecT<F>), hipMemcpyHostToDevice, h->stream));
        if (n_order) HIP_TRY(h, hipMemcpyAsync(d_order, order, n_order * sizeof(int), hipMemcpyHostToDevice, h->stream));
        if (n_seg > 1) HIP_TRY(h, hipStreamSynchronize(h->stream));
        h->stats.tree_copy_ms += copy_ms + ms_since(t2);
        return NBODY_OK;
    }
};
```

nbody-llm_amd/rust/src/lib.rs:

```rust
#![feature(generic_const_exprs)]
#![allow(incomplete_features)]

use std::cell::{Cell, UnsafeCell};
use std::ffi::{c_char, c_int, c_void, CStr};

use nlib::shared::{AABB, Bounds, Float, Integrator, LeapFrogIntegrator, Particle, PointParticle, Simulation, SimulationSettings};

#[cfg(feature = "render")]
use nlib::render::{BufferWrapper, Context, PipelineType, Renderable, Renderer};

#[repr(C)]
struct NbodyConfig {
    struct_size: u32,
    method: i32,
    math_mode: i32,
    leaf_mode: i32,
    device: i32,
    rank: i32,
    world_size: i32,
    host_threads: i32,
    capacity: u64,
    tree_build: i32,
    dtype: i32,
    shard_mode: i32,
    reserved: i32,
}

#[repr(C)]
pub struct NbodyHandle {
    _private: [u8; 0],
}

unsafe extern "C" {
    fn nbody_create(cfg: *const NbodyConfig, out: *mut *mut NbodyHandle) -> c_int;
    fn nbody_destroy(h: *mut NbodyHandle);
    fn nbody_clone(h: *const NbodyHandle, out: *mut *mut NbodyHandle) -> c_int;
    fn nbody_upload(h: *mut NbodyHandle, aos: *const c_void, n: usize, stride: usize) -> c_int;
    fn nbody_download(h: *mut NbodyHandle, aos: *mut c_void, cap: usize, stride: usize, n_out: *mut usize) -> c_int;
    fn nbody_count(h: *mut NbodyHandle, n_out: *mut usize) -> c_int;
    fn nbody_add_point(h: *mut NbodyHandle, particle: *const c_void) -> c_int;
    fn nbody_remove_point(h: *mut NbodyHandle, index: usize) -> c_int;
    fn nbody_set_settings(h: *mut NbodyHandle, g: f32, g_soft: f32, dt: f32, theta2: f32) -> c_int;
    fn nbody_set_settings_f64(h: *mut NbodyHandle, g: f64, g_soft: f64, dt: f64, theta2: f64) -> c_int;
    fn nbody_set_bounds(h: *mut NbodyHandle, center: *const f32, width: f32) -> c_int;
    fn nbody_set_bounds_f64(h: *mut NbodyHandle, center: *const f64, width: f64) -> c_int;
    fn nbody_init(h: *mut NbodyHandle) -> c_int;
    fn nbody_step_by(h: *mut NbodyHandle, dt: f32) -> c_int;
    fn nbody_step_by_f64(h: *mut NbodyHandle, dt: f64) -> c_int;
    fn nbody_steps(h: *mut NbodyHandle, k: c_int) -> c_int;
    fn nbody_update_forces(h: *mut NbodyHandle) -> c_int;
    fn nbody_sync(h: *mut NbodyHandle) -> c_int;
    fn nbody_tree_export_cells(h: *mut NbodyHandle, min_max6: *mut f32, depth: *mut i32, cap: usize, n_nodes: *mut usize) -> c_int;
    fn nbody_set_tuning(h: *mut NbodyHandle, name: *const c_char, value: c_int) -> c_int;
    fn nbody_last_error(h: *const NbodyHandle) -> *const c_char;
}

pub const NBODY_BRUTE_FORCE: i32 = 0;
pub const NBODY_BARNES_HUT: i32 = 1;

#[derive(Debug, Clone, Copy, PartialEq, Eq)]
pub enum MathMode {
    Strict = 0,
    Fast = 1,
}

#[derive(Debug, Clone, Copy, PartialEq, Eq)]
pub enum LeafMode {
    Reference = 0,
    Direct = 1,
}

#[derive(Debug, Clone, Copy, PartialEq, Eq)]
pub enum TreeBuild {
    Host = 0,
    Device = 1,
    Auto = 2,
}

#[derive(Debug, Clone, Copy)]
pub struct HipOptions {
    pub math_mode: MathMode,
    pub leaf_mode: LeafMode,
    pub tree_build: TreeBuild,
    pub host_threads: i32,
    pub device: i32,
    pub capacity: usize,
}

impl Default for HipOptions {
    fn default() -> Self {
        Self { math_mode: MathMode::Fast, leaf_mode: LeafMode::Reference, tree_build: TreeBuild::Auto, host_threads: 0, device: -1, capacity: 0 }
    }
}

mod sealed {
    pub trait Sealed {}
    impl Sealed for f32 {}
    impl Sealed for f64 {}
}

pub trait HipFloat: Float + sealed::Sealed {
    const DTYPE: i32;
    unsafe fn abi_set_settings(h: *mut NbodyHandle, s: &SimulationSettings<Self>) -> c_int;
    unsafe fn abi_set_bounds(h: *mut NbodyHandle, center: [Self; 3], width: Self) -> c_int;
    unsafe fn abi_step_by(h: *mut NbodyHandle, dt: Self) -> c_int;
}

impl HipFloat for f32 {
    const DTYPE: i32 = 0;
    unsafe fn abi_set_settings(h: *mut NbodyHandle, s: &SimulationSettings<f32>) -> c_int {
        unsafe { nbody_set_settings(h, s.g, s.g_soft, s.dt, s.theta2) }
    }
    unsafe fn abi_set_bounds(h: *mut NbodyHandle, center: [f32; 3], width: f32) -> c_int {
        unsafe { nbody_set_bounds(h, center.as_ptr(), width) }
    }
    unsafe fn abi_step_by(h: *mut NbodyHandle, dt: f32) -> c_int {
        unsafe { nbody_step_by(h, dt) }
    }
}

impl HipFloat for f64 {
    const DTYPE: i32 = 1;
    unsafe fn abi_set_settings(h: *mut NbodyHandle, s: &SimulationSettings<f64>) -> c_int {
        unsafe { nbody_set_settings_f64(h, s.g, s.g_soft, s.dt, s.theta2) }
    }
    unsafe fn abi_set_bounds(h: *mut NbodyHandle, center: [f64; 3], width: f64) -> c_int {
        unsafe { nbody_set_bounds_f64(h, center.as_ptr(), width) }
    }
    unsafe fn abi_step_by(h: *mut NbodyHandle, dt: f64) -> c_int {
        unsafe { nbody_step_by_f64(h, dt) }
    }
}

type P<F> = PointParticle<F, 3>;
type I<F> = LeapFrogIntegrator<F, 3, P<F>>;

pub struct HipSimulation<F: HipFloat, const METHOD: i32> {
    handle: *mut NbodyHandle,
    points: UnsafeCell<Vec<P<F>>>,
    dirty: Cell<bool>,
    integrator: I<F>,
    bounds: Bounds<F, 3>,
    settings: SimulationSettings<F>,
    settings_dirty: bool,
    elapsed: F,
    options: HipOptions,
    #[cfg(feature = "render")]
    points_buffer: Option<BufferWrapper>,
    #[cfg(feature = "render")]
    bounds_buffer: Option<BufferWrapper>,
    #[cfg(feature = "render")]
    vertex_scratch: Vec<f32>,
    #[cfg(feature = "render")]
    cell_scratch: (Vec<f32>, Vec<i32>),
}

pub type HipBruteForceSimulation<F> = HipSimulation<F, NBODY_BRUTE_FORCE>;
pub type HipBarnesHutSimulation<F> = HipSimulation<F, NBODY_BARNES_HUT>;

fn last_error(h: *const NbodyHandle) -> String {
    unsafe { CStr::from_ptr(nbody_last_error(h)) }.to_string_lossy().into_owned()
}

impl<F: HipFloat, const METHOD: i32> HipSimulation<F, METHOD> {
    fn check(&self, rc: c_int) {
        if rc != 0 {
            panic!("nbody_hip error {rc}: {}", last_error(self.handle));
        }
    }

    fn push_settings(&mut self) {
        if self.settings_dirty {
            let rc = unsafe { F::abi_set_settings(self.handle, &self.settings) };
            self.check(rc);
            self.settings_dirty = false;
        }
    }

    fn create(points: &[P<F>], bounds: &Bounds<F, 3>, o: &HipOptions) -> *mut NbodyHandle {
        let cfg = NbodyConfig {
            struct_size: std::mem::size_of::<NbodyConfig>() as u32,
            method: METHOD,
            math_mode: o.math_mode as i32,
            leaf_mode: o.leaf_mode as i32,
            device: o.device,
            rank: 0,
            world_size: 1,
            host_threads: o.host_threads,
            capacity: if o.capacity > 0 { o.capacity as u64 } else { (points.len().max(1) * 2) as u64 },
            tree_build: o.tree_build as i32,
            dtype: F::DTYPE,
            shard_mode: 0,
            reserved: 0,
        };
        let mut h: *mut NbodyHandle = std::ptr::null_mut();
        let rc = unsafe { nbody_create(&cfg, &mut h) };
        if rc != 0 {
            panic!("nbody_create failed ({rc}): {}", last_error(std::ptr::null()));
        }
        let c = bounds.center();
        let rc = unsafe { F::abi_set_bounds(h, [c[0], c[1], c[2]], bounds.width) };
        assert_eq!(rc, 0, "nbody_set_bounds: {}", last_error(h));
        let rc = unsafe { nbody_upload(h, points.as_ptr() as *const c_void, points.len(), std::mem::size_of::<P<F>>()) };
        assert_eq!(rc, 0, "nbody_upload: {}", last_error(h));
        h
    }

    pub fn with_options(points: Vec<P<F>>, integrator: I<F>, bounds: Bounds<F, 3>, options: HipOptions) -> Self {
        let handle = Self::create(&points, &bounds, &options);
        Self {
            handle,
            points: UnsafeCell::new(points),
            dirty: Cell::new(false),
            integrator,
            bounds,
            settings: SimulationSettings::default(),
            settings_dirty: true,
            elapsed: F::from(0.0).unwrap(),
            options,
            #[cfg(feature = "render")]
            points_buffer: None,
            #[cfg(feature = "render")]
            bounds_buffer: None,
            #[cfg(feature = "render")]
            vertex_scratch: Vec::new(),
            #[cfg(feature = "render")]
            cell_scratch: (Vec::new(), Vec::new()),
        }
    }

    pub fn set_tuning(&mut self, name: &str, value: i32) {
        let c = std::ffi::CString::new(name).expect("knob names have no interior NUL");
        let rc = unsafe { nbody_set_tuning(self.handle, c.as_ptr(), value) };
        self.check(rc);
    }

    pub fn steps(&mut self, k: usize) {
        self.push_settings();
        let rc = unsafe { nbody_steps(self.handle, k as c_int) };
        self.check(rc);
        let dt = self.settings.dt;
        for _ in 0..k {
            self.elapsed += dt;
        }
        self.dirty.set(true);
    }

    pub fn step_by_with<J: Integrator<F, 3, P<F>>>(&mut self, integrator: &mut J, dt: F) {
        self.push_settings();
        let mut pts: Vec<P<F>> = self.get_points().clone();
        integrator.integrate_pre_force(&mut pts, dt);
        let bounds = self.bounds;
        pts.retain(|p| bounds.contains(p.position()));
        self.upload_points(&pts);
        let rc = unsafe { nbody_update_forces(self.handle) };
        self.check(rc);
        self.dirty.set(true);
        let mut pts: Vec<P<F>> = self.get_points().clone();
        integrator.integrate_after_force(&mut pts, dt);
        self.upload_points(&pts);
        self.elapsed += dt;
    }

    fn upload_points(&mut self, pts: &[P<F>]) {
        let rc = unsafe { nbody_upload(self.handle, pts.as_ptr() as *const c_void, pts.len(), std::mem::size_of::<P<F>>()) };
        self.check(rc);
        self.dirty.set(true);
    }

    pub fn sync(&mut self) {
        let rc = unsafe { nbody_sync(self.handle) };
        self.check(rc);
    }

    pub fn options(&self) -> &HipOptions {
        &self.options
    }
}

impl<F: HipFloat, const METHOD: i32> Drop for HipSimulation<F, METHOD> {
    fn drop(&mut self) {
        unsafe { nbody_destroy(self.handle) }
    }
}

impl<F: HipFloat, const METHOD: i32> Clone for HipSimulation<F, METHOD> {
    fn clone(&self) -> Self {
        let mut h: *mut NbodyHandle = std::ptr::null_mut();
        let rc = unsafe { nbody_clone(self.handle, &mut h) };
        self.check(rc);
        Self {
            handle: h,
            points: UnsafeCell::new(Vec::new()),
            dirty: Cell::new(true),
            integrator: self.integrator.clone(),
            bounds: self.bounds,
            settings: self.settings.clone(),
            settings_dirty: true,
            elapsed: self.elapsed,
            options: self.options,
            #[cfg(feature = "render")]
            points_buffer: self.points_buffer.clone(),
            #[cfg(feature = "render")]
            bounds_buffer: self.bounds_buffer.clone(),
            #[cfg(feature = "render")]
            vertex_scratch: Vec::new(),
            #[cfg(feature = "render")]
            cell_scratch: (Vec::new(), Vec::new()),
        }
    }
}

impl<F: HipFloat, const METHOD: i32> Simulation<F, 3, P<F>, I<F>> for HipSimulation<F, METHOD> {
    fn new(points: Vec<P<F>>, integrator: I<F>, bounds: Bounds<F, 3>) -> Self {
        Self::with_options(points, integrator, bounds, HipOptions::default())
    }

    fn init(&mut self) {
        self.integrator.init();
        self.elapsed = F::from(0.0).unwrap();
        let rc = unsafe { nbody_init(self.handle) };
        self.check(rc);
    }

    fn step_by(&mut self, dt: F) {
        self.push_settings();
        let rc = unsafe { F::abi_step_by(self.handle, dt) };
        self.check(rc);
        self.elapsed += dt;
        self.dirty.set(true);
    }

    fn update_forces(&mut self) {
        self.push_settings();
        let rc = unsafe { nbody_update_forces(self.handle) };
        self.check(rc);
        self.dirty.set(true);
    }

    fn add_point(&mut self, point: P<F>) {
        let rc = unsafe { nbody_add_point(self.handle, &point as *const P<F> as *const c_void) };
        self.check(rc);
        self.dirty.set(true);
    }

    fn remove_point(&mut self, index: usize) {
// ... 127 lines not shown
```

Before: 5690 billion.

## Specialize symmetric brute-force kernels for uniform-mass bodies

At upload and add_point the host checks whether every body has bit-identical finite mass and bounded position, and records that mass. When this holds, the symmetric packed brute-force kernels and the rest kernels run in a uniform-mass form. That form drops the per-pair mj and mi multiplies and the mass lane rotation, and folds G·m into the final reduce. The aim is fewer VALU and cross-lane ops in the inner pair loop, at the cost of extra template instances, host-side scanning on upload, and a path that only applies to single-segment, packed, 4-wave configurations.

```diff
diff --git a/include/nbody_hip.h b/include/nbody_hip.h
--- a/include/nbody_hip.h
+++ b/include/nbody_hip.h
@@ -58,7 +58,7 @@
     int32_t tree_build;
     int32_t dtype;
     int32_t shard_mode;
-    int32_t reserved;
+    int32_t bf_uniform;
 } NbodyConfig;
 
 typedef struct NbodyStats {
diff --git a/nbody-llm_amd/__init__.py b/nbody-llm_amd/__init__.py
--- a/nbody-llm_amd/__init__.py
+++ b/nbody-llm_amd/__init__.py
@@ -66,7 +66,7 @@
     _fields_ = [
         ("struct_size", C.c_uint32), ("method", C.c_int32), ("math_mode", C.c_int32), ("leaf_mode", C.c_int32),
         ("device", C.c_int32), ("rank", C.c_int32), ("world_size", C.c_int32), ("host_threads", C.c_int32),
-        ("capacity", C.c_uint64), ("tree_build", C.c_int32), ("dtype", C.c_int32), ("shard_mode", C.c_int32), ("reserved", C.c_int32),
+        ("capacity", C.c_uint64), ("tree_build", C.c_int32), ("dtype", C.c_int32), ("shard_mode", C.c_int32), ("bf_uniform", C.c_int32),
     ]
 
 
diff --git a/nbody-llm_amd/csrc/bf_pair.h b/nbody-llm_amd/csrc/bf_pair.h
--- a/nbody-llm_amd/csrc/bf_pair.h
+++ b/nbody-llm_amd/csrc/bf_pair.h
@@ -9,8 +9,9 @@
 }
 
 #define PAD_POS 1.0e15f
+#define PAD_LIVE_MAX 3.0e14f
 
-template <int IPT, int DBG = 0, bool SYM = true>
+template <int IPT, int DBG = 0, bool SYM = true, bool UNI = false>
 __device__ __forceinline__ void pair_evals(const float (&xi)[IPT], const float (&yi)[IPT], const float (&zi)[IPT],
                                            const float (&mi)[IPT], float (&axi)[IPT], float (&ayi)[IPT],
                                            float (&azi)[IPT], float xj, float yj, float zj, float mj, float& axj,
@@ -44,13 +45,20 @@
 #pragma unroll
     for (int q = 0; q < IPT; ++q) r[q] = sj[q] * r[q];
     __builtin_amdgcn_sched_barrier(0);
+    if (UNI) {
 #pragma unroll
-    for (int q = 0; q < IPT; ++q) sj[q] = mj * r[q];
-    __builtin_amdgcn_sched_barrier(0);
+        for (int q = 0; q < IPT; ++q) sj[q] = r[q];
+    } else {
+#pragma unroll
+        for (int q = 0; q < IPT; ++q) sj[q] = mj * r[q];
+        __builtin_amdgcn_sched_barrier(0);
+    }
     if (SYM) {
+        if (!UNI) {
 #pragma unroll
-        for (int q = 0; q < IPT; ++q) r[q] = mi[q] * r[q];
-        __builtin_amdgcn_sched_barrier(0);
+            for (int q = 0; q < IPT; ++q) r[q] = mi[q] * r[q];
+            __builtin_amdgcn_sched_barrier(0);
+        }
 #pragma unroll
         for (int q = 0; q < IPT; ++q) {
             axi[q] = __builtin_fmaf(dx[q], sj[q], axi[q]);
@@ -80,7 +88,7 @@
 __device__ __forceinline__ v2f splat2(float v) { v2f r = {v, v}; return r; }
 __device__ __forceinline__ v2f pk_fma(v2f a, v2f b, v2f c) { return __builtin_elementwise_fma(a, b, c); }
 
-template <int IPT2, int DBG = 0, bool SYM = true>
+template <int IPT2, int DBG = 0, bool SYM = true, bool UNI = false>
 __device__ __forceinline__ void pair_evals_pk(const v2f (&xi)[IPT2], const v2f (&yi)[IPT2], const v2f (&zi)[IPT2],
                                               const v2f (&mi)[IPT2], v2f (&axi)[IPT2], v2f (&ayi)[IPT2],
                                               v2f (&azi)[IPT2], float xj, float yj, float zj, float mj, v2f& axj,
@@ -115,13 +123,20 @@
 #pragma unroll
     for (int q = 0; q < IPT2; ++q) r[q] = sj[q] * r[q];
     __builtin_amdgcn_sched_barrier(0);
+    if (UNI) {
 #pragma unroll
-    for (int q = 0; q < IPT2; ++q) sj[q] = mj2 * r[q];
-    __builtin_amdgcn_sched_barrier(0);
+        for (int q = 0; q < IPT2; ++q) sj[q] = r[q];
+    } else {
+#pragma unroll
+        for (int q = 0; q < IPT2; ++q) sj[q] = mj2 * r[q];
+        __builtin_amdgcn_sched_barrier(0);
+    }
     if (SYM) {
+        if (!UNI) {
 #pragma unroll
-        for (int q = 0; q < IPT2; ++q) r[q] = mi[q] * r[q];
-        __builtin_amdgcn_sched_barrier(0);
+            for (int q = 0; q < IPT2; ++q) r[q] = mi[q] * r[q];
+            __builtin_amdgcn_sched_barrier(0);
+        }
 #pragma unroll
         for (int q = 0; q < IPT2; ++q) {
             axi[q] = pk_fma(dx[q], sj[q], axi[q]);
diff --git a/nbody-llm_amd/csrc/kernels.h b/nbody-llm_amd/csrc/kernels.h
--- a/nbody-llm_amd/csrc/kernels.h
+++ b/nbody-llm_amd/csrc/kernels.h
@@ -8,6 +8,7 @@
 struct Tuning {
     int cross_sym = 1;
     int sym_packed = 1;
+    int sym_uniform = 1;
     int bf_fast_variant = 0;
     int bh_walk_duo = -1;
     int bh_walk_xcd = 1;
@@ -91,11 +92,14 @@
 SymPlan make_sym_plan(int n_upper);
 int sym_bodies_per_lane(size_t n);
 uint64_t sym_main_pairs(const SymPlan& p, size_t n);
+inline int sym_plan_wpb(const Tuning& t) { return t.sym_wpb == 8 ? 8 : t.sym_wpb == 12 ? 12 : t.sym_wpb == 16 ? 16 : 4; }
+inline bool sym_uniform_supported(const Tuning& t) { return t.sym_packed && sym_plan_wpb(t) == 4; }
+constexpr float kUniformLiveMax = 3.0e14f, kUniformBoxMax = 1.0e14f;
 void launch_bf_sym_main(hipStream_t s, const Shard& sh, const SymPlan& p, const int* d_bounds, float4* planes,
-                        int n_upper, float g_soft2);
+                        int n_upper, float g_soft2, bool uniform = false);
 void launch_bf_os(hipStream_t s, const Shard& sh, int A, int K, float4* planes, size_t plane_stride, float g_soft2);
 void launch_bf_sym_tail(hipStream_t s, const Shard& sh, const SymPlan& p, float4* planes, int n_upper, float g,
-                        float g_soft2, const float* kick_dt);
+                        float g_soft2, const float* kick_dt, bool uniform = false);
 
 struct CrossPartners {
     static constexpr int kMax = 8;
diff --git a/nbody-llm_amd/csrc/kernels_bf_sym.hip b/nbody-llm_amd/csrc/kernels_bf_sym.hip
--- a/nbody-llm_amd/csrc/kernels_bf_sym.hip
+++ b/nbody-llm_amd/csrc/kernels_bf_sym.hip
@@ -2,6 +2,7 @@
 #include "bf_pair.h"
 
 #include <algorithm>
+#include <cassert>
 
 namespace nbody {
 
@@ -13,15 +14,15 @@
 
 }
 
-template <int IPT>
+template <int IPT, bool UNI>
 __device__ __forceinline__ void sym_rest_wave(const float4* __restrict__ pos, int n, int A, int group, int slice,
                                               int n_slices, float& ax, float& ay, float& az, float eps2);
 
-template <int IPT, int NW>
+template <int IPT, int NW, bool UNI>
 __device__ __forceinline__ void sym_rest_block(const float4* __restrict__ pos, int n, int A, int group,
                                                float4* __restrict__ plane, float eps2, float (*red)[3][64]);
 
-template <int IPT, int WPB, int DBG = 0, bool PK = false>
+template <int IPT, int WPB, int DBG = 0, bool PK = false, bool UNI = false>
 __global__ __launch_bounds__(WPB * 64) void k_bf_sym(const float4* __restrict__ pos, const int* __restrict__ count,
                                                      int A, int K, const int* __restrict__ bounds, int sym_sets,
                                                      float4* __restrict__ planes, size_t plane_stride, float eps2,
@@ -31,7 +32,7 @@
     const int n_main_blocks = (A * K + WPB - 1) / WPB;
     if (int(blockIdx.x) >= n_main_blocks) {
         __shared__ float red[WPB - 1][3][64];
-        sym_rest_block<IPT, WPB>(pos, *count, A, blockIdx.x - n_main_blocks,
+        sym_rest_block<IPT, WPB, UNI>(pos, *count, A, blockIdx.x - n_main_blocks,
                                  planes + size_t(sym_sets + (res_combine ? K / WPB : K)) * plane_stride, eps2, red);
         return;
     }
@@ -74,6 +75,8 @@
         pack_pairs<IPT>(xi, xi2); pack_pairs<IPT>(yi, yi2); pack_pairs<IPT>(zi, zi2); pack_pairs<IPT>(mi, mi2);
         pack_pairs<IPT>(axi, axi2); pack_pairs<IPT>(ayi, ayi2); pack_pairs<IPT>(azi, azi2);
     }
+    static_assert(PK || !UNI, "the uniform-mass instances exist in the packed form only");
+    static_assert(kUniformLiveMax == PAD_LIVE_MAX, "the host's bound on live positions is the one bf_pair.h argues from");
     for (int k = k0; k < k1; ++k) {
         float xj = nxt.x, yj = nxt.y, zj = nxt.z, mj = nxt.w;
         float axj = 0.f, ayj = 0.f, azj = 0.f;
@@ -87,12 +90,14 @@
         }
         if (PK) {
             for (int s = 0; s < 64; s += 2) {
-                const float x1 = rotl(xj, src_lane), y1 = rotl(yj, src_lane), z1 = rotl(zj, src_lane), m1 = rotl(mj, src_lane);
-                pair_evals_pk<IPT / 2, DBG>(xi2, yi2, zi2, mi2, axi2, ayi2, azi2, xj, yj, zj, mj, axj2, ayj2, azj2, eps2v);
+                const float x1 = rotl(xj, src_lane), y1 = rotl(yj, src_lane), z1 = rotl(zj, src_lane);
+                const float m1 = UNI ? 0.f : rotl(mj, src_lane);
+                pair_evals_pk<IPT / 2, DBG, true, UNI>(xi2, yi2, zi2, mi2, axi2, ayi2, azi2, xj, yj, zj, mj, axj2, ayj2, azj2, eps2v);
                 axj2.x = rotl(axj2.x, src_lane); ayj2.x = rotl(ayj2.x, src_lane); azj2.x = rotl(azj2.x, src_lane);
                 axj2.y = rotl(axj2.y, src_lane); ayj2.y = rotl(ayj2.y, src_lane); azj2.y = rotl(azj2.y, src_lane);
-                xj = rotl(x1, src_lane); yj = rotl(y1, src_lane); zj = rotl(z1, src_lane); mj = rotl(m1, src_lane);
-                pair_evals_pk<IPT / 2, DBG>(xi2, yi2, zi2, mi2, axi2, ayi2, azi2, x1, y1, z1, m1, axj2, ayj2, azj2, eps2v);
+                xj = rotl(x1, src_lane); yj = rotl(y1, src_lane); zj = rotl(z1, src_lane);
+                if (!UNI) mj = rotl(m1, src_lane);
+                pair_evals_pk<IPT / 2, DBG, true, UNI>(xi2, yi2, zi2, mi2, axi2, ayi2, azi2, x1, y1, z1, m1, axj2, ayj2, azj2, eps2v);
                 axj2.x = rotl(axj2.x, src_lane); ayj2.x = rotl(ayj2.x, src_lane); azj2.x = rotl(azj2.x, src_lane);
                 axj2.y = rotl(axj2.y, src_lane); ayj2.y = rotl(ayj2.y, src_lane); azj2.y = rotl(azj2.y, src_lane);
             }
@@ -233,7 +238,7 @@
     for (int q = 0; q < IPT; ++q) out[size_t(a * IPT + q) * 64 + lane] = make_float4(axi[q], ayi[q], azi[q], 0.f);
 }
 
-template <int IPT>
+template <int IPT, bool UNI>
 __device__ __forceinline__ void sym_rest_wave(const float4* __restrict__ pos, int n, int A, int group, int slice,
                                               int n_slices, float& ax, float& ay, float& az, float eps2) {
     constexpr int SET = 64 * IPT;
@@ -254,7 +259,8 @@
             const float dx = pj.x - pi.x, dy = pj.y - pi.y, dz = pj.z - pi.z;
             const float r2 = __builtin_fmaf(dz, dz, __builtin_fmaf(dy, dy, __builtin_fmaf(dx, dx, eps2)));
             const float rinv = __builtin_amdgcn_rsqf(r2);
-            float sj = pj.w * ((rinv * rinv) * rinv);
+            float sj = (rinv * rinv) * rinv;
+            if (!UNI) sj = pj.w * sj;
             sj = (j == i) ? 0.f : sj;
             ax = __builtin_fmaf(dx, sj, ax);
             ay = __builtin_fmaf(dy, sj, ay);
@@ -263,13 +269,13 @@
     }
 }
 
-template <int IPT, int NW>
+template <int IPT, int NW, bool UNI>
 __device__ __forceinline__ void sym_rest_block(const float4* __restrict__ pos, int n, int A, int group,
                                                float4* __restrict__ plane, float eps2, float (*red)[3][64]) {
     const int lane = threadIdx.x & 63;
     const int wv = __builtin_amdgcn_readfirstlane(threadIdx.x >> 6);
     float ax, ay, az;
-    sym_rest_wave<IPT>(pos, n, A, group, wv, NW, ax, ay, az, eps2);
+    sym_rest_wave<IPT, UNI>(pos, n, A, group, wv, NW, ax, ay, az, eps2);
     if (wv > 0) { red[wv - 1][0][lane] = ax; red[wv - 1][1][lane] = ay; red[wv - 1][2][lane] = az; }
     __syncthreads();
     if (wv == 0) {
@@ -279,11 +285,11 @@
     }
 }
 
-template <int IPT>
+template <int IPT, bool UNI = false>
 __global__ __launch_bounds__(512) void k_bf_sym_rest(const float4* __restrict__ pos, const int* __restrict__ count,
                                                      int A, float4* __restrict__ plane, float eps2) {
     __shared__ float red[7][3][64];
-    sym_rest_block<IPT, 8>(pos, *count, A, blockIdx.x, plane, eps2, red);
+    sym_rest_block<IPT, 8, UNI>(pos, *count, A, blockIdx.x, plane, eps2, red);
 }
 
 template <bool KICK>
@@ -386,8 +392,7 @@
     p.A = (n_upper + 64 * IPT - 1) / (64 * IPT);
     p.sym_sets = (p.A + 1) / 2 - 1;
     const int L = IPT * p.sym_sets;
-    const int want = tuning().sym_wpb;
-    p.wpb = want == 8 ? 8 : want == 12 ? 12 : want == 16 ? 16 : 4;
+    p.wpb = sym_plan_wpb(tuning());
     int K = 1;
     if (p.wpb == 4) {
         K = L <= 100 ? L : L <= 160 ? (L + 1) / 2 : 64;
@@ -436,7 +441,7 @@
 }
 
 void launch_bf_sym_main(hipStream_t s, const Shard& sh, const SymPlan& p, const int* d_bounds, float4* planes,
-                        int n_upper, float g_soft2) {
+                        int n_upper, float g_soft2, bool uniform) {
     if (n_upper <= 0 || p.sym_sets <= 0) return;
     const int main_blocks = (p.A * p.K + p.wpb - 1) / p.wpb;
     const int rest_blocks = int(p.n_pad / 64);
@@ -447,6 +452,17 @@
 #else
     constexpr int dbg = 0;
 #endif
+#define SYM_ARGS grid, block, 0, s, sh.own_pos(), sh.own_count(), p.A, p.K, d_bounds, p.sym_sets, planes, p.plane_stride, g_soft2, p.res_combine
+    if (uniform) {
+        assert(p.wpb == 4 && tuning().sym_packed && "uniform-mass instances: packed form, 4-wave workgroups (sym_uniform_supported)");
+#ifdef NBODY_TUNING
+        if (dbg == 4 && p.ipt == 8) { hipLaunchKernelGGL((k_bf_sym<8, 4, 4, true, true>), SYM_ARGS); return; }
+#endif
+        if (p.ipt == 4) hipLaunchKernelGGL((k_bf_sym<4, 4, 0, true, true>), SYM_ARGS);
+        else hipLaunchKernelGGL((k_bf_sym<8, 4, 0, true, true>), SYM_ARGS);
+        return;
+    }
+#undef SYM_ARGS
     if (p.ipt == 4) {
         hipLaunchKernelGGL((k_bf_sym<4, 4, 0, true>), grid, block, 0, s, sh.own_pos(), sh.own_count(), p.A, p.K, d_bounds, p.sym_sets, planes, p.plane_stride, g_soft2, p.res_combine);
         return;
@@ -488,17 +504,18 @@
 }
 
 void launch_bf_sym_tail(hipStream_t s, const Shard& sh, const SymPlan& p, float4* planes, int n_upper, float g,
-                        float g_soft2, const float* kick_dt) {
+                        float g_soft2, const float* kick_dt, bool uniform) {
     if (n_upper <= 0) return;
     if (p.sym_sets == 0) {
         float4* resident0 = planes + size_t(p.sym_sets) * p.plane_stride;
         (void)hipMemsetAsync(resident0, 0, size_t(p.k_res) * p.plane_stride * sizeof(float4), s);
-        if (p.ipt == 4)
-            hipLaunchKernelGGL(k_bf_sym_rest<4>, dim3(int(p.n_pad / 64)), dim3(512), 0, s, sh.own_pos(),
-                               sh.own_count(), p.A, planes + size_t(p.sym_sets + p.k_res) * p.plane_stride, g_soft2);
-        else
-        hipLaunchKernelGGL(k_bf_sym_rest<8>, dim3(int(p.n_pad / 64)), dim3(512), 0, s, sh.own_pos(),
-                           sh.own_count(), p.A, planes + size_t(p.sym_sets + p.k_res) * p.plane_stride, g_soft2);
+#define REST_ARGS dim3(int(p.n_pad / 64)), dim3(512), 0, s, sh.own_pos(), sh.own_count(), p.A, planes + size_t(p.sym_sets + p.k_res) * p.plane_stride, g_soft2
+        if (uniform) {
+            if (p.ipt == 4) hipLaunchKernelGGL((k_bf_sym_rest<4, true>), REST_ARGS);
+            else hipLaunchKernelGGL((k_bf_sym_rest<8, true>), REST_ARGS);
+        } else if (p.ipt == 4) hipLaunchKernelGGL((k_bf_sym_rest<4>), REST_ARGS);
+        else hipLaunchKernelGGL((k_bf_sym_rest<8>), REST_ARGS);
+#undef REST_ARGS
     }
     const float dt = kick_dt ? *kick_dt : 0.f;
 #define REDUCE_ARGS planes, p.n_planes, p.plane_stride, sh.own_count(), g, sh.acc, sh.own_pos(), sh.vel, dt, sh.seg_count, sh.n_seg, sh.inter
diff --git a/nbody-llm_amd/csrc/nbody_api.cpp b/nbody-llm_amd/csrc/nbody_api.cpp
--- a/nbody-llm_amd/csrc/nbody_api.cpp
+++ b/nbody-llm_amd/csrc/nbody_api.cpp
@@ -192,7 +192,36 @@
     return NBODY_OK;
 }
 
+bool uniform_candidate(const float* rec) {
+    const float m = rec[9];
+    if (!std::isfinite(m) || m == 0.f) return false;
+    for (int c = 0; c < 3; ++c)
+        if (!(std::fabs(rec[c]) <= nbody::kUniformLiveMax)) return false;
+    return true;
+}
+bool same_bits(float a, float b) { return std::memcmp(&a, &b, sizeof(float)) == 0; }
+
+bool uniform_applies(const NbodyHandle* h, const nbody::Tuning& t) {
+    if (!t.sym_uniform || !h->mass_uniform || h->sh.n_seg != 1 || !nbody::sym_uniform_supported(t) || !h->bounds_set) return false;
+    for (int c = 0; c < 3; ++c)
+        if (!(std::fabs(h->bnd.lo[c]) <= nbody::kUniformBoxMax && std::fabs(h->bnd.hi[c]) <= nbody::kUniformBoxMax)) return false;
+    return true;
+}
+
 constexpr size_t kShardedSymMinBodies = 2048;
+
+struct BfPath {
+    bool sym;
+    bool uniform;
+};
+BfPath bf_path(const NbodyHandle* h, const nbody::Tuning& t) {
+    const bool fast = h->cfg.math_mode == NBODY_MATH_FAST && t.bf_fast_variant == 0;
+    const bool sharded = h->sh.n_seg > 1;
+    BfPath p;
+    p.sym = fast && (sharded ? size_t(h->sh.seg_cap) >= kShardedSymMinBodies : h->n_local >= size_t(std::max(1024, t.sym_min_bodies)));
+    p.uniform = p.sym && !sharded && uniform_applies(h, t);
+    return p;
+}
 
 int ensure_sym_plan(NbodyHandle* h) {
     const size_t set = size_t(64) * size_t(nbody::sym_bodies_per_lane(std::max<size_t>(1, h->n_local)));
@@ -260,9 +289,9 @@
 
 int bf_forces(NbodyHandle* h) {
     const float eps2 = h->g_soft * h->g_soft;
-    const bool fast = h->cfg.math_mode == NBODY_MATH_FAST && nbody::tuning().bf_fast_variant == 0;
     const bool sharded = h->sh.n_seg > 1;
-    const bool sym = fast && (sharded ? size_t(h->sh.seg_cap) >= kShardedSymMinBodies : h->n_local >= size_t(std::max(1024, nbody::tuning().sym_min_bodies)));
+    const BfPath path = bf_path(h, nbody::tuning());
+    const bool sym = path.sym;
     const size_t tot = total_upper(h);
     if (sym) {
         int rc = ensure_sym_plan(h);
@@ -284,13 +313,15 @@
         else nbody::launch_bf_forces_fast(h->stream, h->sh, int(h->n_local), h->g, eps2);
         timed = tot > 0 ? uint64_t(h->n_local) * uint64_t(tot - 1) : 0;
     } else if (!sharded) {
+        h->sym_uniform_now = path.uniform;
         {
             ForceTimer t(h);
-            nbody::launch_bf_sym_main(h->stream, h->sh, p, h->d_sym_bounds, h->d_planes, int(h->n_local), eps2);
+            nbody::launch_bf_sym_main(h->stream, h->sh, p, h->d_sym_bounds, h->d_planes, int(h->n_local), eps2, h->sym_uniform_now);
         }
         timed = 2 * h->sym_pairs;
         h->tail_pending = true;
     } else {
+        h->sym_uniform_now = path.uniform;
         nbody::launch_bf_sym_main(h->stream, h->sh, p, h->d_sym_bounds, h->d_planes, int(h->n_local), eps2);
         {
             int rc = exchange_wait(h);
@@ -648,8 +679,8 @@
     if (!h->tail_pending) return NBODY_OK;
     h->tail_pending = false;
     const float eps2 = h->g_soft * h->g_soft;
-    nbody::launch_bf_sym_tail(h->stream, h->sh, h->sym_plan, h->d_planes, int(h->n_local), h->g, eps2,
-                              h->kick_pending ? &h->kick_dt : nullptr);
+    nbody::launch_bf_sym_tail(h->stream, h->sh, h->sym_plan, h->d_planes, int(h->n_local), h->sym_uniform_now ? h->g * h->mass_m : h->g, eps2,
+                              h->kick_pending ? &h->kick_dt : nullptr, h->sym_uniform_now);
     h->kick_pending = false;
     HIP_TRY(h, hipGetLastError());
     return NBODY_OK;
@@ -986,7 +1017,7 @@
     {
         nbody::Tuning& t = h->tune;
         const struct { const char* env; int* knob; } table[] = {
-            {"NBODY_BF_VARIANT", &t.bf_fast_variant}, {"NBODY_CROSS_SYM", &t.cross_sym}, {"NBODY_SYM_PACKED", &t.sym_packed},
+            {"NBODY_BF_VARIANT", &t.bf_fast_variant}, {"NBODY_CROSS_SYM", &t.cross_sym}, {"NBODY_SYM_PACKED", &t.sym_packed}, {"NBODY_SYM_UNIFORM", &t.sym_uniform},
             {"NBODY_BH_SPLIT", &t.bh_walk_split}, {"NBODY_SYM_WPB", &t.sym_wpb}, {"NBODY_SYM_IPT", &t.sym_ipt}, {"NBODY_BH_DUO", &t.bh_walk_duo}, {"NBODY_BH_XCD", &t.bh_walk_xcd},
 #ifdef NBODY_TUNING
             {"NBODY_BH_VARIANT", &t.bh_walk_variant}, {"NBODY_BH_HOT", &t.bh_hot_cap}, {"NBODY_BH_LDS_BLOCK", &t.bh_walk_lds_block},
@@ -1056,6 +1087,7 @@
     h->n_local = src->n_local;
     h->seg_count_host = src->seg_count_host;
     h->first_global = src->first_global; h->n_at_upload = src->n_at_upload;
+    h->mass_uniform = src->mass_uniform; h->mass_m = src->mass_m;
     if (src->let) {
         rc = nbody::let::clone_state(s, h);
         if (rc) { g_create_err = h->err; free_all(h); return rc; }
@@ -1081,6 +1113,15 @@
     if (rc) return rc;
     const char* src = static_cast<const char*>(aos);
     for (size_t k = 0; k < n; ++k) std::memcpy(h->h_aos + 10 * k, src + k * stride, 40);
+    h->mass_uniform = false;
+    h->mass_m = 0.f;
+    if (G == 1 && n > 0 && uniform_candidate(h->h_aos)) {
+        const float m0 = h->h_aos[9];
+        bool uni = true;
+        for (size_t k = 1; k < n && uni; ++k) uni = same_bits(h->h_aos[10 * k + 9], m0) && uniform_candidate(h->h_aos + 10 * k);
+        h->mass_uniform = uni;
+        h->mass_m = uni ? m0 : 0.f;
+    }
     if (n) HIP_TRY(h, hipMemcpyAsync(h->d_aos, h->h_aos, n * 40, hipMemcpyHostToDevice, h->stream));
     for (size_t s = 0; s < G; ++s) {
         size_t lo = std::min(n, s * blk), hi = std::min(n, lo + blk);
@@ -1172,6 +1213,8 @@
     HIP_TRY(h, hipStreamSynchronize(h->stream));
     h->n_local = k + 1;
     h->seg_count_host[0] = int(h->n_local);
+    if (k == 0) { h->mass_uniform = uniform_candidate(p); h->mass_m = h->mass_uniform ? p[9] : 0.f; }
+    else if (h->mass_uniform && !(same_bits(p[9], h->mass_m) && uniform_candidate(p))) { h->mass_uniform = false; h->mass_m = 0.f; }
     return push_counts(h);
 }
 
@@ -1629,7 +1672,7 @@
 namespace {
 struct Knob { const char* name; int nbody::Tuning::*field; bool tuning_build_only; };
 const Knob kKnobs[] = {
-    {"cross_sym", &nbody::Tuning::cross_sym, false}, {"sym_packed", &nbody::Tuning::sym_packed, false},
+    {"cross_sym", &nbody::Tuning::cross_sym, false}, {"sym_packed", &nbody::Tuning::sym_packed, false}, {"sym_uniform", &nbody::Tuning::sym_uniform, false},
     {"bf_fast_variant", &nbody::Tuning::bf_fast_variant, false}, {"sym_wpb", &nbody::Tuning::sym_wpb, false}, {"sym_ipt", &nbody::Tuning::sym_ipt, false}, {"let_list_div", &nbody::Tuning::let_list_div, false}, {"bh_walk_duo", &nbody::Tuning::bh_walk_duo, false}, {"bh_walk_xcd", &nbody::Tuning::bh_walk_xcd, false},
     {"sym_rounds", &nbody::Tuning::sym_rounds, false}, {"sym_k", &nbody::Tuning::sym_k, false},
     {"sym_min_bodies", &nbody::Tuning::sym_min_bodies, false}, {"sym_reduce_split", &nbody::Tuning::sym_reduce_split, false},
@@ -1671,6 +1714,7 @@
 int nbody_get_config(const NbodyHandle* h, NbodyConfig* out) {
     if (!h || !out) return NBODY_ERR_INVALID;
     *out = h->cfg;
+    out->bf_uniform = (!h->f64 && !h->let && h->cfg.method == NBODY_BRUTE_FORCE && bf_path(h, h->tune).uniform) ? 1 : 0;
     return NBODY_OK;
 }
 
diff --git a/nbody-llm_amd/csrc/nbody_handle.h b/nbody-llm_amd/csrc/nbody_handle.h
--- a/nbody-llm_amd/csrc/nbody_handle.h
+++ b/nbody-llm_amd/csrc/nbody_handle.h
@@ -259,6 +259,9 @@
     bool kick_pending = false;
     float kick_dt = 0.f;
     uint64_t sym_pairs = 0;
+    bool mass_uniform = false;
+    float mass_m = 0.f;
+    bool sym_uniform_now = false;
     size_t sym_pairs_n = 0;
 
     bool async_bh = false;
diff --git a/nbody-llm_amd/rust/src/lib.rs b/nbody-llm_amd/rust/src/lib.rs
--- a/nbody-llm_amd/rust/src/lib.rs
+++ b/nbody-llm_amd/rust/src/lib.rs
@@ -23,7 +23,7 @@
     tree_build: i32,
     dtype: i32,
     shard_mode: i32,
-    reserved: i32,
+    bf_uniform: i32,
 }
 
 #[repr(C)]
@@ -191,7 +191,7 @@
             tree_build: o.tree_build as i32,
             dtype: F::DTYPE,
             shard_mode: 0,
-            reserved: 0,
+            bf_uniform: 0,
         };
         let mut h: *mut NbodyHandle = std::ptr::null_mut();
         let rc = unsafe { nbody_create(&cfg, &mut h) };
```

Result: faster. 6152 billion, median of 6 (+8.1%).
